# VITA-Group/MLSP

Hardware: AMD Instinct MI355X
Metric: points/sec fwd+bwd, DGCNN+MLSP B=32 N=1024 k=20 (higher is better)
Workload: dtype f32; 1 GPU; DGCNN encoder + 3 MLSP heads + losses, fwd+bwd+Adam, B=32/GPU N=1024 k=20 fp32 (BASELINE.json configs[1]), dropout 0.5, BN train; global_batch=32, points_per_cloud=1024, k=20, parallelism=dp1

## Files before the change

### mlsp_amd/csrc/api.hip

```cpp
#include "common.h"
#include "../../include/mlsp_hip.h"
#include "knn_plan.h"

#define CHECK(x) do { int _r = (x); if (_r != MLSP_OK) return _r; } while (0)
#define SLAB_BOUND_FLOATS ((size_t)16 << 20)

#include <mutex>
#include <unordered_map>
hipError_t mlsp_lds_limit(const void* fn, size_t lds) {
    static std::mutex mu;
    static std::unordered_map<uint64_t, size_t> raised;
    int dev = 0;
    (void)hipGetDevice(&dev);
    const uint64_t key = (uint64_t)(uintptr_t)fn * 64u + (uint64_t)(dev & 63);
    std::lock_guard<std::mutex> lk(mu);
    auto it = raised.find(key);
    if (it != raised.end() && it->second >= lds) return hipSuccess;
    const hipError_t e = hipFuncSetAttribute(fn, hipFuncAttributeMaxDynamicSharedMemorySize, (int)lds);
    if (e == hipSuccess) raised[key] = lds;
    return e;
}

extern "C" {

int mlsp_abi_version(void) { return MLSP_ABI_VERSION; }

const char* mlsp_strerror(int code) {
    switch (code) {
        case MLSP_OK: return "ok";
        case MLSP_ERR_ARG: return "mlsp: bad argument (null pointer, non-positive or unsupported shape)";
        case MLSP_ERR_WORKSPACE: return "mlsp: workspace too small (see mlsp_workspace_bytes)";
        case MLSP_ERR_UNSUPPORTED: return "mlsp: unsupported size for this kernel";
        default: return code > 0 ? hipGetErrorString((hipError_t)code) : "mlsp: unknown error";
    }
}

size_t mlsp_workspace_bytes(int rows, int cin, int cout) {
    size_t r = rows > 0 ? rows : 1, ci = cin > 0 ? cin : 1, co = cout > 0 ? cout : 1;
    size_t act = 3 * r * co * sizeof(float) + r * sizeof(float)
               + r * ci * sizeof(float);
    size_t parts = (r / 64 + 2) * 2 * co * sizeof(double);
    size_t wts = 4 * co * ci * sizeof(float) * 2 + 8 * co * sizeof(float);
    return act + parts + wts + SLAB_BOUND_FLOATS * sizeof(float) + (32 << 20) + MLSP_AMAX_TAIL_BYTES;
}

int mlsp_gemm_f32(int ta, int tb, int M, int N, int K, const float* A, int lda, const float* B, int ldb, float* C, int ldc,
                  const float* bias, int precision, void* ws, size_t ws_bytes, mlsp_stream_t st) {
    CallCtx cx(precision, ws, ws_bytes);
    if (!cx.ok()) return MLSP_ERR_ARG;
    Workspace w(ws, ws_bytes);
    GemmOpts o; o.bias = bias;
    take_slab(w, o, gemm_slab_floats(M, N, K));
    if (!o.slab) o.slab_floats = 0;
    return launch_gemm(st, cx, ta != 0, tb != 0, M, N, K, A, lda, B, ldb, C, ldc, o);
}

int mlsp_knn_f32(const float* x, int ldx, int B, int N, int C, int k, int32_t* idx, int32_t* rev_off, int32_t* rev_ent,
                 void* ws, size_t ws_bytes, mlsp_stream_t st) {
    if (B <= 0 || N <= 0) return MLSP_ERR_ARG;
    Workspace w(ws, ws_bytes);
    float* xx = w.take<float>((size_t)B * N);
    if (!w.ok()) return MLSP_ERR_WORKSPACE;
    KnnAsk q;
    q.B = B; q.N = N; q.C = C; q.k = k; q.ld = ldx; q.x16 = ((uintptr_t)x & 15) == 0; q.planes_avail = (size_t)-1;
    const size_t pbytes = knn_plan(q).plane_bytes;
    char* planes = pbytes ? w.take<char>(pbytes) : nullptr;
    {
        const int cls = C <= 4 ? MLSP_PROF_KNN_C3 : C == 64 ? MLSP_PROF_KNN_C64 : C == 128 ? MLSP_PROF_KNN_C128 : 0;
        const int tok = prof_cls_begin(st, cls);
        const int rc = launch_knn(st, x, ldx, B, N, C, k, idx, xx, planes, planes ? pbytes : 0);
        prof_cls_end(st, tok, C <= 4 ? (double)B * N * (C + k) * 4.0 : 2.0 * B * N * (double)N * C);
        if (rc != MLSP_OK) return rc;
    }
    if (rev_off) CHECK(launch_knn_reverse(st, idx, B, N, k, rev_off, rev_ent));
    return MLSP_OK;
}

int mlsp_knn_reverse(const int32_t* idx, int B, int N, int k, int32_t* rev_off, int32_t* rev_ent, mlsp_stream_t st) {
    return launch_knn_reverse(st, idx, B, N, k, rev_off, rev_ent);
}

int mlsp_region_assign_f32(const float* X, int B, int C, int N, const float* thr, int n, float clip, int32_t* regions, mlsp_stream_t st) {
    return launch_region_assign(st, X, B, C, N, thr, n, clip, regions);
}
int mlsp_deform_regions_f32(float* X, int B, int C, int N, const int32_t* regions, const int32_t* order, int nreg, const float* lookup,
                            const float* noise, int min_pts, int groups, float* mask, mlsp_stream_t st) {
    return launch_deform_regions(st, X, B, C, N, regions, order, nreg, lookup, noise, min_pts, groups, mask);
}
int mlsp_knn_query_f32(const float* ref, int ldr, int Nr, const float* qry, int ldq, int Nq, int B, int C, int k, int32_t* idx, float* dist,
                       mlsp_stream_t st) {
    return launch_knn_query(st, ref, ldr, Nr, qry, ldq, Nq, B, C, k, idx, dist);
}
int mlsp_interp3_fwd_f32(const float* feat, const int32_t* idx, const float* dist, int B, int N, int S, int D, float* out, mlsp_stream_t st) {
    return launch_interp3_fwd(st, feat, idx, dist, B, N, S, D, out);
}
int mlsp_interp3_bwd_f32(const float* dout, const float* dist, const int32_t* rev_off, const int32_t* rev_ent, int B, int N, int S, int D,
                         float* dfeat, mlsp_stream_t st) {
    return launch_interp3_bwd(st, dout, dist, rev_off, rev_ent, B, N, S, D, dfeat);
}
int mlsp_compose_linear_fwd_f32(const float* Wa, const float* ba, const float* Wb, const float* bb, int Cm, int Ci, int Co, float* W, float* b,
                                mlsp_stream_t st) {
    if (!Wa || !ba || !Wb || !bb || !W || !b || Cm <= 0 || Ci <= 0 || Co <= 0 || Cm > 1024 || Ci > 1024 || Co > 1024) return MLSP_ERR_ARG;
    return launch_compose_fwd((hipStream_t)st, Wa, ba, Wb, bb, Cm, Ci, Co, W, b);
}
int mlsp_compose_linear_bwd_f32(const float* dW, const float* db, const float* Wa, const float* ba, const float* Wb, int Cm, int Ci, int Co,
                                float* dWa, float* dba, float* dWb, mlsp_stream_t st) {
    if (!dW || !db || !Wa || !ba || !Wb || !dWa || !dba || !dWb || Cm <= 0 || Ci <= 0 || Co <= 0 || Cm > 1024 || Ci > 1024 || Co > 1024) return MLSP_ERR_ARG;
    return launch_compose_bwd((hipStream_t)st, dW, db, Wa, ba, Wb, Cm, Ci, Co, dWa, dba, dWb);
}

int mlsp_transform3_fwd_f32(const float* x, const float* T, int B, int N, float* out, mlsp_stream_t st) {
    return launch_transform3_fwd(st, x, T, B, N, out);
}
int mlsp_transform3_bwd_f32(const float* x, const float* T, const float* dout, int B, int N, float* dx, float* dT, mlsp_stream_t st) {
    return launch_transform3_bwd(st, x, T, dout, B, N, dx, dT);
}
int mlsp_collapse_to_point_f32(float* X, int B, int N, const int32_t* choice, const float* u, const float* noise, float radius2,
                               int min_pts, float* mask, int32_t* chosen, mlsp_stream_t st) {
    return launch_collapse_to_point(st, X, B, N, choice, u, noise, radius2, min_pts, mask, chosen);
}
int mlsp_scan_select_f32(const float* X, int B, int N, int C, const double* R, int pixel, float* Xs, float* mask, mlsp_stream_t st) {
    return launch_scan_select(st, X, B, N, C, R, pixel, Xs, mask);
}
int mlsp_fps_f32(const float* xyz, int ldx, int B, int N, int S, const int32_t* start, int32_t* fps_idx, mlsp_stream_t st) {
    return launch_fps(st, xyz, ldx, B, N, S, start, fps_idx);
}
int mlsp_ball_query_f32(const float* xyz, int ldx, const float* new_xyz, int ldq, int B, int N, int S, float radius_sq, int nsample,
                        int32_t* idx, mlsp_stream_t st) {
    return launch_ball_query(st, xyz, ldx, new_xyz, ldq, B, N, S, radius_sq, nsample, idx);
}
int mlsp_group_reverse(const int32_t* idx, int B, int S, int N, int ns, int32_t* rev_off, int32_t* rev_ent, mlsp_stream_t st) {
    return launch_group_reverse(st, idx, B, S, N, ns, rev_off, rev_ent);
}
int mlsp_sa_group_fwd_f32(const float* xyz, int ldx, const float* feat, int D, const float* new_xyz, int ldq, const int32_t* idx, int B,
                          int N, int S, int ns, float* G, mlsp_stream_t st) {
    return launch_sa_group_fwd(st, xyz, ldx, feat, D, new_xyz, ldq, idx, B, N, S, ns, G);
}
int mlsp_sa_group_bwd_f32(const float* dG, int ldg, int col, int D, const int32_t* rev_off, const int32_t* rev_ent, int B, int N, int S, int ns,
                          float* dfeat, mlsp_stream_t st) {
    return launch_sa_group_bwd(st, dG, ldg, col, D, rev_off, rev_ent, B, N, S, ns, dfeat);
}


int mlsp_sa_fold_fwd_f32(const float* u, const float* w, const int32_t* idx, int B, int N, int S, int ns, int C, const float* gamma,
                         const float* beta, float* run_mean, float* run_var, float momentum, float eps, int training, float* Z,
                         float* bn_save, void* ws, size_t ws_bytes, mlsp_stream_t st) {
    if (B <= 0 || S <= 0 || ns <= 0 || C <= 0) return MLSP_ERR_ARG;
    Workspace wk(ws, ws_bytes);
    double* part = training ? wk.take<double>((size_t)sa_fold_parts((long)B * S * ns) * 2 * C) : nullptr;
    if (!wk.ok()) return MLSP_ERR_WORKSPACE;
    return launch_sa_fold_fwd(st, u, w, idx, B, N, S, ns, C, gamma, beta, run_mean, run_var, momentum, eps, training, Z, bn_save, part);
}

int mlsp_sa_fold_bwd_f32(const float* dZ, const float* u, const float* w, const int32_t* idx, const int32_t* rev_off, const int32_t* rev_ent,
                         const int32_t* rev_cnt, const int32_t* pad_cnt, int B, int N, int S, int ns, int C, const float* bn_save, int training,
                         float* du, float* dw, float* dgamma, float* dbeta, void* ws, size_t ws_bytes, mlsp_stream_t st) {
    if (B <= 0 || S <= 0 || ns <= 0 || C <= 0) return MLSP_ERR_ARG;
    Workspace wk(ws, ws_bytes);
    double* part = wk.take<double>((size_t)sa_fold_parts((long)B * S * ns) * 2 * C);
    float* mean_dz = wk.take<float>(C);
    float* mean_dzy = wk.take<float>(C);
    if (!wk.ok()) return MLSP_ERR_WORKSPACE;
    return launch_sa_fold_bwd(st, dZ, u, w, idx, rev_off, rev_ent, B, N, S, ns, C, bn_save, training, du, dw, dgamma, dbeta, part, mean_dz,
                              mean_dzy, rev_cnt, pad_cnt);
}

int mlsp_group_reverse_compact(const int32_t* idx, int B, int S, int N, int ns, int32_t* rev_off, int32_t* rev_cnt, int32_t* rev_ent,
                               int32_t* pad_cnt, mlsp_stream_t st) {
    return launch_group_reverse_compact(st, idx, B, S, N, ns, rev_off, rev_cnt, rev_ent, pad_cnt);
}

int mlsp_graph_feature_fwd_f32(const float* x, const int32_t* idx, int B, int N, int C, int k, float* F, mlsp_stream_t st) {
    if (!x || !idx || !F || B <= 0 || N <= 0 || C <= 0 || k <= 0) return MLSP_ERR_ARG;
    return launch_graph_feature_fwd(st, x, idx, B * N, N, C, k, F);
}
int mlsp_graph_feature_bwd_f32(const float* dF, const int32_t* rev_off, const int32_t* rev_ent, int B, int N, int C, int k,
                               float* dx, mlsp_stream_t st) {
    if (!dF || !rev_off || !rev_ent || !dx || B <= 0 || N <= 0 || C <= 0 || k <= 0) return MLSP_ERR_ARG;
    return launch_graph_feature_bwd(st, dF, rev_off, rev_ent, B * N, N, C, k, dx);
}

int mlsp_edgeconv_fwd_f32(const float* x, int ldx, const int32_t* idx, const float* W, const float* gamma, const float* beta,
                          float* run_mean, float* run_var, float momentum, float eps, int act, float slope, int training,
                          int B, int N, int C, int Cout, int k, float* out, int ldo, float* uv, float* msel, uint8_t* argsel,
                          float* s1, float* bn_save, float* Wd_out, int precision, void* ws, size_t ws_bytes, mlsp_stream_t st) {
    CallCtx cx(precision, ws, ws_bytes);
    if (!cx.ok()) return MLSP_ERR_ARG;
    if (!x || !idx || !W || !gamma || !beta || !out || !uv || !msel || !argsel || !s1 || !bn_save) return MLSP_ERR_ARG;
    if (B <= 0 || N <= 0 || C <= 0 || Cout <= 0 || k <= 0 || k > 255 || ldx < C || ldo < Cout) return MLSP_ERR_ARG;
    const int P = B * N;
    Workspace w(ws, ws_bytes);
    float* Wd = Wd_out ? Wd_out : w.take<float>((size_t)2 * Cout * C);
    int nparts = edge_reduce_parts(P);
    double* part = w.take<double>((size_t)nparts * 2 * Cout);
    GemmOpts so; take_slab(w, so, gemm_slab_floats(P, 2 * Cout, C));
    if (!w.ok()) return MLSP_ERR_WORKSPACE;
    float* scale = bn_save, *shift = bn_save + Cout, *mean = bn_save + 2 * Cout, *invstd = bn_save + 3 * Cout;
    if (!training) {
        if (!run_mean || !run_var) return MLSP_ERR_ARG;
        CHECK(launch_build_wd_eval(st, W, Cout, C, Wd, Cout, gamma, beta, run_mean, run_var, bn_save, 0, nullptr, nullptr, nullptr, nullptr, nullptr, eps));
    } else CHECK(launch_build_wd(st, W, Cout, C, Wd, (C >= 128 && C % 32 == 0 && build_wd_leaves_bound(Cout, C)) ? cx.reserve(Wd, 2 * Cout, C, C) : nullptr));
    CHECK(launch_gemm(st, cx, false, true, P, 2 * Cout, C, x, ldx, Wd, C, uv, 2 * Cout, so));
    {
        const int tok = prof_cls_begin(st, MLSP_PROF_EDGE_REDUCE);
        const int rc = launch_edge_reduce(st, uv, idx, gamma, P, N, Cout, k, msel, argsel, s1, part, &nparts);
        prof_cls_end(st, tok, (double)P * (Cout * 4.0 + k * 4.0 + Cout * 9.0));
        if (rc != MLSP_OK) return rc;
    }
    if (training) {
        CHECK(launch_bn_finalize(st, part, nparts, (double)P * k, Cout, gamma, beta, run_mean, run_var, momentum, eps, scale,
                                 shift, mean, invstd, cx.offered_output(out, P, Cout, ldo, Cout)));
    }
    CHECK(launch_edge_select_act(st, msel, uv, P, Cout, scale, shift, act, slope, out, ldo));
    return MLSP_OK;
}

int mlsp_edgeconv_bwd_f32(const float* dOut, int lddo, const float* x, int ldx, const int32_t* rev_off, const int32_t* rev_ent,
                          const float* W, const float* out, int ldo, const float* uv, const float* msel, const uint8_t* argsel,
                          const float* s1, const float* bn_save, const float* Wd_in, int act, float slope, int training, int B, int N, int C,
                          int Cout, int k, float* dx, int lddx, int dx_accumulate, float* dW, float* dgamma, float* dbeta, int precision, void* ws,
                          size_t ws_bytes, mlsp_stream_t st) {
    CallCtx cx(precision, ws, ws_bytes);
    if (!cx.ok()) return MLSP_ERR_ARG;
    if (!dOut || !x || !rev_off || !rev_ent || !W || !out || !uv || !msel || !argsel || !s1 || !bn_save || !dW || !dgamma ||
        !dbeta)
        return MLSP_ERR_ARG;
    if (B <= 0 || N <= 0 || C <= 0 || Cout <= 0 || k <= 0 || ldx < C || lddo < Cout || ldo < Cout || (dx && lddx < C)) return MLSP_ERR_ARG;
    const int P = B * N;
    Workspace w(ws, ws_bytes);
    float* Wd = Wd_in ? nullptr : w.take<float>((size_t)2 * Cout * C);
    float* dWd = w.take<float>((size_t)2 * Cout * C);
    float* gz = w.take<float>((size_t)P * Cout);
    float* duv = w.take<float>((size_t)P * 2 * Cout);
    int nparts = bn_parts_max(P);
    double* part = w.take<double>((size_t)nparts * 2 * Cout);
    float* mean_dz = w.take<float>(Cout);
    float* mean_dzy = w.take<float>(Cout);
    GemmOpts so; take_slab(w, so, gemm_slab_floats(P, C, 2 * Cout), gemm_slab_floats(2 * Cout, C, P));
    if (!w.ok()) return MLSP_ERR_WORKSPACE;
    const float* scale = bn_save, *mean = bn_save + 2 * Cout, *invstd = bn_save + 3 * Cout;
    float* duv_amax = (C % 128 == 0 && edge_bwd_leaves_duv_bound(dOut, out, msel, uv, s1, argsel, Cout, scale, mean, invstd, gz, duv, lddo, ldo))
                          ? cx.reserve(duv, P, 2 * Cout, 2 * Cout) : nullptr;
    CHECK(launch_edge_bwd_reduce(st, dOut, out, msel, uv, P, Cout, mean, invstd, act, slope, part, lddo, ldo, duv_amax));
    CHECK(launch_bn_bwd_finalize(st, part, edge_bwd_reduce_parts(P, Cout, dOut, out, msel, uv, mean, invstd, lddo, ldo), (double)P * k, Cout,
                                 dgamma, dbeta, mean_dz, mean_dzy));
    const float* mdz = training ? mean_dz : nullptr;
    CHECK(launch_edge_bwd_point(st, dOut, out, uv, s1, P, Cout, k, scale, mean, invstd, mdz, mean_dzy, act, slope, gz, duv, lddo, ldo, duv_amax));
    CHECK(launch_edge_bwd_gather(st, gz, argsel, uv, rev_off, rev_ent, P, N, Cout, scale, mean, invstd, mdz, mean_dzy, duv, duv_amax));
    const float* Wdc = Wd_in;
    if (!Wdc && dx) { CHECK(launch_build_wd(st, W, Cout, C, Wd)); Wdc = Wd; }
    GemmOpts od = so; od.accumulate = dx_accumulate != 0;
    if (dx) CHECK(launch_gemm(st, cx, false, false, P, C, 2 * Cout, duv, 2 * Cout, Wdc, C, dx, lddx, od));
    bool unfolded = false;
    GemmOpts ow = so; ow.unfold_dw = dW; ow.unfolded = &unfolded;
    CHECK(launch_gemm(st, cx, true, false, 2 * Cout, C, P, duv, 2 * Cout, x, ldx, dWd, C, ow));
    if (!unfolded) CHECK(launch_unbuild_wd(st, dWd, Cout, C, dW));
    return MLSP_OK;
}

int mlsp_tnet_edge_fwd_f32(const float* x, int ldx, const int32_t* idx, const float* W1, const float* gamma1, const float* beta1,
                           float* run_mean1, float* run_var1, const float* W2, const float* gamma2, const float* beta2,
                           float* run_mean2, float* run_var2, float momentum, float eps, float slope, int training, int B, int N,
                           int C, int C1, int C2, int k, float* out, float* uv, float* s1, float* bn1_save, float* zsel,
                           uint8_t* argsel, float* bn2_save, int precision, void* ws, size_t ws_bytes, mlsp_stream_t st) {
    CallCtx cx(precision, ws, ws_bytes);
    if (!cx.ok()) return MLSP_ERR_ARG;
    if (!x || !idx || !W1 || !gamma1 || !beta1 || !W2 || !gamma2 || !beta2 || !out || !uv || !s1 || !bn1_save || !zsel || !argsel ||
        !bn2_save)
        return MLSP_ERR_ARG;
    if (B <= 0 || N <= 0 || C <= 0 || k <= 0 || ldx < C) return MLSP_ERR_ARG;
    if (C1 != 64 || C2 != 128 || tnet_points_per_tile(k) <= 0) return MLSP_ERR_UNSUPPORTED;
    const int P = B * N;
    Workspace w(ws, ws_bytes);
    float* Wd = w.take<float>((size_t)2 * C1 * C);
    float* msel = w.take<float>((size_t)P * C1);
    uint8_t* arg1 = w.take<uint8_t>((size_t)P * C1);
    int np1 = edge_reduce_parts(P), np2 = tnet_fwd_parts(B, N, k);
    double* part = w.take<double>((size_t)(np1 > np2 ? np1 : np2) * 2 * C2);
    GemmOpts so; take_slab(w, so, gemm_slab_floats(P, 2 * C1, C));
    if (!w.ok()) return MLSP_ERR_WORKSPACE;
    if (!training) {
        if (!run_mean1 || !run_var1 || !run_mean2 || !run_var2) return MLSP_ERR_ARG;
        CHECK(launch_build_wd_eval(st, W1, C1, C, Wd, C1, gamma1, beta1, run_mean1, run_var1, bn1_save, C2, gamma2, beta2, run_mean2, run_var2, bn2_save, eps));
    } else CHECK(launch_build_wd(st, W1, C1, C, Wd));
    CHECK(launch_gemm(st, cx, false, true, P, 2 * C1, C, x, ldx, Wd, C, uv, 2 * C1, so));
    CHECK(launch_edge_reduce(st, uv, idx, gamma1, P, N, C1, k, msel, arg1, s1, part, &np1));
    if (training) {
        CHECK(launch_bn_finalize(st, part, np1, (double)P * k, C1, gamma1, beta1, run_mean1, run_var1, momentum, eps, bn1_save,
                                 bn1_save + C1, bn1_save + 2 * C1, bn1_save + 3 * C1));
    }
    {
        const int tok = prof_cls_begin(st, MLSP_PROF_TNET_FWD);
        const int rc = launch_tnet_edge_fwd(st, cx.mode(), uv, idx, bn1_save, W2, gamma2, P, N, k, slope, zsel, argsel, part);
        prof_cls_end(st, tok, 2.0 * P * (double)k * C1 * C2);
        if (rc != MLSP_OK) return rc;
    }
    if (training) {
        CHECK(launch_bn_finalize(st, part, np2, (double)P * k, C2, gamma2, beta2, run_mean2, run_var2, momentum, eps, bn2_save,
                                 bn2_save + C2, bn2_save + 2 * C2, bn2_save + 3 * C2, cx.offered_output(out, P, C2, C2, C2)));
    }
    CHECK(launch_tnet_out(st, zsel, bn2_save, P, slope, out));
    return MLSP_OK;
}

int mlsp_tnet_edge_bwd_f32(const float* dOut, const float* x, int ldx, const int32_t* idx, const int32_t* rev_off,
                           const int32_t* rev_ent, const float* W1, const float* W2, const float* out, const float* uv,
                           const float* s1, const float* bn1_save, const float* zsel, const uint8_t* argsel, const float* bn2_save,
                           float slope, int training, int B, int N, int C, int C1, int C2, int k, float* dx, float* dW1,
                           float* dgamma1, float* dbeta1, float* dW2, float* dgamma2, float* dbeta2, int precision, void* ws, size_t ws_bytes,
                           mlsp_stream_t st) {
    CallCtx cx(precision, ws, ws_bytes);
    if (!cx.ok()) return MLSP_ERR_ARG;
    if (!dOut || !x || !idx || !W1 || !W2 || !out || !uv || !s1 || !bn1_save || !zsel || !argsel || !bn2_save ||
        !dW1 || !dgamma1 || !dbeta1 || !dW2 || !dgamma2 || !dbeta2)
        return MLSP_ERR_ARG;
    if ((!rev_off || !rev_ent) && (dx || C > 4)) return MLSP_ERR_ARG;
    if (B <= 0 || N <= 0 || C <= 0 || k <= 0 || ldx < C) return MLSP_ERR_ARG;
    if (C1 != 64 || C2 != 128 || tnet_points_per_tile(k) <= 0) return MLSP_ERR_UNSUPPORTED;
    const int P = B * N;
    const size_t E = (size_t)P * k;
    const int ntiles = B * ((N + tnet_points_per_tile(k) - 1) / tnet_points_per_tile(k));
    const int nb = tnet_grid(ntiles);
    Workspace w(ws, ws_bytes);
    float* Wd = w.take<float>((size_t)2 * C1 * C);
    float* dWd = w.take<float>((size_t)2 * C1 * C);
    float* g = w.take<float>((size_t)P * C2);
    float* coef = w.take<float>(2 * C2);
    float* dhp = w.take<float>(E * C1);
    float* dW2part = w.take<float>(tnet_bwd_scratch_floats(ntiles));
    int npr = (P + 511) / 512;
    const int nprv = bn_vec_parts(P);
    const int nrows_part = (npr > nb ? npr : nb) > nprv ? (npr > nb ? npr : nb) : nprv;
    double* part = w.take<double>((size_t)nrows_part * 2 * C2);
    float* mean_dz = w.take<float>(C2);
    float* mean_dzy = w.take<float>(C2);
    float* m1 = w.take<float>(C1);
    float* m2 = w.take<float>(C1);
    float* duv = w.take<float>((size_t)P * 2 * C1);
    GemmOpts so; take_slab(w, so, gemm_slab_floats(P, C, 2 * C1), gemm_slab_floats(2 * C1, C, P));
    if (!w.ok()) return MLSP_ERR_WORKSPACE;
    {
        const int rc = launch_bn_act_bwd_partials_vec(st, dOut, zsel, P, C2, bn2_save, bn2_save + C2, bn2_save + 2 * C2, bn2_save + 3 * C2,
                                                      2, slope, part);
        if (rc == MLSP_OK) npr = nprv;
        else if (rc != MLSP_ERR_UNSUPPORTED) return rc;
        else CHECK(launch_tnet_bwd_reduce(st, dOut, out, zsel, bn2_save, P, slope, part));
    }
    CHECK(launch_bn_bwd_finalize(st, part, npr, (double)E, C2, dgamma2, dbeta2, mean_dz, mean_dzy));
    CHECK(launch_tnet_bwd_g(st, dOut, out, bn2_save, training ? mean_dz : nullptr, mean_dzy, P, slope, g, coef));
    int nparts = 0;
    {
        const int tok = prof_cls_begin(st, MLSP_PROF_TNET_BWD);
        const int rc = launch_tnet_edge_bwd(st, cx.mode(), uv, idx, bn1_save, W2, bn2_save, g, argsel, coef, P, N, k, slope, dhp, dW2part, part, dW2, &nparts);
        prof_cls_end(st, tok, 4.0 * P * (double)k * C1 * C2);
        if (rc != MLSP_OK) return rc;
    }
    CHECK(launch_bn_bwd_finalize(st, part, nparts, (double)E, C1, dgamma1, dbeta1, m1, m2));
    if (!dx && C <= 4) {
        double* mom = w.take<double>(tnet_w1_moment_doubles(P, k));
        if (!w.ok()) return MLSP_ERR_WORKSPACE;
        return launch_tnet_bwd_w1_moments(st, dhp, idx, rev_off, x, ldx, W1, bn1_save, training ? m1 : nullptr, m2, P, N, k, C, mom, dW1);
    }
    CHECK(launch_tnet_edge_bwd2(st, dhp, uv, s1, bn1_save, training ? m1 : nullptr, m2, rev_off, rev_ent, P, N, k, duv));
    CHECK(launch_build_wd(st, W1, C1, C, Wd));
    if (dx) CHECK(launch_gemm(st, cx, false, false, P, C, 2 * C1, duv, 2 * C1, Wd, C, dx, C, so));
    CHECK(launch_gemm(st, cx, true, false, 2 * C1, C, P, duv, 2 * C1, x, ldx, dWd, C, so));
    CHECK(launch_unbuild_wd(st, dWd, C1, C, dW1));
    return MLSP_OK;
}

static bool defer_ok(const mlsp_defer_t* in) {
    return in->bn_save && in->ld > 0 && in->col >= 0 && in->p_drop >= 0.f && in->p_drop < 1.f && in->act >= 0 && in->act <= 2;
}
static GemmXf chain_xf(const mlsp_defer_t& in, int which, int batch_stats) {
    GemmXf x;
    x.scale = in.bn_save + in.col; x.shift = in.bn_save + in.ld + in.col; x.act = in.act; x.slope = in.slope; x.thresh = dropout_thresh8(in.p_drop);
    x.inv_keep = dropout_inv_keep8(in.p_drop); x.seed = in.seed; x.ld = in.ld; x.col = in.col; x.which = which;
    if (batch_stats) { x.mean = in.bn_save + 2 * in.ld + in.col; x.invstd = in.bn_save + 3 * in.ld + in.col; }
    return x;
}
static bool defer_fusable(const mlsp_defer_t& in) { return !(in.act == 2 && !(in.slope >= 0.f && in.slope <= 1.f)); }

static int pointmlp_fwd_impl(CallCtx& cx, const float* X, int ldx, int M, int Cin, const float* W, int ldw, int Cout, const float* bias,
                             const float* gbias, int rows_per_group, const float* gamma, const float* beta, float* run_mean,
                             float* run_var, float momentum, float eps, int training, int act, float slope, float p_drop,
                             uint64_t seed, float* Y, float* Z, float* bn_save, void* ws, size_t ws_bytes, mlsp_stream_t st,
                             const mlsp_defer_t* in, float* group_ysum) {
    if (!X || !W || (!Z && !gamma) || M <= 0 || Cin <= 0 || Cout <= 0 || ldx < Cin || ldw < Cin) return MLSP_ERR_ARG;
    if (group_ysum && (!gamma || !gbias || rows_per_group <= 0 || M % rows_per_group || M <= 32)) return MLSP_ERR_ARG;
    if (gamma && (!beta || !Y || !bn_save)) return MLSP_ERR_ARG;
    if (p_drop < 0.f || p_drop >= 1.f) return MLSP_ERR_ARG;
    if (in && (!defer_ok(in) || in->col + Cin > in->ld)) return MLSP_ERR_ARG;
    if (gamma && !gbias && M <= 32 && !in && Z)
        return launch_skinny_linear_bn_act(st, X, ldx, M, Cin, W, ldw, Cout, bias, gamma, beta, run_mean, run_var, momentum, eps,
                                           training, act, slope, p_drop, seed, Y, Z, bn_save);
    Workspace w(ws, ws_bytes);
    const int fused_parts = (gamma && training) ? gemm_stat_parts(cx, M, Cout, Cin) : 0;
    int nparts = fused_parts ? fused_parts : bn_stat_parts(M);
    double* part = gamma ? w.take<double>((size_t)nparts * 2 * Cout) : nullptr;
    GemmOpts o; o.bias = bias; o.gbias = gbias; o.rows_per_group = rows_per_group;
    take_slab(w, o, gemm_slab_floats(M, Cout, Cin));
    GemmXf xf_s;
    if (in) {
        xf_s = chain_xf(*in, 1, training);
        if (defer_fusable(*in) && gemm_xf_supported(cx, false, true, M, Cout, Cin, X, ldx, W, ldw, 1)) o.xf = &xf_s;
        else {
            float* Xa = w.take<float>((size_t)M * Cin);
            if (!w.ok()) return MLSP_ERR_WORKSPACE;
            CHECK(launch_xf_materialize(st, X, ldx, M, Cin, xf_s, Xa));
            X = Xa; ldx = Cin;
        }
    }
    if (!w.ok()) return MLSP_ERR_WORKSPACE;
    if (!gamma) {
        if (act || p_drop > 0.f) return MLSP_ERR_UNSUPPORTED;
        return launch_gemm(st, cx, false, true, M, Cout, Cin, X, ldx, W, ldw, Z, Cout, o);
    }
    float* scale = bn_save, *shift = bn_save + Cout, *mean = bn_save + 2 * Cout, *invstd = bn_save + 3 * Cout;
    o.stat_part = fused_parts ? part : nullptr;
    CHECK(launch_gemm(st, cx, false, true, M, Cout, Cin, X, ldx, W, ldw, Y, Cout, o));
    const int prow = fused_parts ? M / fused_parts : 0;
    const bool gsum_fin = group_ysum && training && fused_parts && M % fused_parts == 0 && rows_per_group % prow == 0;
    if (training) {
        if (!fused_parts) CHECK(launch_colstats(st, Y, M, Cout, Cout, part));
        if (gsum_fin) CHECK(launch_bn_finalize_groups(st, part, nparts, (double)M, Cout, gamma, beta, run_mean, run_var, momentum, eps, scale, shift,
                                                      mean, invstd, group_ysum, rows_per_group / prow));
        else CHECK(launch_bn_finalize(st, part, nparts, (double)M, Cout, gamma, beta, run_mean, run_var, momentum, eps, scale, shift,
                                      mean, invstd));
    } else {
        if (!run_mean || !run_var) return MLSP_ERR_ARG;
        CHECK(launch_bn_eval_prepare(st, Cout, gamma, beta, run_mean, run_var, eps, scale, shift, mean, invstd));
    }
    if (group_ysum && !gsum_fin) {
        float* gscr = w.take<float>((size_t)(M / rows_per_group) * 16 * Cout);
        if (!w.ok()) return MLSP_ERR_WORKSPACE;
        CHECK(launch_colsum_groups(st, Y, M / rows_per_group, rows_per_group, Cout, group_ysum, gscr));
    }
    if (Z) CHECK(launch_bn_act_fwd(st, Y, Z, (size_t)M, Cout, scale, shift, act, slope, training ? p_drop : 0.f, seed));
    return MLSP_OK;
}

int mlsp_pointmlp_fwd_f32(const float* X, int ldx, int M, int Cin, const float* W, int ldw, int Cout, const float* bias,
                          const float* gbias, int rows_per_group, const float* gamma, const float* beta, float* run_mean,
                          float* run_var, float momentum, float eps, int training, int act, float slope, float p_drop,
                          uint64_t seed, float* Y, float* Z, float* bn_save, float* group_ysum, int precision, void* ws, size_t ws_bytes,
                          mlsp_stream_t st) {
    CallCtx cx(precision, ws, ws_bytes);
    if (!cx.ok()) return MLSP_ERR_ARG;
    return pointmlp_fwd_impl(cx, X, ldx, M, Cin, W, ldw, Cout, bias, gbias, rows_per_group, gamma, beta, run_mean, run_var, momentum, eps,
                             training, act, slope, p_drop, seed, Y, Z, bn_save, ws, ws_bytes, st, nullptr, group_ysum);
}

int mlsp_pointmlp_fwd_chain_f32(const float* Xpre, int ldx, const mlsp_defer_t* in, int M, int Cin, const float* W, int ldw, int Cout, const float* bias,
                                const float* gbias, int rows_per_group, const float* gamma, const float* beta, float* run_mean,
                                float* run_var, float momentum, float eps, int training, int act, float slope, float p_drop,
                                uint64_t seed, float* Y, float* Z, float* bn_save, float* group_ysum, int precision, void* ws, size_t ws_bytes,
                                mlsp_stream_t st) {
    CallCtx cx(precision, ws, ws_bytes);
    if (!cx.ok()) return MLSP_ERR_ARG;
    if (!in) return MLSP_ERR_ARG;
    return pointmlp_fwd_impl(cx, Xpre, ldx, M, Cin, W, ldw, Cout, bias, gbias, rows_per_group, gamma, beta, run_mean, run_var, momentum, eps,
                             training, act, slope, p_drop, seed, Y, Z, bn_save, ws, ws_bytes, st, in, group_ysum);
}

static int pointmlp_bwd_impl(CallCtx& cx, const float* dZ, const float* X, int ldx, int M, int Cin, const float* W, int ldw, int Cout, const float* Y,
                             const float* bn_save, int has_bn, int training, int act, float slope, float p_drop, uint64_t seed,
                             int n_groups, int rows_per_group, float* dX, int lddx, int dx_accumulate, float* dW, float* dbias, float* dgbias,
                             float* dgamma, float* dbeta, void* ws, size_t ws_bytes, mlsp_stream_t st, const mlsp_defer_t* in,
                             double* in_stats, const double* pre_stats, int pre_parts, const float* group_ysum) {
    if (!dZ || !X || !W || !dW || M <= 0 || Cin <= 0 || Cout <= 0 || ldx < Cin || ldw < Cin) return MLSP_ERR_ARG;
    if (in_stats && (!in || !dX || dx_accumulate)) return MLSP_ERR_ARG;
    if (pre_stats && (!has_bn || pre_parts <= 0 || M <= 32)) return MLSP_ERR_ARG;
    if (!pre_stats && pre_parts < 0 && (!has_bn || M <= 32)) return MLSP_ERR_ARG;
    if (has_bn && (!Y || !bn_save || !dgamma || !dbeta)) return MLSP_ERR_ARG;
    if (dgbias && (n_groups <= 0 || rows_per_group <= 0 || (long)n_groups * rows_per_group != M)) return MLSP_ERR_ARG;
    Workspace w(ws, ws_bytes);
    float* dY = has_bn ? w.take<float>((size_t)M * Cout) : nullptr;
    int nparts = bn_parts_max(M);
    double* part = (has_bn || dbias) ? w.take<double>((size_t)nparts * 2 * Cout) : nullptr;
    float* mean_dz = has_bn ? w.take<float>(Cout) : nullptr;
    float* mean_dzy = has_bn ? w.take<float>(Cout) : nullptr;
    GemmOpts so; take_slab(w, so, dX ? gemm_slab_floats(M, Cin, Cout) : 0, gemm_slab_floats(Cout, Cin, M));
    float* gscratch = dgbias ? w.take<float>((size_t)n_groups * 16 * Cout) : nullptr;
    float* coef = has_bn ? w.take<float>((size_t)4 * Cout) : nullptr;
    const float* Xorig = X; const int ldx_orig = ldx;
    GemmXf xf_s; const GemmXf* xf = nullptr;
    if (in) {
        if (!defer_ok(in) || in->col + Cin > in->ld || M <= 32) return MLSP_ERR_ARG;
        xf_s = chain_xf(*in, 2, training);
        if (defer_fusable(*in) && gemm_xf_supported(cx, true, false, Cout, Cin, M, dZ, Cout, X, ldx, 2)) xf = &xf_s;
        else {
            float* Xa = w.take<float>((size_t)M * Cin);
            if (!w.ok()) return MLSP_ERR_WORKSPACE;
            CHECK(launch_xf_materialize(st, X, ldx, M, Cin, xf_s, Xa));
            X = Xa; ldx = Cin;
        }
    }
    if (!w.ok()) return MLSP_ERR_WORKSPACE;
    const float* g = dZ;
    int g_slabs = 0;
    GemmDy dy_s = {Y, coef, Cout, 1}; const GemmDy* dy = nullptr;
    if (has_bn && M > 32 && pre_stats && training && (!in || xf) && M % pre_parts == 0 &&
        (!dX || gemm_dy_supported(cx, false, false, M, Cin, Cout, dZ, Cout, W, ldw)) && gemm_dy_supported(cx, true, false, Cout, Cin, M, dZ, Cout, X, ldx) &&
        (!dgbias || (rows_per_group >= 256 && rows_per_group % (M / pre_parts) == 0 && Cout % 4 == 0 && 256 % (Cout / 4) == 0 && Cout <= 1024)))
        dy = &dy_s;
    float* zb = (dbias && has_bn && training) ? dbias : nullptr;
    bool dbias_zeroed = false;
    if (dy && dgbias && group_ysum) {
        CHECK(launch_bn_bwd_finalize_coef_groups(st, pre_stats, pre_parts, (double)M, Cout, bn_save, dgamma, dbeta, coef, group_ysum,
                                                 rows_per_group / (M / pre_parts), rows_per_group, dgbias));
    } else if (dy) {
        CHECK(launch_bn_bwd_finalize_coef_z(st, pre_stats, pre_parts, (double)M, Cout, bn_save, dgamma, dbeta, coef, zb));
        dbias_zeroed = zb != nullptr;
        if (dgbias) CHECK(launch_bn_dy_gbias(st, Y, n_groups, rows_per_group, Cout, pre_stats, M / pre_parts, coef, gscratch, dgbias, group_ysum));
    } else if (has_bn && M <= 32) {
        CHECK(launch_skinny_bn_bwd_z(st, dZ, Y, dY, M, Cout, bn_save, training, act, slope, p_drop, seed, dgamma, dbeta, zb));
        dbias_zeroed = zb != nullptr;
        g = dY;
    } else if (has_bn) {
        const float* scale = bn_save, *shift = bn_save + Cout, *mean = bn_save + 2 * Cout, *invstd = bn_save + 3 * Cout;
        CHECK(launch_bn_act_bwd(st, dZ, Y, dY, M, Cout, scale, shift, mean, invstd, training, act, slope, training ? p_drop : 0.f, seed, part,
                                dgamma, dbeta, mean_dz, mean_dzy, zb, dgbias ? gscratch : nullptr, rows_per_group, &g_slabs, pre_stats, pre_parts));
        dbias_zeroed = zb != nullptr;
        g = dY;
    }
    GemmBs bs_s; const GemmBs* bs = nullptr;
    if (in_stats) {
        bs_s = {Xorig, ldx_orig, in->bn_save + in->col, in->ld, in->act, in->slope, dropout_thresh8(in->p_drop), dropout_inv_keep8(in->p_drop), in->seed,
                in->ld, in->col, in_stats + in->col, in->ld};
        bs_s.amax = (float*)(in_stats + (size_t)(M / 128) * 2 * in->ld) + in->col;
        bs = &bs_s;
    }
    if (M <= 32 && dX && !bs && !dy && !xf) {
        CHECK(launch_skinny_bwd_pair(st, g, Cout, W, ldw, X, ldx, dX, lddx, dW, M, Cin, Cout, dx_accumulate));
    } else {
    GemmOpts od = so; od.accumulate = dx_accumulate != 0; od.bs = bs; od.dy = dy;
    if (dX) CHECK(launch_gemm(st, cx, false, false, M, Cin, Cout, g, Cout, W, ldw, dX, lddx, od));
    GemmOpts ow = so; ow.xf = xf; ow.dy = dy;
    CHECK(launch_gemm(st, cx, true, false, Cout, Cin, M, g, Cout, X, ldx, dW, Cin, ow));
    }
    if (dbias) {
        if (has_bn && training) {
            if (!dbias_zeroed) {
                hipError_t e = hipMemsetAsync(dbias, 0, (size_t)Cout * sizeof(float), st);
                if (e != hipSuccess) return (int)e;
            }
        } else {
            CHECK(launch_colsum(st, g, M, Cout, part, dbias));
        }
    }
    if (dgbias && !dy) {
        if (g_slabs > 0) CHECK(launch_colsum_groups_fin(st, gscratch, n_groups, Cout, g_slabs, dgbias));
        else CHECK(launch_colsum_groups(st, g, n_groups, rows_per_group, Cout, dgbias, gscratch));
    }
    return MLSP_OK;
}

int mlsp_pointmlp_bwd_f32(const float* dZ, const float* X, int ldx, int M, int Cin, const float* W, int ldw, int Cout, const float* Y,
                          const float* bn_save, int has_bn, int training, int act, float slope, float p_drop, uint64_t seed,
                          int n_groups, int rows_per_group, float* dX, int lddx, int dx_accumulate, float* dW, float* dbias, float* dgbias,
                          float* dgamma, float* dbeta, const double* pre_stats, int pre_parts, const float* group_ysum, int precision, void* ws,
                          size_t ws_bytes, mlsp_stream_t st) {
    CallCtx cx(precision, ws, ws_bytes);
    if (!cx.ok()) return MLSP_ERR_ARG;
    return pointmlp_bwd_impl(cx, dZ, X, ldx, M, Cin, W, ldw, Cout, Y, bn_save, has_bn, training, act, slope, p_drop, seed, n_groups,
                             rows_per_group, dX, lddx, dx_accumulate, dW, dbias, dgbias, dgamma, dbeta, ws, ws_bytes, st, nullptr, nullptr,
                             pre_stats, pre_parts, group_ysum);
}

int mlsp_pointmlp_bwd_stats_parts(int M, int Cin, int Cout, int ldw, int lddx, int precision) {
    const CallCtx cx = CallCtx::query(precision);
    if (!cx.ok()) return 0;
    const int t = thin_bs_parts(M, Cin, Cout);
    return t ? t : gemm_bs_parts(cx, M, Cin, Cout, Cout, ldw, lddx);
}

int mlsp_pointmlp_bwd_chain_f32(const float* dZ, const float* Xpre, int ldx, const mlsp_defer_t* in, int M, int Cin, const float* W, int ldw, int Cout, const float* Y,
                                const float* bn_save, int has_bn, int training, int act, float slope, float p_drop, uint64_t seed,
                                int n_groups, int rows_per_group, float* dX, int lddx, int dx_accumulate, float* dW, float* dbias,
                                float* dgbias, float* dgamma, float* dbeta, double* in_stats, const double* pre_stats, int pre_parts,
                                const float* group_ysum, int precision, void* ws, size_t ws_bytes, mlsp_stream_t st) {
    CallCtx cx(precision, ws, ws_bytes);
    if (!cx.ok()) return MLSP_ERR_ARG;
    if (!in) return MLSP_ERR_ARG;
    return pointmlp_bwd_impl(cx, dZ, Xpre, ldx, M, Cin, W, ldw, Cout, Y, bn_save, has_bn, training, act, slope, p_drop, seed, n_groups,
                             rows_per_group, dX, lddx, dx_accumulate, dW, dbias, dgbias, dgamma, dbeta, ws, ws_bytes, st, in, in_stats,
                             pre_stats, pre_parts, group_ysum);
}

int mlsp_pointmlp_segmax_fwd_f32(const float* X, int ldx, int M, int Cin, const float* W, int ldw, int Cout, const float* bias,
                                 const float* gamma, const float* beta, float* run_mean, float* run_var, float momentum, float eps,
                                 int training, int act, float slope, int k, float* Y, float* out, float* ysel, uint8_t* argk, float* bn_save,
                                 int precision, void* ws, size_t ws_bytes, mlsp_stream_t st) {
    CallCtx cx(precision, ws, ws_bytes);
    if (!cx.ok()) return MLSP_ERR_ARG;
    if (!X || !W || !gamma || !beta || !Y || !out || !ysel || !argk || !bn_save || M <= 0 || Cin <= 0 || Cout <= 0 || ldx < Cin || ldw < Cin)
        return MLSP_ERR_ARG;
    if (k < 1 || k > 255 || M % k || Cout % 4) return MLSP_ERR_UNSUPPORTED;
    Workspace w(ws, ws_bytes);
    const int fused_parts = training ? gemm_stat_parts(cx, M, Cout, Cin) : 0;
    int nparts = fused_parts ? fused_parts : bn_stat_parts(M);
    double* part = w.take<double>((size_t)nparts * 2 * Cout);
    GemmOpts o; o.bias = bias; o.stat_part = fused_parts ? part : nullptr;
    take_slab(w, o, gemm_slab_floats(M, Cout, Cin));
    if (!w.ok()) return MLSP_ERR_WORKSPACE;
    float* scale = bn_save, *shift = bn_save + Cout, *mean = bn_save + 2 * Cout, *invstd = bn_save + 3 * Cout;
    CHECK(launch_gemm(st, cx, false, true, M, Cout, Cin, X, ldx, W, ldw, Y, Cout, o));
    if (training) {
        if (!fused_parts) CHECK(launch_colstats(st, Y, M, Cout, Cout, part));
        CHECK(launch_bn_finalize(st, part, nparts, (double)M, Cout, gamma, beta, run_mean, run_var, momentum, eps, scale, shift, mean, invstd));
    } else {
        if (!run_mean || !run_var) return MLSP_ERR_ARG;
        CHECK(launch_bn_eval_prepare(st, Cout, gamma, beta, run_mean, run_var, eps, scale, shift, mean, invstd));
    }
    return launch_segsel_act_fwd(st, Y, M / k, k, Cout, scale, shift, act, slope, out, ysel, argk);
}

int mlsp_pointmlp_segmax_bwd_f32(const float* dOut, const float* X, int ldx, int M, int Cin, const float* W, int ldw, int Cout, const float* Y,
                                 const float* ysel, const uint8_t* argk, const float* bn_save, int training, int act, float slope, int k,
                                 float* dX, int lddx, float* dW, float* dbias, float* dgamma, float* dbeta, int precision, void* ws, size_t ws_bytes,
                                 mlsp_stream_t st) {
    CallCtx cx(precision, ws, ws_bytes);
    if (!cx.ok()) return MLSP_ERR_ARG;
    if (!dOut || !X || !W || !Y || !ysel || !argk || !bn_save || !dW || !dgamma || !dbeta || M <= 0 || Cin <= 0 || Cout <= 0 || ldx < Cin ||
        ldw < Cin) return MLSP_ERR_ARG;
    if (k < 1 || k > 255 || M % k || Cout % 4) return MLSP_ERR_UNSUPPORTED;
    const int G = M / k;
    Workspace w(ws, ws_bytes);
    float* dY = w.take<float>((size_t)M * Cout);
    const int npr = bn_vec_parts(G);
    double* part = w.take<double>((size_t)npr * 2 * Cout);
    float* mean_dz = w.take<float>(Cout);
    float* mean_dzy = w.take<float>(Cout);
    GemmOpts so; take_slab(w, so, dX ? gemm_slab_floats(M, Cin, Cout) : 0, gemm_slab_floats(Cout, Cin, M));
    if (!w.ok()) return MLSP_ERR_WORKSPACE;
    const float* scale = bn_save, *shift = bn_save + Cout, *mean = bn_save + 2 * Cout, *invstd = bn_save + 3 * Cout;
    {
        const int rc = launch_bn_act_bwd_partials_vec(st, dOut, ysel, G, Cout, scale, shift, mean, invstd, act, slope, part);
        if (rc != MLSP_OK) return rc;
    }
    CHECK(launch_bn_bwd_finalize(st, part, npr, (double)M, Cout, dgamma, dbeta, mean_dz, mean_dzy));
    CHECK(launch_segsel_bwd_apply(st, dOut, Y, ysel, argk, (size_t)M, k, Cout, bn_save, training ? mean_dz : nullptr, mean_dzy, act, slope, dY));
    if (dX) CHECK(launch_gemm(st, cx, false, false, M, Cin, Cout, dY, Cout, W, ldw, dX, lddx, so));
    CHECK(launch_gemm(st, cx, true, false, Cout, Cin, M, dY, Cout, X, ldx, dW, Cin, so));
    if (dbias) {
        if (training) {
            hipError_t e = hipMemsetAsync(dbias, 0, (size_t)Cout * sizeof(float), st);
            if (e != hipSuccess) return (int)e;
        } else {
            CHECK(launch_colsum(st, dY, M, Cout, part, dbias));
        }
    }
    return MLSP_OK;
}

static int pointmlp_mx_supported(const CallCtx& cx, int M, int Cin, int Cout, int ldx, int x_bf16, int training) {
    if (M <= 32 || Cin % 32 || Cout % 128 || M % 128) return 0;
    if (x_bf16 ? (ldx % 8) : (ldx % 4)) return 0;
    if (Cout > 1024 || 256 % (Cout / 4)) return 0;
    if (training && gemm_stat_parts(cx, M, Cout, Cin) <= 0) return 0;
    if (gemm_slab_floats(M, Cout, Cin) != 0 || gemm_slab_floats(M, Cin, Cout) != 0) return 0;
    return 1;
}

int mlsp_pointmlp_mx_supported(int M, int Cin, int Cout, int ldx, int x_bf16, int training, int precision) {
    const CallCtx cx = CallCtx::query(precision);
    return cx.ok() ? pointmlp_mx_supported(cx, M, Cin, Cout, ldx, x_bf16, training) : 0;
}

int mlsp_pointmlp_fwd_mx(const void* X, int x_bf16, int ldx, int M, int Cin, const float* W, int ldw, int Cout, const float* bias,
                         const float* gbias, int rows_per_group, const float* gamma, const float* beta, float* run_mean,
                         float* run_var, float momentum, float eps, int training, int act, float slope, float p_drop, uint64_t seed,
                         void* Y, void* Z, int out_bf16, float* bn_save, int precision, void* ws, size_t ws_bytes, mlsp_stream_t st) {
    CallCtx cx(precision, ws, ws_bytes);
    if (!cx.ok()) return MLSP_ERR_ARG;
    if (!X || !W || !Y || !Z || !gamma || !beta || !bn_save || ldw < Cin || ldx < Cin) return MLSP_ERR_ARG;
    if (p_drop < 0.f || p_drop >= 1.f) return MLSP_ERR_ARG;
    if (!pointmlp_mx_supported(cx, M, Cin, Cout, ldx, x_bf16, training)) return MLSP_ERR_UNSUPPORTED;
    Workspace w(ws, ws_bytes);
    const int fused_parts = training ? gemm_stat_parts(cx, M, Cout, Cin) : 0;
    double* part = w.take<double>((size_t)(fused_parts ? fused_parts : 1) * 2 * Cout);
    if (!w.ok()) return MLSP_ERR_WORKSPACE;
    float* scale = bn_save, *shift = bn_save + Cout, *mean = bn_save + 2 * Cout, *invstd = bn_save + 3 * Cout;
    GemmOpts o; o.bias = bias; o.gbias = gbias; o.rows_per_group = rows_per_group; o.stat_part = fused_parts ? part : nullptr;
    CHECK(launch_gemm_mx(st, cx, false, true, M, Cout, Cin, X, x_bf16, ldx, W, 0, ldw, Y, out_bf16, Cout, o));
    if (training) {
        CHECK(launch_bn_finalize(st, part, fused_parts, (double)M, Cout, gamma, beta, run_mean, run_var, momentum, eps, scale, shift,
                                 mean, invstd));
    } else {
        if (!run_mean || !run_var) return MLSP_ERR_ARG;
        CHECK(launch_bn_eval_prepare(st, Cout, gamma, beta, run_mean, run_var, eps, scale, shift, mean, invstd));
    }
    if (out_bf16) return launch_bn_act_fwd_b16(st, Y, Z, M, Cout, scale, shift, act, slope, training ? p_drop : 0.f, seed);
    return launch_bn_act_fwd(st, (const float*)Y, (float*)Z, (size_t)M, Cout, scale, shift, act, slope, training ? p_drop : 0.f, seed);
}

int mlsp_pointmlp_bwd_mx(const void* dZ, const void* X, int x_bf16, int ldx, int M, int Cin, const float* W, int ldw, int Cout,
                         const void* Y, int out_bf16, const float* bn_save, int training, int act, float slope, float p_drop,
                         uint64_t seed, int n_groups, int rows_per_group, void* dX, int lddx, int dx_accumulate, float* dW, float* dbias,
                         float* dgbias, float* dgamma, float* dbeta, int precision, void* ws, size_t ws_bytes, mlsp_stream_t st) {
    CallCtx cx(precision, ws, ws_bytes);
    if (!cx.ok()) return MLSP_ERR_ARG;
    if (!dZ || !X || !W || !Y || !bn_save || !dW || !dgamma || !dbeta || ldw < Cin || ldx < Cin) return MLSP_ERR_ARG;
    if (dgbias && (n_groups <= 0 || rows_per_group <= 0 || (long)n_groups * rows_per_group != M)) return MLSP_ERR_ARG;
    if (!pointmlp_mx_supported(cx, M, Cin, Cout, ldx, x_bf16, training)) return MLSP_ERR_UNSUPPORTED;
    if (dbias && !training) return MLSP_ERR_UNSUPPORTED;
    Workspace w(ws, ws_bytes);
    void* dY = w.take<char>((size_t)M * Cout * (out_bf16 ? 2 : 4));
    const int nparts = bn_parts_max(M);
    double* part = w.take<double>((size_t)nparts * 2 * Cout);
    float* mean_dz = w.take<float>(Cout);
    float* mean_dzy = w.take<float>(Cout);
    GemmOpts ow; take_slab(w, ow, gemm_slab_floats(Cout, Cin, M));
    float* gscratch = dgbias ? w.take<float>((size_t)n_groups * 16 * Cout) : nullptr;
    if (!w.ok()) return MLSP_ERR_WORKSPACE;
    const float* scale = bn_save, *shift = bn_save + Cout, *mean = bn_save + 2 * Cout, *invstd = bn_save + 3 * Cout;
    if (out_bf16) CHECK(launch_bn_act_bwd_b16(st, dZ, Y, dY, M, Cout, scale, shift, mean, invstd, training, act, slope, training ? p_drop : 0.f, seed,
                                              part, dgamma, dbeta, mean_dz, mean_dzy, dbias));
    else CHECK(launch_bn_act_bwd(st, (const float*)dZ, (const float*)Y, (float*)dY, M, Cout, scale, shift, mean, invstd, training, act, slope,
                                 training ? p_drop : 0.f, seed, part, dgamma, dbeta, mean_dz, mean_dzy, dbias));
    GemmOpts od; od.accumulate = dx_accumulate != 0;
    if (dX) CHECK(launch_gemm_mx(st, cx, false, false, M, Cin, Cout, dY, out_bf16, Cout, W, 0, ldw, dX, x_bf16, lddx, od));
    CHECK(launch_gemm_mx(st, cx, true, false, Cout, Cin, M, dY, out_bf16, Cout, X, x_bf16, ldx, dW, 0, Cin, ow));
    if (dgbias) {
        if (out_bf16) CHECK(launch_colsum_groups_b16(st, dY, n_groups, rows_per_group, Cout, dgbias, gscratch));
        else CHECK(launch_colsum_groups(st, (const float*)dY, n_groups, rows_per_group, Cout, dgbias, gscratch));
    }
    return MLSP_OK;
}

static int colmax_fused_panel_rows(const CallCtx& cx, int N, int P, int Cin, int Cout) {
    const int prow = gemm_panel_rows(cx, P, Cout, Cin);
    return ((N % prow == 0) && gemm_stat_parts(cx, P, Cout, Cin) > 0) ? prow : 0;
}

int mlsp_pointmlp_colmax_panel_rows(int B, int N, int Cin, int Cout, int precision) {
    const CallCtx cx = CallCtx::query(precision);
    if (!cx.ok() || B <= 0 || N <= 0 || Cin <= 0 || Cout <= 0) return 0;
    return colmax_fused_panel_rows(cx, N, B * N, Cin, Cout);
}

int mlsp_pointmlp_colmax_fwd_f32(const float* X, int ldx, int B, int N, int Cin, const float* W, int ldw, int Cout,
                                 const float* gamma, const float* beta, float* run_mean, float* run_var, float momentum, float eps,
                                 int training, int act, float slope, float* out, float* ysel, int32_t* arg, float* bn_save, int precision, void* ws,
                                 size_t ws_bytes, mlsp_stream_t st) {
    CallCtx cx(precision, ws, ws_bytes);
    if (!cx.ok()) return MLSP_ERR_ARG;
    if (!X || !W || !gamma || !beta || !out || !ysel || !arg || !bn_save) return MLSP_ERR_ARG;
    if (B <= 0 || N <= 0 || Cin <= 0 || Cout <= 0 || ldx < Cin || ldw < Cin) return MLSP_ERR_ARG;
    const int P = B * N;
    Workspace w(ws, ws_bytes);
    const int fused_parts = training ? gemm_stat_parts(cx, P, Cout, Cin) : 0;
    const int prow = colmax_fused_panel_rows(cx, N, P, Cin, Cout);
    const bool fuse_sel = prow > 0;
    float* Y = fuse_sel ? nullptr : w.take<float>((size_t)P * Cout);
    float* pv = fuse_sel ? w.take<float>((size_t)(P / prow) * Cout) : nullptr;
    int* pr = fuse_sel ? w.take<int>((size_t)(P / prow) * Cout) : nullptr;
    int nparts = fused_parts ? fused_parts : bn_stat_parts(P);
    double* part = w.take<double>((size_t)nparts * 2 * Cout);
    GemmOpts o; o.stat_part = fused_parts ? part : nullptr; o.sel_gamma = fuse_sel ? gamma : nullptr; o.sel_val = pv; o.sel_row = pr;
    take_slab(w, o, gemm_slab_floats(P, Cout, Cin));
    if (!w.ok()) return MLSP_ERR_WORKSPACE;
    CHECK(launch_gemm(st, cx, false, true, P, Cout, Cin, X, ldx, W, ldw, Y, Cout, o));
    if (training) {
        if (!fused_parts) CHECK(launch_colstats(st, Y, P, Cout, Cout, part));
        CHECK(launch_bn_finalize(st, part, nparts, (double)P, Cout, gamma, beta, run_mean, run_var, momentum, eps, bn_save,
                                 bn_save + Cout, bn_save + 2 * Cout, bn_save + 3 * Cout));
    } else {
        if (!run_mean || !run_var) return MLSP_ERR_ARG;
        CHECK(launch_bn_eval_prepare(st, Cout, gamma, beta, run_mean, run_var, eps, bn_save, bn_save + Cout, bn_save + 2 * Cout,
                                     bn_save + 3 * Cout));
    }
    if (fuse_sel) CHECK(launch_colsel_panels(st, pv, pr, gamma, B, N, Cout, prow, ysel, arg, bn_save, act, slope, out));
    else {
        CHECK(launch_colsel(st, Y, gamma, B, N, Cout, ysel, arg));
        CHECK(launch_colsel_out(st, ysel, bn_save, B, Cout, act, slope, out));
    }
    return MLSP_OK;
}

int mlsp_pointmlp_colmax_bwd_f32(const float* dOut, const float* X, int ldx, int B, int N, int Cin, const float* W, int ldw,
                                 int Cout, const float* out, const float* ysel, const int32_t* arg, const float* bn_save,
                                 int training, int act, float slope, float* dX, int dx_accumulate, float* dW, float* dgamma, float* dbeta,
                                 int precision, void* ws, size_t ws_bytes, mlsp_stream_t st) {
    CallCtx cx(precision, ws, ws_bytes);
    if (!cx.ok()) return MLSP_ERR_ARG;
    if (!dOut || !X || !W || !out || !ysel || !arg || !bn_save || !dW || !dgamma || !dbeta) return MLSP_ERR_ARG;
    if (B <= 0 || N <= 0 || Cin <= 0 || Cout <= 0 || ldx != Cin || ldw < Cin) return MLSP_ERR_ARG;
    const int P = B * N;
    Workspace w(ws, ws_bytes);
    float* g = w.take<float>((size_t)B * Cout);
    float* coef = w.take<float>((size_t)4 * Cout);
    float* S = w.take<float>((size_t)Cout * Cin);
    float* sx = w.take<float>(Cin);
    double* part = w.take<double>((size_t)bn_parts_max(P) * 2 * Cin);
    float* G = w.take<float>((size_t)Cin * Cin);
    float* WG = w.take<float>((size_t)Cout * Cin);
    float* Wb = w.take<float>((size_t)Cout * Cin);
    float* Mneg = w.take<float>((size_t)Cin * Cin);
    float* negr = w.take<float>(Cin);
    const size_t s1 = gemm_slab_floats(Cin, Cin, P), s2 = gemm_slab_floats(Cout, Cin, Cin), s3 = gemm_slab_floats(Cin, Cin, Cout),
                 s4 = gemm_slab_floats(P, Cin, Cin);
    GemmOpts so; take_slab(w, so, s1 > s2 ? s1 : s2, s3 > s4 ? s3 : s4);
    if (!w.ok()) return MLSP_ERR_WORKSPACE;
    CHECK(launch_colmax_bwd_coef(st, dOut, out, ysel, bn_save, B, Cout, (double)P, act, slope, training, g, coef, dgamma, dbeta));
    CHECK(launch_colmax_gather_rows(st, g, arg, X, ldx, B, N, Cout, Cin, S));
    if (training) {
        CHECK(launch_colsum(st, X, P, Cin, part, sx));
        CHECK(launch_gemm(st, cx, true, false, Cin, Cin, P, X, ldx, X, ldx, G, Cin, so));
        CHECK(launch_gemm(st, cx, false, false, Cout, Cin, Cin, W, ldw, G, Cin, WG, Cin, so));
        CHECK(launch_colmax_dw(st, S, WG, sx, coef, bn_save, Cout, Cin, dW));
    } else {
        hipError_t e = hipMemcpyAsync(dW, S, (size_t)Cout * Cin * sizeof(float), hipMemcpyDeviceToDevice, st);
        if (e != hipSuccess) return (int)e;
    }
    if (dX) {
        if (training) {
            CHECK(launch_wt_vec_neg_scale_rows(st, W, ldw, coef + 2 * Cout, coef + 3 * Cout, Cout, Cin, negr, Wb));
            CHECK(launch_gemm(st, cx, true, false, Cin, Cin, Cout, Wb, Cin, W, ldw, Mneg, Cin, so));
            GemmOpts od = so; od.bias = negr; od.accumulate = dx_accumulate != 0;
            CHECK(launch_gemm(st, cx, false, false, P, Cin, Cin, X, ldx, Mneg, Cin, dX, Cin, od));
        } else if (!dx_accumulate) {
            hipError_t e = hipMemsetAsync(dX, 0, (size_t)P * Cin * sizeof(float), st);
            if (e != hipSuccess) return (int)e;
        }
        CHECK(launch_colmax_scatter_rows(st, g, arg, W, ldw, B, N, Cout, Cin, dX, Cin));
    }
    return MLSP_OK;
}

int mlsp_radius_count_f32(const float* x, int ldx, int B, int N, float radius, int max_nn, int32_t* count, mlsp_stream_t st) {
    if (!x || !count || B <= 0 || N <= 0 || ldx < 3 || !(radius > 0.f) || max_nn <= 0) return MLSP_ERR_ARG;
    return launch_radius_count(st, x, ldx, B, N, radius, max_nn, count);
}
int mlsp_knn_normals_f32(const float* x, int ldx, const int32_t* idx, int B, int N, int k, float* normals, mlsp_stream_t st) {
    if (!x || !idx || !normals || B <= 0 || N <= 0 || k < 3 || ldx < 3) return MLSP_ERR_ARG;
    return launch_knn_normals(st, x, ldx, idx, B, N, k, normals);
}

int mlsp_segmax_fwd_f32(const float* Z, int P, int k, int C, float* out, uint8_t* argk, mlsp_stream_t st) {
    if (!Z || !out || !argk || P <= 0 || k <= 0 || k > 255 || C <= 0) return MLSP_ERR_ARG;
    return launch_segmax_fwd(st, Z, P, k, C, out, argk);
}
int mlsp_segmax_bwd_f32(const float* dOut, const uint8_t* argk, int P, int k, int C, float* dZ, mlsp_stream_t st) {
    if (!dOut || !argk || !dZ || P <= 0 || k <= 0 || C <= 0) return MLSP_ERR_ARG;
    return launch_segmax_bwd(st, dOut, argk, P, k, C, dZ);
}
int mlsp_colmax_fwd_f32(const float* Z, int B, int N, int C, float* out, int32_t* arg, mlsp_stream_t st) {
    if (!Z || !out || !arg || B <= 0 || N <= 0 || C <= 0) return MLSP_ERR_ARG;
    return launch_colmax_fwd(st, Z, B, N, C, out, arg);
}
int mlsp_colmax_bwd_f32(const float* dOut, const int32_t* arg, int B, int N, int C, float* dZ, mlsp_stream_t st) {
    if (!dOut || !arg || !dZ || B <= 0 || N <= 0 || C <= 0) return MLSP_ERR_ARG;
    return launch_colmax_bwd(st, dOut, arg, B, N, C, dZ);
}

int mlsp_chamfer_masked_fwd_f32(const float* pred, const float* gold, const float* mask, int B, int N, float scale,
                                float* per_cloud, int32_t* argA, int32_t* argB, float* loss, mlsp_stream_t st) {
    if (!pred || !gold || !mask || !per_cloud || !argA || !argB || !loss || B <= 0 || N <= 0) return MLSP_ERR_ARG;
    return launch_chamfer_fwd(st, pred, gold, mask, B, N, scale, per_cloud, argA, argB, loss);
}
int mlsp_chamfer_masked_bwd_f32(const float* pred, const float* gold, const float* mask, int B, int N, float scale,
                                const float* per_cloud, const int32_t* argA, const int32_t* argB, const float* grad_loss,
                                float* dpred, mlsp_stream_t st) {
    if (!pred || !gold || !mask || !per_cloud || !argA || !argB || !grad_loss || !dpred || B <= 0 || N <= 0) return MLSP_ERR_ARG;
    return launch_chamfer_bwd(st, pred, gold, mask, B, N, scale, per_cloud, argA, argB, grad_loss, dpred);
}

int mlsp_chamfer_dir_fwd_f32(const float* p1, const float* p2, const float* mask_cord, int B, int N, float* per_cloud, int32_t* arg,
                             float* loss, mlsp_stream_t st) {
    if (!p1 || !p2 || !mask_cord || !per_cloud || !arg || !loss || B <= 0 || N <= 0) return MLSP_ERR_ARG;
    return launch_chamfer_dir_fwd(st, p1, p2, mask_cord, B, N, per_cloud, arg, loss);
}
int mlsp_chamfer_dir_bwd_f32(const float* p1, const float* p2, const float* mask_cord, int B, int N, const float* per_cloud,
                             const int32_t* arg, const float* grad_loss, float* dp1, float* dp2, mlsp_stream_t st) {
    if (!p1 || !p2 || !mask_cord || !per_cloud || !arg || !grad_loss || (!dp1 && !dp2) || B <= 0 || N <= 0) return MLSP_ERR_ARG;
    return launch_chamfer_dir_bwd(st, p1, p2, mask_cord, B, N, per_cloud, arg, grad_loss, dp1, dp2);
}

int mlsp_normal_loss_fwd_f32(const float* pred, const float* gt, const float* wgt, int P, float weight, float* out, void* ws,
                             size_t ws_bytes, mlsp_stream_t st) {
    if (!pred || !gt || !out || P <= 0) return MLSP_ERR_ARG;
    Workspace w(ws, ws_bytes);
    double* part = w.take<double>(256 * 2);
    if (!w.ok()) return MLSP_ERR_WORKSPACE;
    return launch_normal_loss_fwd(st, pred, gt, wgt, P, weight, part, out);
}
int mlsp_normal_loss_bwd_f32(const float* pred, const float* gt, const float* wgt, int P, float weight, const float* fwd_out,
                             const float* grad_loss, float* dpred, mlsp_stream_t st) {
    if (!pred || !gt || !fwd_out || !grad_loss || !dpred || P <= 0) return MLSP_ERR_ARG;
    return launch_normal_loss_bwd(st, pred, gt, wgt, P, weight, fwd_out, grad_loss, dpred);
}

int mlsp_density_tail_fwd_f32(const float* logits, const float* fc2w, int P, int nc, float* pvec, float* dens, mlsp_stream_t st) {
    if (!logits || !fc2w || !pvec || !dens || P <= 0 || nc <= 0) return MLSP_ERR_ARG;
    return launch_density_tail_fwd(st, logits, fc2w, P, nc, pvec, dens);
}
int mlsp_density_tail_bwd_f32(const float* pvec, const float* fc2w, const float* dpvec, const float* ddens, int P, int nc,
                              float* dlogits, mlsp_stream_t st) {
    if (!pvec || !fc2w || !dlogits || P <= 0 || nc <= 0) return MLSP_ERR_ARG;
    return launch_density_tail_bwd(st, pvec, fc2w, dpvec, ddens, P, nc, dlogits);
}

int mlsp_density_loss_fwd_f32(const float* pvec, const float* dens, const float* target_vec, const float* target,
                              const float* mask, int P, int nc, float density_weight, float* out, void* ws, size_t ws_bytes,
                              mlsp_stream_t st) {
    if (!pvec || !dens || !target_vec || !target || !out || P <= 0 || nc <= 0) return MLSP_ERR_ARG;
    Workspace w(ws, ws_bytes);
    double* part = w.take<double>(256 * 3);
    if (!w.ok()) return MLSP_ERR_WORKSPACE;
    return launch_density_loss_fwd(st, pvec, dens, target_vec, target, mask, P, nc, density_weight, part, out);
}
int mlsp_density_loss_bwd_f32(const float* pvec, const float* dens, const float* target_vec, const float* target,
                              const float* mask, int P, int nc, float density_weight, const float* fwd_out,
                              const float* grad_kl, const float* grad_mae, float* dpvec, float* ddens, mlsp_stream_t st) {
    if (!pvec || !dens || !target_vec || !target || !fwd_out || !dpvec || !ddens || P <= 0 || nc <= 0) return MLSP_ERR_ARG;
    return launch_density_loss_bwd(st, pvec, dens, target_vec, target, mask, P, nc, density_weight, fwd_out, grad_kl, grad_mae,
                                   dpvec, ddens);
}

int mlsp_def_nearest_index_f32(const float* pred, const float* gold, const float* mask, int B, int N, int64_t* index1, int64_t* index2,
                               mlsp_stream_t st) {
    if (!pred || !gold || !mask || !index1 || !index2 || B <= 0 || N <= 0) return MLSP_ERR_ARG;
    return launch_def_nearest(st, pred, gold, mask, B, N, index1, index2);
}
int mlsp_def_normal_loss_fwd_f32(const float* pred, const float* labels, const float* mask, const int64_t* index1, const int64_t* index2,
                                 int B, int N, int defpart, float weight, float* out, void* ws, size_t ws_bytes, mlsp_stream_t st) {
    if (!pred || !labels || !mask || !index1 || !index2 || !out || B <= 0 || N <= 0) return MLSP_ERR_ARG;
    Workspace w(ws, ws_bytes);
    double* part = w.take<double>((size_t)B * 2);
    if (!w.ok()) return MLSP_ERR_WORKSPACE;
    return launch_def_normal_fwd(st, pred, labels, mask, index1, index2, B, N, defpart, weight, part, out);
}
int mlsp_def_normal_loss_bwd_f32(const float* pred, const float* labels, const float* mask, const int64_t* index1, const int64_t* index2,
                                 int B, int N, int defpart, float weight, const float* fwd_out, const float* grad_loss, float* dpred,
                                 mlsp_stream_t st) {
    if (!pred || !labels || !mask || !index1 || !index2 || !fwd_out || !grad_loss || !dpred || B <= 0 || N <= 0) return MLSP_ERR_ARG;
    return launch_def_normal_bwd(st, pred, labels, mask, index1, index2, B, N, defpart, weight, fwd_out, grad_loss, dpred);
}
int mlsp_def_density_loss_fwd_f32(const float* pvec, const float* dens, const float* label_vec, const float* label_val, const float* mask,
                                  const int64_t* index1, const int64_t* index2, int B, int N, int nc, int defpart, float density_weight,
                                  float* out, void* ws, size_t ws_bytes, mlsp_stream_t st) {
    if (!pvec || !dens || !label_vec || !label_val || !mask || !index1 || !index2 || !out || B <= 0 || N <= 0 || nc <= 0 ||
        (long long)B * N > INT32_MAX)
        return MLSP_ERR_ARG;
    Workspace w(ws, ws_bytes);
    double* part = w.take<double>(256 * 3);
    if (!w.ok()) return MLSP_ERR_WORKSPACE;
    return launch_def_density_fwd(st, pvec, dens, label_vec, label_val, mask, index1, index2, B, N, nc, defpart, density_weight, part,
                                  out);
}
int mlsp_def_density_loss_bwd_f32(const float* pvec, const float* dens, const float* label_vec, const float* label_val, const float* mask,
                                  const int64_t* index1, const int64_t* index2, int B, int N, int nc, int defpart, float density_weight,
                                  const float* fwd_out, const float* grad_kl, const float* grad_mae, float* dpvec, float* ddens,
                                  mlsp_stream_t st) {
    if (!pvec || !dens || !label_vec || !label_val || !mask || !index1 || !index2 || !fwd_out || !dpvec || !ddens || B <= 0 || N <= 0 ||
        nc <= 0)
        return MLSP_ERR_ARG;
    return launch_def_density_bwd(st, pvec, dens, label_vec, label_val, mask, index1, index2, B, N, nc, defpart, density_weight, fwd_out,
                                  grad_kl, grad_mae, dpvec, ddens);
}
int mlsp_gather_rows_u32(const void* x, const int64_t* index, int B, int N, int W, void* out, mlsp_stream_t st) {
    if (!x || !index || !out || B <= 0 || N <= 0 || W <= 0) return MLSP_ERR_ARG;
    return launch_def_gather(st, (const uint32_t*)x, index, B, N, W, (uint32_t*)out);
}
int mlsp_gather_rows_bwd_f32(const float* dout, const int64_t* index, int B, int N, int C, float* dx, mlsp_stream_t st) {
    if (!dout || !index || !dx || B <= 0 || N <= 0 || C <= 0 || (long long)N * C > INT32_MAX) return MLSP_ERR_ARG;
    return launch_def_gather_bwd(st, dout, index, B, N, C, dx);
}

int mlsp_vecattn_delta_fwd_f32(const float* xyz, int ldx, const int32_t* idx, const float* Wd1, const float* bd1, int B, int N, int k, int d,
                               float* H1, mlsp_stream_t st) {
    if (!xyz || !idx || !Wd1 || !bd1 || !H1 || B <= 0 || N <= 0 || k <= 0 || d <= 0) return MLSP_ERR_ARG;
    return launch_vecattn_delta_fwd(st, xyz, ldx, idx, Wd1, bd1, B, N, k, d, H1);
}
int mlsp_vecattn_delta_bwd_f32(const float* dH1, const float* H1, const float* xyz, int ldx, const int32_t* idx, int B, int N, int k, int d,
                               float* dWd1, float* dbd1, void* ws, size_t ws_bytes, mlsp_stream_t st) {
    if (!dH1 || !H1 || !xyz || !idx || !dWd1 || !dbd1 || B <= 0 || N <= 0 || k <= 0 || d <= 0) return MLSP_ERR_ARG;
    if (d % 4 || k > 64) return MLSP_ERR_UNSUPPORTED;
    Workspace w(ws, ws_bytes);
    float* part = w.take<float>(vecattn_delta_bwd_ws_floats(B, N, k, d));
    if (!w.ok()) return MLSP_ERR_WORKSPACE;
    return launch_vecattn_delta_bwd(st, dH1, H1, xyz, ldx, idx, B, N, k, d, part, dWd1, dbd1);
}
int mlsp_vecattn_mix_fwd_f32(const float* q, int ldq, const float* kk, int ldk, const float* pos, const int32_t* idx, int B, int N, int k, int d,
                             float* T, mlsp_stream_t st) {
    if (!q || !kk || !pos || !idx || !T || B <= 0 || N <= 0 || k <= 0 || d <= 0) return MLSP_ERR_ARG;
    return launch_vecattn_mix_fwd(st, q, ldq, kk, ldk, pos, idx, B, N, k, d, T);
}
int mlsp_vecattn_mix_bwd_f32(const float* dT, int B, int N, int k, int d, float* dq, mlsp_stream_t st) {
    if (!dT || !dq || B <= 0 || N <= 0 || k <= 0 || d <= 0) return MLSP_ERR_ARG;
    return launch_vecattn_mix_bwd(st, dT, B, N, k, d, dq);
}
int mlsp_vecattn_aggregate_fwd_f32(const float* A, const float* v, int ldv, const float* pos, const int32_t* idx, int B, int N, int k, int d,
                                   float* attn, float* res, mlsp_stream_t st) {
    if (!A || !v || !pos || !idx || !attn || !res || B <= 0 || N <= 0 || k <= 0 || d <= 0) return MLSP_ERR_ARG;
    return launch_vecattn_aggregate_fwd(st, A, v, ldv, pos, idx, B, N, k, d, attn, res);
}
int mlsp_vecattn_aggregate_bwd_f32(const float* dres, const float* attn, const float* v, int ldv, const float* pos, const int32_t* idx, int B,
                                   int N, int k, int d, float* dVP, float* dA, mlsp_stream_t st) {
    if (!dres || !attn || !v || !pos || !idx || !dVP || !dA || B <= 0 || N <= 0 || k <= 0 || d <= 0) return MLSP_ERR_ARG;
    return launch_vecattn_aggregate_bwd(st, dres, attn, v, ldv, pos, idx, B, N, k, d, dVP, dA);
}
int mlsp_vecattn_relu_fwd_f32(const float* x, int64_t rows, int d, float* y, mlsp_stream_t st) {
    if (!x || !y) return MLSP_ERR_ARG;
    return launch_vecattn_relu_fwd(st, x, rows, d, y);
}
int mlsp_vecattn_relu_bwd_f32(const float* dy, const float* y, int64_t rows, int d, float* dx, mlsp_stream_t st) {
    if (!dy || !y || !dx) return MLSP_ERR_ARG;
    return launch_vecattn_relu_bwd(st, dy, y, rows, d, dx);
}

int mlsp_mhsa_fwd_f32(const float* qkv, int ld, int B, int L, int H, int dh, float scale, float* out, float* lse, mlsp_stream_t st) {
    if (!qkv || !out || !lse || B <= 0 || L <= 0 || H <= 0 || dh <= 0) return MLSP_ERR_ARG;
    return launch_mhsa_fwd(st, qkv, ld, B, L, H, dh, scale, out, lse);
}
int mlsp_mhsa_bwd_f32(const float* qkv, int ld, const float* lse, const float* dout, int B, int L, int H, int dh, float scale, float* dqkv, int ldd,
                      mlsp_stream_t st) {
    if (!qkv || !lse || !dout || !dqkv || B <= 0 || L <= 0 || H <= 0 || dh <= 0) return MLSP_ERR_ARG;
    return launch_mhsa_bwd(st, qkv, ld, lse, dout, B, L, H, dh, scale, dqkv, ldd);
}
int mlsp_layernorm_fwd_f32(const float* x, const float* add, const float* sample_scale, int rows_per_sample, const float* gamma, const float* beta,
                           int64_t rows, int d, float eps, float* u, float* y, float* mean, float* rstd, mlsp_stream_t st) {
    if (!x || (sample_scale && !add) || (!gamma && !(add && u)) || (gamma && (!beta || !y || !mean || !rstd)) || (add && !u)) return MLSP_ERR_ARG;
    return launch_layernorm_fwd(st, x, add, sample_scale, rows_per_sample, gamma, beta, rows, d, eps, u, y, mean, rstd);
}
int mlsp_layernorm_bwd_f32(const float* dy, const float* du, const float* u, const float* sample_scale, int rows_per_sample, const float* gamma,
                           const float* mean, const float* rstd, int64_t rows, int d, float* dx, float* dadd, float* dgamma, float* dbeta,
                           void* ws, size_t ws_bytes, mlsp_stream_t st) {
    if (dy ? (!u || !gamma || !mean || !rstd || !dx || !dgamma || !dbeta) : (!du || !dadd)) return MLSP_ERR_ARG;
    if (rows <= 0 || d <= 0 || d % 4) return MLSP_ERR_UNSUPPORTED;
    Workspace w(ws, ws_bytes);
    float* part = dy ? w.take<float>(layernorm_bwd_ws_floats(rows, d)) : nullptr;
    if (!w.ok()) return MLSP_ERR_WORKSPACE;
    return launch_layernorm_bwd(st, dy, du, u, sample_scale, rows_per_sample, gamma, mean, rstd, rows, d, dx, dadd, part, dgamma, dbeta);
}
int mlsp_gelu_fwd_f32(const float* x, int64_t rows, int d, float* y, mlsp_stream_t st) {
    if (!x || !y) return MLSP_ERR_ARG;
    return launch_gelu_fwd(st, x, rows, d, y);
}
int mlsp_gelu_bwd_f32(const float* dy, const float* x, int64_t rows, int d, float* dx, mlsp_stream_t st) {
    if (!dy || !x || !dx) return MLSP_ERR_ARG;
    return launch_gelu_bwd(st, dy, x, rows, d, dx);
}

size_t mlsp_gn_edge_workspace_bytes(int B, int Nk, int Nq, int k, int C, int groups) { return gn_edge_ws_bytes(B, Nk, Nq, k, C, groups); }
int mlsp_gn_edge_fwd_f32(const float* u, int ldu, const float* w, int ldw, const int32_t* idx, const float* gamma, const float* beta, int B, int Nk,
                         int Nq, int k, int C, int groups, float eps, float slope, float* out, uint8_t* argk, float* stats, void* ws,
                         size_t ws_bytes, mlsp_stream_t st) {
    if (!u || !w || !idx || !gamma || !beta || !out || !argk || !stats || B <= 0 || Nk <= 0 || Nq <= 0 || k <= 0 || C <= 0 || groups <= 0)
        return MLSP_ERR_ARG;
    Workspace wsp(ws, ws_bytes);
    return launch_gn_edge_fwd(st, u, ldu, w, ldw, idx, gamma, beta, B, Nk, Nq, k, C, groups, eps, slope, out, argk, stats, wsp);
}
int mlsp_gn_edge_bwd_f32(const float* dOut, const float* u, int ldu, const float* w, int ldw, const int32_t* idx, const uint8_t* argk,
                         const float* stats, const int32_t* rev_off, const int32_t* rev_ent, const float* gamma, const float* beta, int B, int Nk,
                         int Nq, int k, int C, int groups, float slope, float* du, float* dw, float* dgamma, float* dbeta, void* ws,
                         size_t ws_bytes, mlsp_stream_t st) {
    if (!dOut || !u || !w || !idx || !argk || !stats || !rev_off || !rev_ent || !gamma || !beta || !du || !dw || !dgamma || !dbeta || B <= 0 ||
        Nk <= 0 || Nq <= 0 || k <= 0 || C <= 0 || groups <= 0)
        return MLSP_ERR_ARG;
    Workspace wsp(ws, ws_bytes);
    return launch_gn_edge_bwd(st, dOut, u, ldu, w, ldw, idx, argk, stats, rev_off, rev_ent, gamma, beta, B, Nk, Nq, k, C, groups, slope, du, dw,
                              dgamma, dbeta, wsp);
}

size_t mlsp_thin_in_workspace_bytes(int M, int Cin, int C) { return thin_in_ws_bytes(M, Cin, C); }
int mlsp_thin_in_fwd_f32(const float* X, int ldx, int M, int Cin, const float* W, const float* bias, int C, const float* gamma, const float* beta,
                         float* run_mean, float* run_var, float momentum, float eps, int training, int act, float* H, float* bn_save, double* xmom,
                         void* ws, size_t ws_bytes, mlsp_stream_t st) {
    const bool bn = gamma != nullptr;
    if (!X || !W || !H || (bn && (!beta || !bn_save)) || (!bn && beta) || M <= 0 || Cin <= 0 || C <= 0) return MLSP_ERR_ARG;
    if (bn && training && (M < 2 || !xmom)) return MLSP_ERR_ARG;
    if (bn && !training && (!run_mean || !run_var)) return MLSP_ERR_ARG;
    Workspace wsp(ws, ws_bytes);
    return launch_thin_in_fwd(st, X, ldx, M, Cin, W, bias, C, gamma, beta, run_mean, run_var, momentum, eps, training, act, H, bn_save, xmom, wsp);
}
int mlsp_thin_in_bwd_f32(const float* dH, const float* X, int ldx, int M, int Cin, const float* W, const float* bias, int C, const float* gamma,
                         const float* beta, const float* bn_save, const double* xmom, int training, int act, float* dW, float* db, float* dgamma,
                         float* dbeta, void* ws, size_t ws_bytes, mlsp_stream_t st) {
    const bool bn = gamma != nullptr;
    if (!dH || !X || !W || !dW || (bn && (!beta || !bn_save || !dgamma || !dbeta)) || (!bn && beta) || M <= 0 || Cin <= 0 || C <= 0)
        return MLSP_ERR_ARG;
    if (bn && training && (M < 2 || !xmom)) return MLSP_ERR_ARG;
    Workspace wsp(ws, ws_bytes);
    return launch_thin_in_bwd(st, dH, X, ldx, M, Cin, W, bias, C, gamma, beta, bn_save, xmom, training, act, dW, db, dgamma, dbeta, wsp);
}
int mlsp_token_pool_fwd_f32(const float* y, int B, int L, int d, float* out, int32_t* arg, mlsp_stream_t st) {
    if (!y || !out || !arg || B <= 0 || L <= 0 || d <= 0) return MLSP_ERR_ARG;
    return launch_token_pool_fwd(st, y, B, L, d, out, arg);
}
int mlsp_token_pool_bwd_f32(const float* dOut, const int32_t* arg, int B, int L, int d, float* dy, mlsp_stream_t st) {
    if (!dOut || !arg || !dy || B <= 0 || L <= 0 || d <= 0) return MLSP_ERR_ARG;
    return launch_token_pool_bwd(st, dOut, arg, B, L, d, dy);
}

int mlsp_interp3_add_fwd_f32(const float* feat, const int32_t* idx, const float* dist, const float* add, int B, int N, int S, int C, float* out,
                             mlsp_stream_t st) {
    if (!feat || !add || !out || (S != 1 && (!idx || !dist)) || B <= 0 || N <= 0 || S <= 0 || C <= 0) return MLSP_ERR_ARG;
    return launch_interp3_add_fwd(st, feat, idx, dist, add, B, N, S, C, out);
}
int mlsp_interp3_add_bwd_f32(const float* dout, const float* dist, const int32_t* rev_off, const int32_t* rev_ent, int B, int N, int S, int C,
                             float* dfeat, mlsp_stream_t st) {
    if (!dout || !dfeat || (S != 1 && (!dist || !rev_off || !rev_ent)) || B <= 0 || N <= 0 || S <= 0 || C <= 0) return MLSP_ERR_ARG;
    return launch_interp3_add_bwd(st, dout, dist, rev_off, rev_ent, B, N, S, C, dfeat);
}
int mlsp_cloud_mean_fwd_f32(const float* X, int B, int N, int C, float* out, mlsp_stream_t st) {
    if (!X || !out || B <= 0 || N <= 0 || C <= 0) return MLSP_ERR_ARG;
    return launch_cloud_mean_fwd(st, X, B, N, C, out);
}
int mlsp_cloud_mean_bwd_f32(const float* dOut, int B, int N, int C, float* dX, mlsp_stream_t st) {
    if (!dOut || !dX || B <= 0 || N <= 0 || C <= 0) return MLSP_ERR_ARG;
    return launch_cloud_mean_bwd(st, dOut, B, N, C, dX);
}

int mlsp_batch_prepare_f32(const float* raw, int ld, int B, int Nmax, const int* counts, int S, const int* flags, const int* start,
                           const double* Rpre, const double* Rpost, const double* noise, double sigma, double clip, float* out, int* idx,
                           mlsp_stream_t st) {
    return launch_batch_prepare(st, raw, ld, B, Nmax, counts, S, flags, start, Rpre, Rpost, noise, sigma, clip, out, idx);
}

}
```

### mlsp_amd/csrc/edge.hip

```cpp
#include "common.h"
#include <math.h>
#include <cstdlib>

#define EDGE_PTS_PER_WAVE 16

__global__ __launch_bounds__(256) void build_wd_kernel(const float* __restrict__ W, int Cout, int C, float* __restrict__ Wd, float* __restrict__ amax) {
    __shared__ float sm[4];
    int t = blockIdx.x * blockDim.x + threadIdx.x;
    float m = 0.f;
    if (t < Cout * C) {
        int o = t / C, c = t % C;
        float wa = W[(size_t)o * 2 * C + c], wb = W[(size_t)o * 2 * C + C + c];
        Wd[(size_t)o * C + c] = wa;
        Wd[(size_t)(Cout + o) * C + c] = wb - wa;
        m = fmaxf(fabsf(wa), fabsf(wb - wa));
    }
    if (!amax) return;
#pragma unroll
    for (int o = 1; o < 64; o <<= 1) m = fmaxf(m, __shfl_xor(m, o, 64));
    if ((threadIdx.x & 63) == 0) sm[threadIdx.x >> 6] = m;
    __syncthreads();
    if (threadIdx.x == 0) amax[blockIdx.x] = fmaxf(fmaxf(sm[0], sm[1]), fmaxf(sm[2], sm[3]));
    if (blockIdx.x == 0 && threadIdx.x >= gridDim.x) amax[threadIdx.x] = 0.f;
}
struct EvalPrep { int C; const float* gamma; const float* beta; const float* rm; const float* rv; float eps; float* save; };
__device__ __forceinline__ void eval_prep_one(const EvalPrep& e, int c) {
    const float invstd = 1.0f / sqrtf(e.rv[c] + e.eps);
    const float sc = e.gamma[c] * invstd;
    e.save[c] = sc; e.save[e.C + c] = e.beta[c] - e.rm[c] * sc; e.save[2 * e.C + c] = e.rm[c]; e.save[3 * e.C + c] = invstd;
}
__global__ void build_wd_eval_kernel(const float* __restrict__ W, int Cout, int C, float* __restrict__ Wd, EvalPrep a, EvalPrep b) {
    int t = blockIdx.x * blockDim.x + threadIdx.x;
    if (t < a.C) eval_prep_one(a, t);
    if (t < b.C) eval_prep_one(b, t);
    if (t >= Cout * C) return;
    int o = t / C, c = t % C;
    float wa = W[(size_t)o * 2 * C + c], wb = W[(size_t)o * 2 * C + C + c];
    Wd[(size_t)o * C + c] = wa;
    Wd[(size_t)(Cout + o) * C + c] = wb - wa;
}
__global__ void unbuild_wd_kernel(const float* __restrict__ dWd, int Cout, int C, float* __restrict__ dW) {
    int t = blockIdx.x * blockDim.x + threadIdx.x;
    if (t >= Cout * C) return;
    int o = t / C, c = t % C;
    float du = dWd[(size_t)o * C + c], dv = dWd[(size_t)(Cout + o) * C + c];
    dW[(size_t)o * 2 * C + c] = du - dv;
    dW[(size_t)o * 2 * C + C + c] = dv;
}

__global__ __launch_bounds__(256) void edge_reduce_kernel(const float* __restrict__ uv, const int* __restrict__ idx,
                                                          const float* __restrict__ gamma, int P, int N, int Cout, int k,
                                                          float* __restrict__ msel, uint8_t* __restrict__ argsel,
                                                          float* __restrict__ s1out, double* __restrict__ part) {
    extern __shared__ double shd[];
    const int lane = threadIdx.x & 63;
    const int w = __builtin_amdgcn_readfirstlane(threadIdx.x >> 6);
    const int ld = 2 * Cout;
    const int p0 = (blockIdx.x * 4 + w) * EDGE_PTS_PER_WAVE;
    for (int c = lane; c < Cout; c += 64) {
        const bool use_max = gamma[c] >= 0.f;
        double ps = 0.0, pq = 0.0;
        for (int pi = 0; pi < EDGE_PTS_PER_WAVE; ++pi) {
            const int i = p0 + pi;
            if (i >= P) break;
            const int base = (i / N) * N;
            const int* irow = idx + (size_t)i * k;
            float best = 0.f, s1 = 0.f, s2 = 0.f;
            int bs = 0;
            for (int s = 0; s < k; ++s) {
                const int j = base + irow[s];
                float u = uv[(size_t)j * ld + c];
                s1 += u; s2 = fmaf(u, u, s2);
                bool take = (s == 0) || (use_max ? (u > best) : (u < best));
                best = take ? u : best; bs = take ? s : bs;
            }
            float v = uv[(size_t)i * ld + Cout + c];
            msel[(size_t)i * Cout + c] = best;
            argsel[(size_t)i * Cout + c] = (uint8_t)bs;
            s1out[(size_t)i * Cout + c] = s1;
            ps += (double)s1 + (double)k * v;
            pq += (double)s2 + 2.0 * (double)v * s1 + (double)k * v * v;
        }
        shd[(0 * 4 + w) * Cout + c] = ps;
        shd[(1 * 4 + w) * Cout + c] = pq;
    }
    __syncthreads();
    for (int c = threadIdx.x; c < Cout; c += 256) {
        double a = 0.0, b = 0.0;
        for (int u = 0; u < 4; ++u) { a += shd[(0 * 4 + u) * Cout + c]; b += shd[(1 * 4 + u) * Cout + c]; }
        part[((size_t)blockIdx.x * 2 + 0) * Cout + c] = a;
        part[((size_t)blockIdx.x * 2 + 1) * Cout + c] = b;
    }
}


template <int LR>
__global__ __launch_bounds__(256) void edge_reduce_vec_kernel(const float* __restrict__ uv, const int* __restrict__ idx,
                                                              const float* __restrict__ gamma, int P, int N, int k,
                                                              float* __restrict__ msel, uint8_t* __restrict__ argsel,
                                                              float* __restrict__ s1out, double* __restrict__ part) {
    constexpr int Cout = LR * 4, NP = 64 / LR;
    __shared__ double shd[2][4][Cout];
    const int lane = threadIdx.x & 63;
    const int w = __builtin_amdgcn_readfirstlane(threadIdx.x >> 6);
    const int sub = lane / LR, c = (lane % LR) * 4;
    const int ld = 2 * Cout;
    int p0 = (blockIdx.x * 4 + w) * EDGE_PTS_PER_WAVE;
    if (N % (4 * EDGE_PTS_PER_WAVE) == 0) {
        int cloud, chunk;
        xcd_cloud_map(blockIdx.x, N / (4 * EDGE_PTS_PER_WAVE), P / N, cloud, chunk);
        p0 = cloud * N + (chunk * 4 + w) * EDGE_PTS_PER_WAVE;
    }
    const f32x4 g4 = *(const f32x4*)(gamma + c);
    bool use_max[4];
#pragma unroll
    for (int e = 0; e < 4; ++e) use_max[e] = g4[e] >= 0.f;
    double ps[4] = {0, 0, 0, 0}, pq[4] = {0, 0, 0, 0};
    for (int pi = 0; pi < EDGE_PTS_PER_WAVE; ++pi) {
        const int i = p0 + pi;
        if (i >= P) break;
        const int base = (i / N) * N;
        const int* irow = idx + (size_t)i * k;
        float best[4], s1[4] = {0, 0, 0, 0}, s2[4] = {0, 0, 0, 0};
        int bs[4];
#pragma unroll
        for (int e = 0; e < 4; ++e) { best[e] = use_max[e] ? -INFINITY : INFINITY; bs[e] = 255; }
        int jv = base;
        for (int s0 = 0; s0 < k; s0 += NP) {
            if ((s0 & 63) == 0) jv = s0 + lane < k ? base + irow[s0 + lane] : base;
            const int s = s0 + sub;
            const bool ok = s < k;
            const int j = __shfl(jv, ok ? (s & 63) : 0, 64);
            const f32x4 u = *(const f32x4*)(uv + (size_t)j * ld + c);
#pragma unroll
            for (int e = 0; e < 4; ++e) {
                const float ue = ok ? u[e] : 0.f;
                s1[e] += ue; s2[e] = fmaf(ue, ue, s2[e]);
                bool take = ok && (use_max[e] ? (u[e] > best[e]) : (u[e] < best[e]));
                best[e] = take ? u[e] : best[e]; bs[e] = take ? s : bs[e];
            }
        }
#pragma unroll
        for (int o = LR; o < 64; o <<= 1) {
#pragma unroll
            for (int e = 0; e < 4; ++e) {
                float ob = __shfl_xor(best[e], o, 64);
                int os = __shfl_xor(bs[e], o, 64);
                s1[e] += __shfl_xor(s1[e], o, 64);
                s2[e] += __shfl_xor(s2[e], o, 64);
                bool better = use_max[e] ? (ob > best[e]) : (ob < best[e]);
                bool take = better || (ob == best[e] && os < bs[e]);
                best[e] = take ? ob : best[e]; bs[e] = take ? os : bs[e];
            }
        }
        if (sub == 0) {
            const f32x4 v = *(const f32x4*)(uv + (size_t)i * ld + Cout + c);
            f32x4 b4, s4;
            uint32_t a4 = 0;
#pragma unroll
            for (int e = 0; e < 4; ++e) {
                b4[e] = best[e]; s4[e] = s1[e]; a4 |= (uint32_t)(bs[e] & 255) << (8 * e);
                ps[e] += (double)s1[e] + (double)k * v[e];
                pq[e] += (double)s2[e] + 2.0 * (double)v[e] * s1[e] + (double)k * v[e] * v[e];
            }
            *(f32x4*)(msel + (size_t)i * Cout + c) = b4;
            *(f32x4*)(s1out + (size_t)i * Cout + c) = s4;
            *(uint32_t*)(argsel + (size_t)i * Cout + c) = a4;
        }
    }
    if (sub == 0) {
#pragma unroll
        for (int e = 0; e < 4; ++e) { shd[0][w][c + e] = ps[e]; shd[1][w][c + e] = pq[e]; }
    }
    __syncthreads();
    for (int cc = threadIdx.x; cc < Cout; cc += 256) {
        part[((size_t)blockIdx.x * 2 + 0) * Cout + cc] = shd[0][0][cc] + shd[0][1][cc] + shd[0][2][cc] + shd[0][3][cc];
        part[((size_t)blockIdx.x * 2 + 1) * Cout + cc] = shd[1][0][cc] + shd[1][1][cc] + shd[1][2][cc] + shd[1][3][cc];
    }
}

#define ELDS_CS 8
template <int KMAX, bool EXACT>
__global__ __launch_bounds__(256) void edge_reduce_lds_kernel(const float* __restrict__ uv, const int* __restrict__ idx,
                                                              const float* __restrict__ gamma, int B, int N, int k, int Cout, int psplit,
                                                              float* __restrict__ msel, uint8_t* __restrict__ argsel,
                                                              float* __restrict__ s1out, double* __restrict__ part) {
    extern __shared__ __attribute__((aligned(16))) float esm[];
    constexpr int CS = ELDS_CS, QPP = CS / 4, PL = 256 / QPP;
    float* Us = esm;
    unsigned short* Is = (unsigned short*)(esm + (size_t)N * CS);
    const int tid = threadIdx.x;
    const int nsl = Cout / CS, bpc = nsl * psplit;
    int b, r;
    xcd_cloud_map(blockIdx.x, bpc, B, b, r);
    const int sl = r % nsl, ch = r / nsl;
    const int c0 = sl * CS, ld = 2 * Cout;
    const int pper = (N + psplit - 1) / psplit, pbeg = ch * pper, pend = min(N, pbeg + pper);
    const int q = tid % QPP, pl = tid / QPP;
    const float* ub = uv + (size_t)b * N * ld;
    for (int row = pl; row < N; row += PL)
        *(f32x4*)(Us + row * CS + 4 * q) = *(const f32x4*)(ub + (size_t)row * ld + c0 + 4 * q);
    const int* ib = idx + ((size_t)b * N + pbeg) * k;
    for (int t = tid; t < (pend - pbeg) * k; t += 256) Is[t] = (unsigned short)ib[t];
    __syncthreads();
    const f32x4 g4 = *(const f32x4*)(gamma + c0 + 4 * q);
    bool use_max[4];
#pragma unroll
    for (int e = 0; e < 4; ++e) use_max[e] = g4[e] >= 0.f;
    double ps[4] = {0, 0, 0, 0}, pq[4] = {0, 0, 0, 0};
    for (int il = pl; il < pend - pbeg; il += PL) {
        const unsigned short* irow = Is + il * k;
        float best[4];
        f32x2 s1a = {0.f, 0.f}, s1b = {0.f, 0.f}, s2a = {0.f, 0.f}, s2b = {0.f, 0.f};
        const f32x2 sga = {use_max[0] ? 1.f : -1.f, use_max[1] ? 1.f : -1.f}, sgb = {use_max[2] ? 1.f : -1.f, use_max[3] ? 1.f : -1.f};
        int bs[4] = {0, 0, 0, 0};
        int jr[KMAX];
#pragma unroll
        for (int s = 0; s < KMAX; ++s) jr[s] = (EXACT || s < k) ? (int)irow[s] : 0;
#pragma unroll
        for (int s = 0; s < KMAX; ++s) {
            if (EXACT || s < k) {
                const f32x4 u = *(const f32x4*)(Us + jr[s] * CS + 4 * q);
                const f32x2 ua = {u[0], u[1]}, ub = {u[2], u[3]};
                s1a += ua; s1b += ub;
                s2a = __builtin_elementwise_fma(ua, ua, s2a); s2b = __builtin_elementwise_fma(ub, ub, s2b);
                const f32x2 ta = ua * sga, tb = ub * sgb;
                const float t[4] = {ta[0], ta[1], tb[0], tb[1]};
#pragma unroll
                for (int e = 0; e < 4; ++e) {
                    const bool take = (s == 0) || (t[e] > best[e]);
                    best[e] = take ? t[e] : best[e]; bs[e] = take ? s : bs[e];
                }
            }
        }
        const float s1[4] = {s1a[0], s1a[1], s1b[0], s1b[1]}, s2[4] = {s2a[0], s2a[1], s2b[0], s2b[1]};
#pragma unroll
        for (int e = 0; e < 4; ++e) best[e] = use_max[e] ? best[e] : -best[e];
        const size_t i = (size_t)b * N + pbeg + il;
        const f32x4 v = *(const f32x4*)(uv + i * ld + Cout + c0 + 4 * q);
        f32x4 b4, s4;
        uint32_t a4 = 0;
#pragma unroll
        for (int e = 0; e < 4; ++e) {
            b4[e] = best[e]; s4[e] = s1[e]; a4 |= (uint32_t)(bs[e] & 255) << (8 * e);
            ps[e] += (double)s1[e] + (double)k * v[e];
            pq[e] += (double)s2[e] + 2.0 * (double)v[e] * s1[e] + (double)k * v[e] * v[e];
        }
        *(f32x4*)(msel + i * Cout + c0 + 4 * q) = b4;
        *(f32x4*)(s1out + i * Cout + c0 + 4 * q) = s4;
        *(uint32_t*)(argsel + i * Cout + c0 + 4 * q) = a4;
    }
    __syncthreads();
    double* red = (double*)esm;
#pragma unroll
    for (int e = 0; e < 4; ++e) { red[(0 * PL + pl) * CS + 4 * q + e] = ps[e]; red[(1 * PL + pl) * CS + 4 * q + e] = pq[e]; }
    __syncthreads();
    if (tid < 2 * CS) {
        const int which = tid / CS, c = tid % CS;
        double a = 0.0;
        for (int u = 0; u < PL; ++u) a += red[(which * PL + u) * CS + c];
        part[((size_t)(b * psplit + ch) * 2 + which) * Cout + c0 + c] = a;
    }
}

template <int KMAX, bool EXACT, int CS, int NT>
__global__ __launch_bounds__(NT, 4) void edge_reduce_wide_kernel(const float* __restrict__ uv, const int* __restrict__ idx,
                                                                const float* __restrict__ gamma, int B, int N, int k, int Cout, int psplit,
                                                                float* __restrict__ msel, uint8_t* __restrict__ argsel,
                                                                float* __restrict__ s1out, double* __restrict__ part) {
    extern __shared__ __attribute__((aligned(16))) float esm[];
    constexpr int QPP = CS / 4, PL = NT / QPP;
    float* Us = esm;
    const int tid = threadIdx.x;
    const int nsl = Cout / CS, bpc = nsl * psplit;
    int b, r;
    xcd_cloud_map(blockIdx.x, bpc, B, b, r);
    const int sl = r % nsl, ch = r / nsl;
    const int c0 = sl * CS, ld = 2 * Cout;
    const int pper = (N + psplit - 1) / psplit, pbeg = ch * pper, pend = min(N, pbeg + pper);
    const int q = tid % QPP, pl = tid / QPP;
    const float* ub = uv + (size_t)b * N * ld;
    const f32x4 g4 = *(const f32x4*)(gamma + c0 + 4 * q);
    f32x4 sg;
#pragma unroll
    for (int e = 0; e < 4; ++e) sg[e] = g4[e] >= 0.f ? 1.f : -1.f;
    for (int row = pl; row < N; row += 4 * PL) {
        f32x4 v[4];
#pragma unroll
        for (int u = 0; u < 4; ++u)
            if (row + u * PL < N) v[u] = *(const f32x4*)(ub + (size_t)(row + u * PL) * ld + c0 + 4 * q);
#pragma unroll
        for (int u = 0; u < 4; ++u)
            if (row + u * PL < N) *(f32x4*)(Us + (row + u * PL) * CS + 4 * q) = v[u] * sg;
    }
    __syncthreads();
    double ps[4] = {0, 0, 0, 0}, pq[4] = {0, 0, 0, 0};
    constexpr int KC = (KMAX % 20 == 0) ? 20 : KMAX;
    for (int il = pbeg + pl; il < pend; il += PL) {
        const size_t i = (size_t)b * N + il;
        const int* irow = idx + i * k;
        const f32x4 v = *(const f32x4*)(uv + i * ld + Cout + c0 + 4 * q);
        float best[4];
        f32x2 s1a = {0.f, 0.f}, s1b = {0.f, 0.f}, s2a = {0.f, 0.f}, s2b = {0.f, 0.f};
        int bs[4] = {0, 0, 0, 0};
#pragma unroll 1
        for (int s0 = 0; s0 < KMAX; s0 += KC) {
            int jr[KC];
            if (EXACT && (KC % 4) == 0) {
#pragma unroll
                for (int s4 = 0; s4 < KC / 4; ++s4) {
                    const int4 t = *(const int4*)(irow + s0 + 4 * s4);
                    jr[4 * s4] = t.x; jr[4 * s4 + 1] = t.y; jr[4 * s4 + 2] = t.z; jr[4 * s4 + 3] = t.w;
                }
            } else {
#pragma unroll
                for (int s = 0; s < KC; ++s) jr[s] = (EXACT || s0 + s < k) ? irow[s0 + s] : 0;
            }
#pragma unroll
            for (int s = 0; s < KC; ++s) {
                if (EXACT || s0 + s < k) {
                    const f32x4 t = *(const f32x4*)(Us + jr[s] * CS + 4 * q);
                    const f32x2 ta = {t[0], t[1]}, tb = {t[2], t[3]};
                    s1a += ta; s1b += tb;
                    s2a = __builtin_elementwise_fma(ta, ta, s2a); s2b = __builtin_elementwise_fma(tb, tb, s2b);
#pragma unroll
                    for (int e = 0; e < 4; ++e) {
                        const bool take = (s0 + s == 0) || (t[e] > best[e]);
                        best[e] = take ? t[e] : best[e]; bs[e] = take ? s0 + s : bs[e];
                    }
                }
            }
        }
        const float s1[4] = {s1a[0] * sg[0], s1a[1] * sg[1], s1b[0] * sg[2], s1b[1] * sg[3]}, s2[4] = {s2a[0], s2a[1], s2b[0], s2b[1]};
        f32x4 b4, s4;
        uint32_t a4 = 0;
#pragma unroll
        for (int e = 0; e < 4; ++e) {
            b4[e] = best[e] * sg[e]; s4[e] = s1[e]; a4 |= (uint32_t)(bs[e] & 255) << (8 * e);
            ps[e] += (double)s1[e] + (double)k * v[e];
            pq[e] += (double)s2[e] + 2.0 * (double)v[e] * s1[e] + (double)k * v[e] * v[e];
        }
        *(f32x4*)(msel + i * Cout + c0 + 4 * q) = b4;
        *(f32x4*)(s1out + i * Cout + c0 + 4 * q) = s4;
        *(uint32_t*)(argsel + i * Cout + c0 + 4 * q) = a4;
    }
    __syncthreads();
    double* red = (double*)esm;
#pragma unroll
    for (int e = 0; e < 4; ++e) { red[(0 * PL + pl) * CS + 4 * q + e] = ps[e]; red[(1 * PL + pl) * CS + 4 * q + e] = pq[e]; }
    __syncthreads();
    if (tid < 2 * CS) {
        const int which = tid / CS, c = tid % CS;
        double a = 0.0;
        for (int u = 0; u < PL; ++u) a += red[(which * PL + u) * CS + c];
        part[((size_t)(b * psplit + ch) * 2 + which) * Cout + c0 + c] = a;
    }
}

__device__ __forceinline__ void edge_amax_raise(float* __restrict__ amax, float m) {
    __shared__ float wm[4];
#pragma unroll
    for (int o = 1; o < 64; o <<= 1) m = fmaxf(m, __shfl_xor(m, o, 64));
    if ((threadIdx.x & 63) == 0) wm[threadIdx.x >> 6] = m;
    __syncthreads();
    if (threadIdx.x == 0) atomicMax((unsigned int*)amax + (blockIdx.x & 255), __float_as_uint(fmaxf(fmaxf(wm[0], wm[1]), fmaxf(wm[2], wm[3]))));
}

template <int LR>
__global__ __launch_bounds__(256) void edge_bwd_gather_vec_kernel(const float* __restrict__ gz, const uint8_t* __restrict__ argsel,
                                                                  const float* __restrict__ uv, const int* __restrict__ rev_off,
                                                                  const int* __restrict__ rev_ent, int P, int N,
                                                                  const float* __restrict__ scale, const float* __restrict__ mean,
                                                                  const float* __restrict__ invstd,
                                                                  const float* __restrict__ mean_dz,
                                                                  const float* __restrict__ mean_dzy, float* __restrict__ duv,
                                                                  float* __restrict__ duv_amax) {
    constexpr int Cout = LR * 4, NP = 64 / LR;
    const int lane = threadIdx.x & 63;
    const int w = __builtin_amdgcn_readfirstlane(threadIdx.x >> 6);
    int j = blockIdx.x * 4 + w;
    if (N % 4 == 0) {
        int cloud, chunk;
        xcd_cloud_map(blockIdx.x, N / 4, P / N, cloud, chunk);
        j = cloud * N + chunk * 4 + w;
    }
    float pm = 0.f;
    if (j < P) {
        const int sub = lane / LR, c = (lane % LR) * 4;
        const int base = (j / N) * N;
        const int e0 = rev_off[j], e1 = rev_off[j + 1];
        const int ld = 2 * Cout;
        float A[4] = {0, 0, 0, 0}, Bc[4] = {0, 0, 0, 0};
        if (mean_dz) {
#pragma unroll
            for (int e = 0; e < 4; ++e) { float sc = scale[c + e]; A[e] = sc * mean_dz[c + e]; Bc[e] = sc * invstd[c + e] * mean_dzy[c + e]; }
        }
        float acc[4] = {0, 0, 0, 0};
        for (int ec = e0; ec < e1; ec += 64) {
            const int nent = min(64, e1 - ec);
            const int entv = lane < nent ? rev_ent[ec + lane] : 0;
            for (int t0 = 0; t0 < nent; t0 += NP) {
                const int t = t0 + sub;
                const bool ok = t < nent;
                const int ent = __shfl(entv, ok ? t : 0, 64);
                const int i = base + (ent >> 8), slot = ent & 255;
                const f32x4 g = *(const f32x4*)(gz + (size_t)i * Cout + c);
                const uint32_t a4 = *(const uint32_t*)(argsel + (size_t)i * Cout + c);
                const f32x4 v = *(const f32x4*)(uv + (size_t)i * ld + Cout + c);
#pragma unroll
                for (int e = 0; e < 4; ++e) {
                    float ge = (((a4 >> (8 * e)) & 255) == (uint32_t)slot) ? g[e] : 0.f;
                    acc[e] += ok ? (ge - Bc[e] * v[e]) : 0.f;
                }
            }
        }
#pragma unroll
        for (int o = LR; o < 64; o <<= 1)
#pragma unroll
            for (int e = 0; e < 4; ++e) acc[e] += __shfl_xor(acc[e], o, 64);
        if (sub == 0) {
            const f32x4 u = *(const f32x4*)(uv + (size_t)j * ld + c);
            f32x4 o4;
#pragma unroll
            for (int e = 0; e < 4; ++e) { o4[e] = acc[e] - (float)(e1 - e0) * (A[e] + Bc[e] * (u[e] - mean[c + e])); pm = fmaxf(pm, fabsf(o4[e])); }
            *(f32x4*)(duv + (size_t)j * ld + c) = o4;
        }
    }
    if (duv_amax) edge_amax_raise(duv_amax, pm);
}

__global__ __launch_bounds__(256) void edge_select_act_kernel(const float* __restrict__ msel, const float* __restrict__ uv,
                                                              int P, int Cout, const float* __restrict__ scale,
                                                              const float* __restrict__ shift, int act, float slope,
                                                              float* __restrict__ out, int ldo) {
    size_t total = (size_t)P * Cout;
    for (size_t t = blockIdx.x * (size_t)blockDim.x + threadIdx.x; t < total; t += (size_t)gridDim.x * blockDim.x) {
        size_t i = t / Cout; int c = (int)(t % Cout);
        float y = msel[t] + uv[i * 2 * Cout + Cout + c];
        out[i * ldo + c] = lrelu_or_relu(fmaf(y, scale[c], shift[c]), act, slope);
    }
}

__global__ __launch_bounds__(256) void edge_bwd_reduce_kernel(const float* __restrict__ dOut, const float* __restrict__ out,
                                                              const float* __restrict__ msel, const float* __restrict__ uv,
                                                              int P, int Cout, const float* __restrict__ mean,
                                                              const float* __restrict__ invstd, int act, float slope,
                                                              double* __restrict__ part, int lddo, int ldo) {
    __shared__ double sh[2][4][64];
    const int lane = threadIdx.x & 63, w = threadIdx.x >> 6;
    const int c = blockIdx.x * 64 + lane;
    const int r0 = blockIdx.y * 512, r1 = min(P, r0 + 512);
    double s = 0.0, q = 0.0;
    if (c < Cout) {
        float mu = mean[c], is = invstd[c];
        for (int r = r0 + w; r < r1; r += 4) {
            size_t t = (size_t)r * Cout + c;
            float d = dOut[(size_t)r * lddo + c];
            if (act && !(out[(size_t)r * ldo + c] > 0.f)) d *= (act == 1 ? 0.f : slope);
            float yh = (msel[t] + uv[(size_t)r * 2 * Cout + Cout + c] - mu) * is;
            s += d; q += (double)d * yh;
        }
    }
    sh[0][w][lane] = s; sh[1][w][lane] = q;
    __syncthreads();
    if (w == 0 && c < Cout) {
        part[((size_t)blockIdx.y * 2 + 0) * Cout + c] = sh[0][0][lane] + sh[0][1][lane] + sh[0][2][lane] + sh[0][3][lane];
        part[((size_t)blockIdx.y * 2 + 1) * Cout + c] = sh[1][0][lane] + sh[1][1][lane] + sh[1][2][lane] + sh[1][3][lane];
    }
}

__global__ __launch_bounds__(256) void edge_bwd_point_kernel(const float* __restrict__ dOut, const float* __restrict__ out,
                                                             const float* __restrict__ uv, const float* __restrict__ s1,
                                                             int P, int Cout, int k, const float* __restrict__ scale,
                                                             const float* __restrict__ mean, const float* __restrict__ invstd,
                                                             const float* __restrict__ mean_dz,
                                                             const float* __restrict__ mean_dzy, int act, float slope,
                                                             float* __restrict__ gz, float* __restrict__ duv, int lddo, int ldo) {
    size_t total = (size_t)P * Cout;
    for (size_t t = blockIdx.x * (size_t)blockDim.x + threadIdx.x; t < total; t += (size_t)gridDim.x * blockDim.x) {
        size_t i = t / Cout; int c = (int)(t % Cout);
        float d = dOut[i * lddo + c];
        if (act && !(out[i * ldo + c] > 0.f)) d *= (act == 1 ? 0.f : slope);
        float sc = scale[c];
        float g = sc * d;
        gz[t] = g;
        float dv = g;
        if (mean_dz) {
            float A = sc * mean_dz[c], Bc = sc * invstd[c] * mean_dzy[c];
            float v = uv[i * 2 * Cout + Cout + c];
            dv = g - (float)k * A - Bc * (s1[t] + (float)k * (v - mean[c]));
        }
        duv[i * 2 * Cout + Cout + c] = dv;
    }
}


#define EVROWS 64
__global__ __launch_bounds__(256) void edge_bwd_reduce_vec_kernel(const float* __restrict__ dOut, const float* __restrict__ out,
                                                                  const float* __restrict__ msel, const float* __restrict__ uv,
                                                                  int P, int Cout, const float* __restrict__ mean,
                                                                  const float* __restrict__ invstd, int act, float slope,
                                                                  double* __restrict__ part, int lddo, int ldo,
                                                                  float* __restrict__ duv_amax) {
    __shared__ double shd[256 * 8];
    const int tid = threadIdx.x, tpr = Cout >> 2, nrg = 256 / tpr;
    if (duv_amax && blockIdx.x == 0) duv_amax[tid] = 0.f;
    const int cg = tid % tpr, rg = tid / tpr, c = cg * 4;
    double s[4] = {0, 0, 0, 0}, q[4] = {0, 0, 0, 0};
    const f32x4 mu = *(const f32x4*)(mean + c), is = *(const f32x4*)(invstd + c);
    const int r0 = blockIdx.x * EVROWS, r1 = min(P, r0 + EVROWS);
    for (int r = r0 + rg; r < r1; r += nrg) {
        const size_t t = (size_t)r * Cout + c;
        const f32x4 d4 = *(const f32x4*)(dOut + (size_t)r * lddo + c), o4 = *(const f32x4*)(out + (size_t)r * ldo + c);
        const f32x4 m4 = *(const f32x4*)(msel + t);
        const f32x4 v4 = *(const f32x4*)(uv + (size_t)r * 2 * Cout + Cout + c);
#pragma unroll
        for (int e = 0; e < 4; ++e) {
            float d = d4[e];
            if (act && !(o4[e] > 0.f)) d *= (act == 1 ? 0.f : slope);
            s[e] += d; q[e] += (double)d * ((m4[e] + v4[e] - mu[e]) * is[e]);
        }
    }
#pragma unroll
    for (int e = 0; e < 4; ++e) { shd[tid * 8 + e] = s[e]; shd[tid * 8 + 4 + e] = q[e]; }
    __syncthreads();
    if (tid < tpr) {
        double a[8] = {0, 0, 0, 0, 0, 0, 0, 0};
        for (int g = 0; g < nrg; ++g)
#pragma unroll
            for (int e = 0; e < 8; ++e) a[e] += shd[(g * tpr + tid) * 8 + e];
#pragma unroll
        for (int e = 0; e < 4; ++e) {
            part[((size_t)blockIdx.x * 2 + 0) * Cout + tid * 4 + e] = a[e];
            part[((size_t)blockIdx.x * 2 + 1) * Cout + tid * 4 + e] = a[4 + e];
        }
    }
}

__global__ __launch_bounds__(256) void edge_select_act_vec_kernel(const float* __restrict__ msel, const float* __restrict__ uv,
                                                                  size_t total4, int C4, const float* __restrict__ scale,
                                                                  const float* __restrict__ shift, int act, float slope,
                                                                  float* __restrict__ out, int ldo) {
    for (size_t v = blockIdx.x * (size_t)blockDim.x + threadIdx.x; v < total4; v += (size_t)gridDim.x * blockDim.x) {
        const size_t i = v / C4; const int c = (int)(v % C4) * 4;
        const f32x4 m = *(const f32x4*)(msel + v * 4), vv = *(const f32x4*)(uv + i * 8 * C4 + 4 * C4 + c);
        const f32x4 sc = *(const f32x4*)(scale + c), sh = *(const f32x4*)(shift + c);
        f32x4 o;
#pragma unroll
        for (int e = 0; e < 4; ++e) o[e] = lrelu_or_relu(fmaf(m[e] + vv[e], sc[e], sh[e]), act, slope);
        *(f32x4*)(out + i * ldo + c) = o;
    }
}

__global__ __launch_bounds__(256) void edge_bwd_point_vec_kernel(const float* __restrict__ dOut, const float* __restrict__ out,
                                                                 const float* __restrict__ uv, const float* __restrict__ s1,
                                                                 size_t total4, int C4, int k, const float* __restrict__ scale,
                                                                 const float* __restrict__ mean, const float* __restrict__ invstd,
                                                                 const float* __restrict__ mean_dz, const float* __restrict__ mean_dzy,
                                                                 int act, float slope, float* __restrict__ gz,
                                                                 float* __restrict__ duv, int lddo, int ldo,
                                                                 float* __restrict__ duv_amax) {
    const float fk = (float)k;
    float pm = 0.f;
    for (size_t v = blockIdx.x * (size_t)blockDim.x + threadIdx.x; v < total4; v += (size_t)gridDim.x * blockDim.x) {
        const size_t i = v / C4; const int c = (int)(v % C4) * 4;
        const f32x4 d4 = *(const f32x4*)(dOut + i * lddo + c), o4 = *(const f32x4*)(out + i * ldo + c);
        const f32x4 sc = *(const f32x4*)(scale + c);
        f32x4 g, dv;
#pragma unroll
        for (int e = 0; e < 4; ++e) {
            float d = d4[e];
            if (act && !(o4[e] > 0.f)) d *= (act == 1 ? 0.f : slope);
            g[e] = sc[e] * d; dv[e] = g[e];
        }
        if (mean_dz) {
            const f32x4 vv = *(const f32x4*)(uv + i * 8 * C4 + 4 * C4 + c), s4 = *(const f32x4*)(s1 + v * 4);
#pragma unroll
            for (int e = 0; e < 4; ++e) {
                float A = sc[e] * mean_dz[c + e], Bc = sc[e] * invstd[c + e] * mean_dzy[c + e];
                dv[e] = g[e] - fk * A - Bc * (s4[e] + fk * (vv[e] - mean[c + e]));
            }
        }
        *(f32x4*)(gz + v * 4) = g;
        *(f32x4*)(duv + i * 8 * C4 + 4 * C4 + c) = dv;
#pragma unroll
        for (int e = 0; e < 4; ++e) pm = fmaxf(pm, fabsf(dv[e]));
    }
    if (duv_amax) edge_amax_raise(duv_amax, pm);
}

__global__ __launch_bounds__(256) void edge_bwd_gather_kernel(const float* __restrict__ gz, const uint8_t* __restrict__ argsel,
                                                              const float* __restrict__ uv, const int* __restrict__ rev_off,
                                                              const int* __restrict__ rev_ent, int P, int N, int Cout,
                                                              const float* __restrict__ scale, const float* __restrict__ mean,
                                                              const float* __restrict__ invstd,
                                                              const float* __restrict__ mean_dz,
                                                              const float* __restrict__ mean_dzy, float* __restrict__ duv) {
    const int lane = threadIdx.x & 63;
    const int w = __builtin_amdgcn_readfirstlane(threadIdx.x >> 6);
    const int j = blockIdx.x * 4 + w;
    if (j >= P) return;
    const int base = (j / N) * N;
    const int e0 = rev_off[j], e1 = rev_off[j + 1];
    const int ld = 2 * Cout;
    for (int c = lane; c < Cout; c += 64) {
        float A = 0.f, Bc = 0.f;
        if (mean_dz) { float sc = scale[c]; A = sc * mean_dz[c]; Bc = sc * invstd[c] * mean_dzy[c]; }
        float acc = 0.f;
        for (int e = e0; e < e1; ++e) {
            int ent = rev_ent[e];
            int i = base + (ent >> 8), slot = ent & 255;
            size_t t = (size_t)i * Cout + c;
            float g = (argsel[t] == slot) ? gz[t] : 0.f;
            acc += g - Bc * uv[(size_t)i * ld + Cout + c];
        }
        float u = uv[(size_t)j * ld + c];
        duv[(size_t)j * ld + c] = acc - (float)(e1 - e0) * (A + Bc * (u - mean[c]));
    }
}

__global__ __launch_bounds__(256) void graph_feature_fwd_kernel(const float* __restrict__ x, const int* __restrict__ idx,
                                                                int P, int N, int C, int k, float* __restrict__ F) {
    size_t total = (size_t)P * k * C;
    for (size_t t = blockIdx.x * (size_t)blockDim.x + threadIdx.x; t < total; t += (size_t)gridDim.x * blockDim.x) {
        int c = (int)(t % C);
        size_t e = t / C;
        size_t i = e / k;
        int j = (int)(i / N) * N + idx[e];
        float xi = x[i * C + c];
        F[e * 2 * C + c] = x[(size_t)j * C + c] - xi;
        F[e * 2 * C + C + c] = xi;
    }
}

__global__ __launch_bounds__(256) void graph_feature_bwd_kernel(const float* __restrict__ dF, const int* __restrict__ rev_off,
                                                                const int* __restrict__ rev_ent, int P, int N, int C, int k,
                                                                float* __restrict__ dx) {
    size_t total = (size_t)P * C;
    for (size_t t = blockIdx.x * (size_t)blockDim.x + threadIdx.x; t < total; t += (size_t)gridDim.x * blockDim.x) {
        int c = (int)(t % C);
        size_t i = t / C;
        int base = (int)(i / N) * N;
        float acc = 0.f;
        for (int s = 0; s < k; ++s) {
            const float* r = dF + (i * k + s) * 2 * C;
            acc += r[C + c] - r[c];
        }
        for (int e = rev_off[i]; e < rev_off[i + 1]; ++e) {
            int ent = rev_ent[e];
            size_t src = (size_t)(base + (ent >> 8)) * k + (ent & 255);
            acc += dF[src * 2 * C + c];
        }
        dx[t] = acc;
    }
}

static inline int ew_blocks2(size_t total) {
    size_t b = (total + 255) / 256;
    return (int)(b < 4096 ? (b ? b : 1) : 4096);
}

int edge_bwd_reduce_parts(int P, int Cout, const void* a, const void* b, const void* c, const void* d, const void* e, const void* f,
                          int lddo, int ldo) {
    bool vec = Cout % 4 == 0 && Cout <= 1024 && 256 % (Cout / 4) == 0 && lddo % 4 == 0 && ldo % 4 == 0 &&
               ((((uintptr_t)a | (uintptr_t)b | (uintptr_t)c | (uintptr_t)d | (uintptr_t)e | (uintptr_t)f) & 15) == 0);
    return vec ? (P + EVROWS - 1) / EVROWS : (P + 511) / 512;
}
int edge_reduce_parts(int P) { return (P + 4 * EDGE_PTS_PER_WAVE - 1) / (4 * EDGE_PTS_PER_WAVE); }

bool build_wd_leaves_bound(int Cout, int C) { return (Cout * C + 255) / 256 <= 256; }
int launch_build_wd(hipStream_t st, const float* W, int Cout, int C, float* Wd, float* amax) {
    if (amax && (Cout * C + 255) / 256 > 256) return MLSP_ERR_ARG;
    hipLaunchKernelGGL(build_wd_kernel, dim3((Cout * C + 255) / 256), dim3(256), 0, st, W, Cout, C, Wd, amax);
    return mlsp_launch_status();
}
int launch_build_wd_eval(hipStream_t st, const float* W, int Cout, int C, float* Wd, int Ca, const float* ga, const float* ba, const float* rma,
                         const float* rva, float* sva, int Cb, const float* gb, const float* bb, const float* rmb, const float* rvb, float* svb,
                         float eps) {
    const EvalPrep a = {Ca, ga, ba, rma, rva, eps, sva}, b = {Cb, gb, bb, rmb, rvb, eps, svb};
    int n = Cout * C; if (Ca > n) n = Ca; if (Cb > n) n = Cb;
    hipLaunchKernelGGL(build_wd_eval_kernel, dim3((n + 255) / 256), dim3(256), 0, st, W, Cout, C, Wd, a, b);
    return mlsp_launch_status();
}
int launch_unbuild_wd(hipStream_t st, const float* dWd, int Cout, int C, float* dW) {
    hipLaunchKernelGGL(unbuild_wd_kernel, dim3((Cout * C + 255) / 256), dim3(256), 0, st, dWd, Cout, C, dW);
    return mlsp_launch_status();
}
int launch_edge_reduce(hipStream_t st, const float* uv, const int* idx, const float* gamma, int P, int N, int Cout, int k,
                       float* msel, uint8_t* argsel, float* s1, double* part, int* nparts_used) {
    const bool al = (((uintptr_t)uv | (uintptr_t)msel | (uintptr_t)s1 | (uintptr_t)gamma) & 15) == 0 && (((uintptr_t)argsel) & 3) == 0;
    if (nparts_used) *nparts_used = edge_reduce_parts(P);
    if (al && P % N == 0 && N % 4 == 0 && (k == 20 || k == 40 || k <= 32) && Cout % 32 == 0 && N <= 2048) {
        constexpr int CS = 16;
        const int B = P / N, nsl = Cout / CS;
        const int NT = N <= 1024 ? 512 : 1024;
        const int want = NT == 512 ? 512 : 256;
        int psplit = 1;
        while (psplit < 8 && B * nsl * psplit < want && N % (psplit * 2) == 0) psplit *= 2;
        const size_t lds = (size_t)N * CS * sizeof(float);
        const size_t red = (size_t)2 * (NT / (CS / 4)) * CS * sizeof(double);
        if ((lds > red ? lds : red) <= 150 * 1024 && B * psplit <= edge_reduce_parts(P)) {
            const size_t ldsz = lds > red ? lds : red;
#define EW_GO(KM, EX) do { auto kern = NT == 512 ? edge_reduce_wide_kernel<KM, EX, CS, 512> : edge_reduce_wide_kernel<KM, EX, CS, 1024>; \
                if (ldsz > 64 * 1024) { hipError_t e_ = mlsp_lds_limit((const void*)kern, ldsz); if (e_ != hipSuccess) return (int)e_; } \
                hipLaunchKernelGGL(kern, dim3(B * nsl * psplit), dim3(NT), ldsz, st, uv, idx, gamma, B, N, k, Cout, psplit, msel, argsel, s1, part); } while (0)
            if (k == 20) EW_GO(20, true); else if (k <= 20) EW_GO(20, false); else if (k <= 32) EW_GO(32, false); else EW_GO(40, true);
#undef EW_GO
            if (nparts_used) *nparts_used = B * psplit;
            return mlsp_launch_status();
        }
    }
    if (al && Cout % ELDS_CS == 0 && P % N == 0 && N <= 4096 && k <= 40 && N % 4 == 0) {
        const int B = P / N, nsl = Cout / ELDS_CS;
        int psplit = 1;
        while (psplit < 8 && (B * nsl * psplit < 512 || (N / psplit) * k * 2 > 16 * 1024) && N % (psplit * 2) == 0) psplit *= 2;
        const size_t lds = (size_t)N * ELDS_CS * sizeof(float) + align_up((size_t)((N + psplit - 1) / psplit) * k * 2, 16);
        if (lds <= 150 * 1024 && B * psplit <= edge_reduce_parts(P) && lds >= (size_t)2 * (256 / (ELDS_CS / 4)) * ELDS_CS * sizeof(double)) {
            auto kern = k == 20 ? edge_reduce_lds_kernel<20, true> : k <= 20 ? edge_reduce_lds_kernel<20, false> : k <= 32 ? edge_reduce_lds_kernel<32, false>
                      : k == 40 ? edge_reduce_lds_kernel<40, true> : edge_reduce_lds_kernel<40, false>;
            if (lds > 64 * 1024) {
                hipError_t e = mlsp_lds_limit((const void*)kern, lds);
                if (e != hipSuccess) return (int)e;
            }
            hipLaunchKernelGGL(kern, dim3(B * nsl * psplit), dim3(256), lds, st, uv, idx, gamma, B, N, k, Cout, psplit, msel, argsel, s1, part);
            if (nparts_used) *nparts_used = B * psplit;
            return mlsp_launch_status();
        }
    }
    if (al && (Cout == 64 || Cout == 128 || Cout == 256)) {
        dim3 g(edge_reduce_parts(P)), b(256);
        if (Cout == 64) hipLaunchKernelGGL((edge_reduce_vec_kernel<16>), g, b, 0, st, uv, idx, gamma, P, N, k, msel, argsel, s1, part);
        else if (Cout == 128) hipLaunchKernelGGL((edge_reduce_vec_kernel<32>), g, b, 0, st, uv, idx, gamma, P, N, k, msel, argsel, s1, part);
        else hipLaunchKernelGGL((edge_reduce_vec_kernel<64>), g, b, 0, st, uv, idx, gamma, P, N, k, msel, argsel, s1, part);
        return mlsp_launch_status();
    }
    size_t lds = (size_t)8 * Cout * sizeof(double);
    if (lds > 64 * 1024) return MLSP_ERR_UNSUPPORTED;
    hipLaunchKernelGGL(edge_reduce_kernel, dim3(edge_reduce_parts(P)), dim3(256), lds, st, uv, idx, gamma, P, N, Cout, k,
                       msel, argsel, s1, part);
    return mlsp_launch_status();
}
int launch_edge_select_act(hipStream_t st, const float* msel, const float* uv, int P, int Cout, const float* scale,
                           const float* shift, int act, float slope, float* out, int ldo) {
    if (Cout % 4 == 0 && ldo % 4 == 0 && ((((uintptr_t)msel | (uintptr_t)uv | (uintptr_t)out | (uintptr_t)scale | (uintptr_t)shift) & 15) == 0)) {
        size_t t4 = (size_t)P * Cout / 4;
        hipLaunchKernelGGL(edge_select_act_vec_kernel, dim3(ew_blocks2(t4)), dim3(256), 0, st, msel, uv, t4, Cout / 4, scale, shift,
                           act, slope, out, ldo);
        return mlsp_launch_status();
    }
    hipLaunchKernelGGL(edge_select_act_kernel, dim3(ew_blocks2((size_t)P * Cout)), dim3(256), 0, st, msel, uv, P, Cout, scale,
                       shift, act, slope, out, ldo);
    return mlsp_launch_status();
}
static bool edge_bwd_reduce_vec_ok(const float* dOut, const float* out, const float* msel, const float* uv, int Cout, const float* mean,
                                   const float* invstd, int lddo, int ldo) {
    return Cout % 4 == 0 && Cout <= 1024 && 256 % (Cout / 4) == 0 && lddo % 4 == 0 && ldo % 4 == 0 &&
           ((((uintptr_t)dOut | (uintptr_t)out | (uintptr_t)msel | (uintptr_t)uv | (uintptr_t)mean | (uintptr_t)invstd) & 15) == 0);
}
static bool edge_bwd_point_vec_ok(const float* dOut, const float* out, const float* uv, const float* s1, int Cout, const float* scale,
                                  const float* gz, const float* duv, int lddo, int ldo) {
    return Cout % 4 == 0 && lddo % 4 == 0 && ldo % 4 == 0 &&
           ((((uintptr_t)dOut | (uintptr_t)out | (uintptr_t)uv | (uintptr_t)s1 | (uintptr_t)gz | (uintptr_t)duv | (uintptr_t)scale) & 15) == 0);
}
static bool edge_bwd_gather_vec_ok(const float* gz, const uint8_t* argsel, const float* uv, int Cout, const float* duv) {
    return (((uintptr_t)uv | (uintptr_t)gz | (uintptr_t)duv) & 15) == 0 && (((uintptr_t)argsel) & 3) == 0 && (Cout == 64 || Cout == 128 || Cout == 256);
}
bool edge_bwd_leaves_duv_bound(const float* dOut, const float* out, const float* msel, const float* uv, const float* s1, const uint8_t* argsel,
                               int Cout, const float* scale, const float* mean, const float* invstd, const float* gz, const float* duv,
                               int lddo, int ldo) {
    return edge_bwd_reduce_vec_ok(dOut, out, msel, uv, Cout, mean, invstd, lddo, ldo) &&
           edge_bwd_point_vec_ok(dOut, out, uv, s1, Cout, scale, gz, duv, lddo, ldo) && edge_bwd_gather_vec_ok(gz, argsel, uv, Cout, duv);
}
int launch_edge_bwd_reduce(hipStream_t st, const float* dOut, const float* out, const float* msel, const float* uv, int P,
                           int Cout, const float* mean, const float* invstd, int act, float slope, double* part, int lddo, int ldo,
                           float* duv_amax) {
    if (edge_bwd_reduce_vec_ok(dOut, out, msel, uv, Cout, mean, invstd, lddo, ldo)) {
        hipLaunchKernelGGL(edge_bwd_reduce_vec_kernel, dim3((P + EVROWS - 1) / EVROWS), dim3(256), 0, st, dOut, out, msel, uv, P, Cout,
                           mean, invstd, act, slope, part, lddo, ldo, duv_amax);
        return mlsp_launch_status();
    }
    hipLaunchKernelGGL(edge_bwd_reduce_kernel, dim3((Cout + 63) / 64, (P + 511) / 512), dim3(256), 0, st, dOut, out, msel, uv,
                       P, Cout, mean, invstd, act, slope, part, lddo, ldo);
    return mlsp_launch_status();
}
int launch_edge_bwd_point(hipStream_t st, const float* dOut, const float* out, const float* uv, const float* s1, int P,
                          int Cout, int k, const float* scale, const float* mean, const float* invstd, const float* mean_dz,
                          const float* mean_dzy, int act, float slope, float* gz, float* duv, int lddo, int ldo, float* duv_amax) {
    if (edge_bwd_point_vec_ok(dOut, out, uv, s1, Cout, scale, gz, duv, lddo, ldo)) {
        size_t t4 = (size_t)P * Cout / 4;
        hipLaunchKernelGGL(edge_bwd_point_vec_kernel, dim3(ew_blocks2(t4)), dim3(256), 0, st, dOut, out, uv, s1, t4, Cout / 4, k, scale,
                           mean, invstd, mean_dz, mean_dzy, act, slope, gz, duv, lddo, ldo, duv_amax);
        return mlsp_launch_status();
    }
    hipLaunchKernelGGL(edge_bwd_point_kernel, dim3(ew_blocks2((size_t)P * Cout)), dim3(256), 0, st, dOut, out, uv, s1, P, Cout,
                       k, scale, mean, invstd, mean_dz, mean_dzy, act, slope, gz, duv, lddo, ldo);
    return mlsp_launch_status();
}
int launch_edge_bwd_gather(hipStream_t st, const float* gz, const uint8_t* argsel, const float* uv, const int* rev_off,
                           const int* rev_ent, int P, int N, int Cout, const float* scale, const float* mean,
                           const float* invstd, const float* mean_dz, const float* mean_dzy, float* duv, float* duv_amax) {
    if (edge_bwd_gather_vec_ok(gz, argsel, uv, Cout, duv)) {
        dim3 g((P + 3) / 4), b(256);
        if (Cout == 64) hipLaunchKernelGGL((edge_bwd_gather_vec_kernel<16>), g, b, 0, st, gz, argsel, uv, rev_off, rev_ent, P, N, scale, mean, invstd, mean_dz, mean_dzy, duv, duv_amax);
        else if (Cout == 128) hipLaunchKernelGGL((edge_bwd_gather_vec_kernel<32>), g, b, 0, st, gz, argsel, uv, rev_off, rev_ent, P, N, scale, mean, invstd, mean_dz, mean_dzy, duv, duv_amax);
        else hipLaunchKernelGGL((edge_bwd_gather_vec_kernel<64>), g, b, 0, st, gz, argsel, uv, rev_off, rev_ent, P, N, scale, mean, invstd, mean_dz, mean_dzy, duv, duv_amax);
        return mlsp_launch_status();
    }
    hipLaunchKernelGGL(edge_bwd_gather_kernel, dim3((P + 3) / 4), dim3(256), 0, st, gz, argsel, uv, rev_off, rev_ent, P, N,
                       Cout, scale, mean, invstd, mean_dz, mean_dzy, duv);
    return mlsp_launch_status();
}
int launch_graph_feature_fwd(hipStream_t st, const float* x, const int* idx, int P, int N, int C, int k, float* F) {
    hipLaunchKernelGGL(graph_feature_fwd_kernel, dim3(ew_blocks2((size_t)P * k * C)), dim3(256), 0, st, x, idx, P, N, C, k, F);
    return mlsp_launch_status();
}
int launch_graph_feature_bwd(hipStream_t st, const float* dF, const int* rev_off, const int* rev_ent, int P, int N, int C,
                             int k, float* dx) {
    hipLaunchKernelGGL(graph_feature_bwd_kernel, dim3(ew_blocks2((size_t)P * C)), dim3(256), 0, st, dF, rev_off, rev_ent, P, N,
                       C, k, dx);
    return mlsp_launch_status();
}
```

### mlsp_amd/csrc/launchers.h

```cpp
#pragma once

hipError_t mlsp_lds_limit(const void* fn, size_t lds);

int launch_slab_reduce(hipStream_t st, const float* slab, float* C, int M, int N, int ldc, int nsplit, float* unfold_dw = nullptr,
                       bool* unfolded = nullptr);
int gemm_stat_parts(const CallCtx& cx, int M, int N, int K);
int gemm_panel_rows(const CallCtx& cx, int M, int N, int K);
size_t gemm_slab_floats(int M, int N, int K);
int prof_cls_begin(hipStream_t st, int cls);
void prof_cls_end(hipStream_t st, int token, double work);
bool gemm_xf_supported(const CallCtx& cx, bool ta, bool tb, int M, int N, int K, const float* A, int lda, const float* B, int ldb, int which);
int gemm_bs_parts(const CallCtx& cx, int M, int N, int K, int lda, int ldb, int ldc);
bool gemm_dy_supported(const CallCtx& cx, bool ta, bool tb, int M, int N, int K, const float* A, int lda, const float* B, int ldb);
bool gemm_xf_on_split(const CallCtx& cx, bool ta, bool tb, int M, int N, int K, int which);
int launch_gemm(hipStream_t st, CallCtx& cx, bool ta, bool tb, int M, int N, int K, const float* A, int lda, const float* B, int ldb, float* C,
                int ldc, const GemmOpts& o = GemmOpts());
int launch_gemm_mx(hipStream_t st, CallCtx& cx, bool ta, bool tb, int M, int N, int K, const void* A, int a_bf16, int lda, const void* B, int b_bf16,
                   int ldb, void* C, int c_bf16, int ldc, const GemmOpts& o = GemmOpts());

int launch_knn(hipStream_t st, const float* x, int ld, int B, int N, int C, int k, int* idx, float* xx_ws, void* planes, size_t plane_bytes);
bool knn6_vex_supported(int B, int N, int C, int k);
bool knn6_supported(int B, int N, int C, int k);
bool knn6w_supported(int B, int N, int C, int k);

struct KnnPlan;
int launch_knn6(hipStream_t st, const KnnPlan& p, const float* x, int ld, int B, int N, int C, int k, int* idx, float* xx, void* planes,
                int** flags_out);

int launch_group_reverse(hipStream_t st, const int* idx, int B, int S, int N, int k, int* rev_off, int* rev_ent);
int launch_group_reverse_compact(hipStream_t st, const int* idx, int B, int S, int N, int k, int* rev_off, int* rev_cnt, int* rev_ent, int* pad_cnt);
int launch_knn_reverse(hipStream_t st, const int* idx, int B, int N, int k, int* rev_off, int* rev_ent);

int bn_vec_parts(int M);
int bn_stat_parts(int M);
int bn_parts_max(int M);
int launch_colstats_n(hipStream_t st, const float* Y, int M, int C, int ld, double* part, int* nparts_out);
int launch_colstats(hipStream_t st, const float* Y, int M, int C, int ld, double* part);
int launch_bn_finalize(hipStream_t st, const double* part, int nparts, double count, int C, const float* gamma, const float* beta, float* run_mean,
                       float* run_var, float momentum, float eps, float* scale, float* shift, float* save_mean, float* save_invstd,
                       float* bound_out = nullptr);
int launch_bn_finalize_groups(hipStream_t st, const double* part, int nparts, double count, int C, const float* gamma, const float* beta,
                              float* run_mean, float* run_var, float momentum, float eps, float* scale, float* shift, float* save_mean,
                              float* save_invstd, float* gsum, int ppg);
int launch_bn_eval_prepare(hipStream_t st, int C, const float* gamma, const float* beta, const float* run_mean, const float* run_var, float eps,
                           float* scale, float* shift, float* save_mean, float* save_invstd);
int launch_bn_act_fwd(hipStream_t st, const float* Y, float* Z, size_t rows, int C, const float* scale, const float* shift, int act, float slope,
                      float p_drop, uint64_t seed);
int launch_bn_act_bwd(hipStream_t st, const float* dZ, const float* Y, float* dY, int M, int C, const float* scale, const float* shift,
                      const float* mean, const float* invstd, int training, int act, float slope, float p_drop, uint64_t seed, double* part,
                      float* dgamma, float* dbeta, float* mean_dz, float* mean_dzy, float* zero_vec, float* gpart = nullptr,
                      int rows_per_group = 0, int* gpart_slabs = nullptr, const double* pre_stats = nullptr, int pre_parts = 0);
int launch_bn_bwd_finalize_coef_z(hipStream_t st, const double* part, int nparts, double count, int C, const float* bn_save, float* dgamma,
                                  float* dbeta, float* coef, float* zero_vec);
int launch_bn_bwd_finalize_coef_groups(hipStream_t st, const double* part, int nparts, double count, int C, const float* bn_save, float* dgamma,
                                       float* dbeta, float* coef, const float* gys, int ppg, int rows, float* gout);
int launch_bn_bwd_finalize_z(hipStream_t st, const double* part, int nparts, double count, int C, float* dgamma, float* dbeta, float* mean_dz,
                             float* mean_dzy, float* zero_vec);
int launch_bn_bwd_finalize(hipStream_t st, const double* part, int nparts, double count, int C, float* dgamma, float* dbeta, float* mean_dz,
                           float* mean_dzy);
int launch_colsum_groups(hipStream_t st, const float* X, int G, int rows_per_group, int C, float* out, float* scratch = nullptr);
int launch_bn_dy_gbias(hipStream_t st, const float* Y, int G, int rows_per_group, int C, const double* stats, int panel_rows, const float* coef,
                       float* scratch, float* out, const float* ysum);
int launch_colsum_groups_fin(hipStream_t st, const float* scratch, int G, int C, int slabs, float* out);
int launch_colsum(hipStream_t st, const float* X, int M, int C, double* part, float* out);
int launch_bn_act_bwd_partials_vec(hipStream_t st, const float* dZ, const float* Y, int M, int C, const float* scale, const float* shift,
                                   const float* mean, const float* invstd, int act, float slope, double* part);
int launch_colmax_fwd(hipStream_t st, const float* Z, int B, int N, int C, float* out, int* arg);
int launch_colmax_bwd(hipStream_t st, const float* dOut, const int* arg, int B, int N, int C, float* dZ);
int launch_segmax_fwd(hipStream_t st, const float* Z, int P, int k, int C, float* out, uint8_t* argk);
int launch_segsel_act_fwd(hipStream_t st, const float* Y, int G, int k, int C, const float* scale, const float* shift, int act, float slope,
                          float* out, float* ysel, uint8_t* argk);
int launch_segsel_bwd_apply(hipStream_t st, const float* dOut, const float* Y, const float* ysel, const uint8_t* argk, size_t M, int k, int C,
                            const float* bn, const float* m1, const float* m2, int act, float slope, float* dY);
int launch_segmax_bwd(hipStream_t st, const float* dOut, const uint8_t* argk, int P, int k, int C, float* dZ);
int launch_bn_act_fwd_b16(hipStream_t st, const void* Y, void* Z, int rows, int C, const float* scale, const float* shift, int act, float slope,
                          float p_drop, uint64_t seed);
int launch_bn_act_bwd_b16(hipStream_t st, const void* dZ, const void* Y, void* dY, int M, int C, const float* scale, const float* shift,
                          const float* mean, const float* invstd, int training, int act, float slope, float p_drop, uint64_t seed, double* part,
                          float* dgamma, float* dbeta, float* mean_dz, float* mean_dzy, float* zero_vec);
int launch_colsum_groups_b16(hipStream_t st, const void* X, int G, int rows_per_group, int C, float* out, float* scratch);

int edge_bwd_reduce_parts(int P, int Cout, const void* a, const void* b, const void* c, const void* d, const void* e, const void* f, int lddo,
                          int ldo);
int edge_reduce_parts(int P);
bool build_wd_leaves_bound(int Cout, int C);
int launch_build_wd(hipStream_t st, const float* W, int Cout, int C, float* Wd, float* amax = nullptr);
int launch_build_wd_eval(hipStream_t st, const float* W, int Cout, int C, float* Wd, int Ca, const float* ga, const float* ba, const float* rma,
                         const float* rva, float* sva, int Cb, const float* gb, const float* bb, const float* rmb, const float* rvb, float* svb,
                         float eps);
int launch_unbuild_wd(hipStream_t st, const float* dWd, int Cout, int C, float* dW);
int launch_edge_reduce(hipStream_t st, const float* uv, const int* idx, const float* gamma, int P, int N, int Cout, int k, float* msel,
                       uint8_t* argsel, float* s1, double* part, int* nparts_used);
int launch_edge_select_act(hipStream_t st, const float* msel, const float* uv, int P, int Cout, const float* scale, const float* shift, int act,
                           float slope, float* out, int ldo);
bool edge_bwd_leaves_duv_bound(const float* dOut, const float* out, const float* msel, const float* uv, const float* s1, const uint8_t* argsel,
                               int Cout, const float* scale, const float* mean, const float* invstd, const float* gz, const float* duv, int lddo,
                               int ldo);
int launch_edge_bwd_reduce(hipStream_t st, const float* dOut, const float* out, const float* msel, const float* uv, int P, int Cout,
                           const float* mean, const float* invstd, int act, float slope, double* part, int lddo, int ldo, float* duv_amax);
int launch_edge_bwd_point(hipStream_t st, const float* dOut, const float* out, const float* uv, const float* s1, int P, int Cout, int k,
                          const float* scale, const float* mean, const float* invstd, const float* mean_dz, const float* mean_dzy, int act,
                          float slope, float* gz, float* duv, int lddo, int ldo, float* duv_amax);
int launch_edge_bwd_gather(hipStream_t st, const float* gz, const uint8_t* argsel, const float* uv, const int* rev_off, const int* rev_ent, int P,
                           int N, int Cout, const float* scale, const float* mean, const float* invstd, const float* mean_dz, const float* mean_dzy,
                           float* duv, float* duv_amax);
int launch_graph_feature_fwd(hipStream_t st, const float* x, const int* idx, int P, int N, int C, int k, float* F);
int launch_graph_feature_bwd(hipStream_t st, const float* dF, const int* rev_off, const int* rev_ent, int P, int N, int C, int k, float* dx);

int launch_chamfer_fwd(hipStream_t st, const float* pred, const float* gold, const float* mask, int B, int N, float scale, float* per_cloud,
                       int* argA, int* argB, float* loss);
int launch_chamfer_bwd(hipStream_t st, const float* pred, const float* gold, const float* mask, int B, int N, float scale, const float* per_cloud,
                       const int* argA, const int* argB, const float* gout, float* dpred);
int launch_chamfer_dir_fwd(hipStream_t st, const float* p1, const float* p2, const float* mc, int B, int N, float* per_cloud, int* arg, float* loss);
int launch_chamfer_dir_bwd(hipStream_t st, const float* p1, const float* p2, const float* mc, int B, int N, const float* per_cloud, const int* arg,
                           const float* gout, float* dp1, float* dp2);
int launch_normal_loss_fwd(hipStream_t st, const float* pred, const float* gt, const float* w, int P, float weight, double* part, float* out);
int launch_normal_loss_bwd(hipStream_t st, const float* pred, const float* gt, const float* w, int P, float weight, const float* fwd_out,
                           const float* gout, float* dpred);
int launch_density_tail_fwd(hipStream_t st, const float* logits, const float* w, int P, int nc, float* pvec, float* dens);
int launch_density_tail_bwd(hipStream_t st, const float* pvec, const float* w, const float* dp, const float* dd, int P, int nc, float* dlogits);
int launch_density_loss_fwd(hipStream_t st, const float* pvec, const float* dens, const float* tvec, const float* target, const float* m, int P,
                            int nc, float dweight, double* part, float* out);
int launch_density_loss_bwd(hipStream_t st, const float* pvec, const float* dens, const float* tvec, const float* target, const float* m, int P,
                            int nc, float dweight, const float* fwd_out, const float* gkl, const float* gmae, float* dp, float* dd);

int tnet_grid(int ntiles);
int tnet_points_per_tile(int k);
int tnet_fwd_parts(int B, int N, int k);
int launch_tnet_edge_fwd(hipStream_t st, int mode, const float* uv, const int* idx, const float* bn1, const float* W2, const float* gamma2, int P, int N, int k,
                         float slope, float* zsel, uint8_t* argsel, double* part);
int launch_tnet_out(hipStream_t st, const float* zsel, const float* bn2, int P, float slope, float* out);
int launch_tnet_bwd_reduce(hipStream_t st, const float* dT, const float* T, const float* zsel, const float* bn2, int P, float slope, double* part);
int launch_tnet_bwd_g(hipStream_t st, const float* dT, const float* T, const float* bn2, const float* mean_dz, const float* mean_dzy, int P,
                      float slope, float* g, float* coef);
size_t tnet_bwd_scratch_floats(int ntiles);
int launch_tnet_edge_bwd(hipStream_t st, int mode, const float* uv, const int* idx, const float* bn1, const float* W2, const float* bn2, const float* g,
                         const uint8_t* argsel, const float* coef, int P, int N, int k, float slope, float* dhp, float* scratch, double* part1,
                         float* dW2, int* nparts);
int launch_tnet_edge_bwd2(hipStream_t st, const float* dhp, const float* uv, const float* s1, const float* bn1, const float* m1, const float* m2,
                          const int* rev_off, const int* rev_ent, int P, int N, int k, float* duv);
size_t tnet_w1_moment_doubles(int P, int k);
int launch_tnet_bwd_w1_moments(hipStream_t st, const float* dhp, const int* idx, const int* rev_off, const float* x, int ldx, const float* W1,
                               const float* bn1, const float* m1, const float* m2, int P, int N, int k, int C, double* scratch, float* dW1);

int launch_colsel(hipStream_t st, const float* Y, const float* gamma, int B, int N, int C, float* ysel, int* arg);
int launch_colsel_panels(hipStream_t st, const float* pv, const int* pr, const float* gamma, int B, int N, int C, int panel_rows, float* ysel,
                         int* arg, const float* bn, int act, float slope, float* out);
int launch_colsel_out(hipStream_t st, const float* ysel, const float* bn, int B, int C, int act, float slope, float* out);
int launch_colmax_bwd_coef(hipStream_t st, const float* dOut, const float* out, const float* ysel, const float* bn, int B, int C, double count,
                           int act, float slope, int training, float* g, float* coef, float* dgamma, float* dbeta);
int launch_wt_vec_neg_scale_rows(hipStream_t st, const float* W, int ldw, const float* v, const float* rowscale, int Cout, int Cin, float* negr,
                                 float* Wb);
int launch_colmax_gather_rows(hipStream_t st, const float* g, const int* arg, const float* X, int ldx, int B, int N, int Cout, int Cin, float* S);
int launch_colmax_dw(hipStream_t st, const float* S, const float* WG, const float* sx, const float* coef, const float* bn, int Cout, int Cin,
                     float* dW);
int launch_colmax_scatter_rows(hipStream_t st, const float* g, const int* arg, const float* W, int ldw, int B, int N, int Cout, int Cin, float* dX,
                               int lddx);

int launch_radius_count(hipStream_t st, const float* x, int ld, int B, int N, float radius, int max_nn, int* count);
int launch_knn_normals(hipStream_t st, const float* x, int ld, const int* idx, int B, int N, int k, float* normals);

int launch_skinny_bwd_pair(hipStream_t st, const float* G, int ldg, const float* W, int ldw, const float* X, int ldx, float* dX, int lddx, float* dW,
                           int M, int Cin, int Cout, int dx_accumulate = 0);
int launch_skinny_gemm(hipStream_t st, bool ta, bool tb, int M, int N, int K, const float* A, int lda, const float* B, int ldb, float* C, int ldc,
                       const float* bias);
int launch_skinny_linear_bn_act(hipStream_t st, const float* X, int ldx, int M, int Cin, const float* W, int ldw, int Cout, const float* bias,
                                const float* gamma, const float* beta, float* run_mean, float* run_var, float momentum, float eps, int training,
                                int act, float slope, float p_drop, uint64_t seed, float* Y, float* Z, float* bn_save);
int launch_skinny_bn_bwd_z(hipStream_t st, const float* dZ, const float* Y, float* dY, int M, int C, const float* bn_save, int training, int act,
                           float slope, float p_drop, uint64_t seed, float* dgamma, float* dbeta, float* zero_vec);
int launch_compose_fwd(hipStream_t st, const float* Wa, const float* ba, const float* Wb, const float* bb, int Cm, int Ci, int Co, float* W,
                       float* b);
int launch_compose_bwd(hipStream_t st, const float* dW, const float* db, const float* Wa, const float* ba, const float* Wb, int Cm, int Ci, int Co,
                       float* dWa, float* dba, float* dWb);

int launch_fps(hipStream_t st, const float* xyz, int ldx, int B, int N, int S, const int* start, int* out);
int launch_ball_query(hipStream_t st, const float* xyz, int ldx, const float* q, int ldq, int B, int N, int S, float r2, int nsample, int* idx);
int launch_sa_group_fwd(hipStream_t st, const float* xyz, int ldx, const float* feat, int D, const float* q, int ldq, const int* idx, int B, int N,
                        int S, int ns, float* G);
int launch_sa_group_bwd(hipStream_t st, const float* dG, int ldg, int col, int D, const int* rev_off, const int* rev_ent, int B, int N, int S, int ns,
                        float* dfeat);
int launch_knn_query(hipStream_t st, const float* ref, int ldr, int Nr, const float* qry, int ldq, int Nq, int B, int C, int k, int* idx,
                     float* dist);
int launch_interp3_fwd(hipStream_t st, const float* feat, const int* idx, const float* dist, int B, int N, int S, int D, float* out);
int launch_interp3_bwd(hipStream_t st, const float* dout, const float* dist, const int* rev_off, const int* rev_ent, int B, int N, int S, int D,
                       float* dfeat);
int sa_fold_parts(long E);
int launch_sa_fold_fwd(hipStream_t st, const float* u, const float* w, const int* idx, int B, int N, int S, int ns, int C, const float* gamma,
                       const float* beta, float* run_mean, float* run_var, float momentum, float eps, int training, float* Z, float* bn_save,
                       double* part);
int launch_sa_fold_bwd(hipStream_t st, const float* dZ, const float* u, const float* w, const int* idx, const int* rev_off, const int* rev_ent, int B,
                       int N, int S, int ns, int C, const float* bn_save, int training, float* du, float* dw, float* dgamma, float* dbeta,
                       double* part, float* mean_dz, float* mean_dzy, const int* rev_cnt, const int* pad_cnt);

int launch_collapse_to_point(hipStream_t st, float* X, int B, int N, const int* choice, const float* u, const float* noise, float r2, int min_pts,
                             float* mask, int* chosen);
int launch_scan_select(hipStream_t st, const float* X, int B, int N, int C, const double* R, int pixel, float* Xs, float* mask);
int launch_region_assign(hipStream_t st, const float* X, int B, int C, int N, const float* thr, int n, float clip, int* Y);
int launch_deform_regions(hipStream_t st, float* X, int B, int C, int N, const int* regions, const int* order, int nreg, const float* lookup,
                          const float* noise, int min_pts, int groups, float* mask);
int launch_transform3_fwd(hipStream_t st, const float* x, const float* T, int B, int N, float* out);
int launch_transform3_bwd(hipStream_t st, const float* x, const float* T, const float* dout, int B, int N, float* dx, float* dT);

size_t thin_tn_slab_floats(int M, int N, int K);
int thin_bs_parts(int M, int N, int K);
int launch_thin_gemm(hipStream_t st, bool ta, bool tb, int M, int N, int K, const float* A, int lda, const float* B, int ldb, float* C, int ldc,
                     const GemmOpts& o);
bool thin_xf_supported(bool ta, bool tb, int M, int N, int K, const float* A, int lda, const float* B, int ldb, int which);

int launch_xf_materialize(hipStream_t st, const float* X, int ldx, int M, int C, const GemmXf& xf, float* out);

int launch_def_nearest(hipStream_t st, const float* pred, const float* gold, const float* mask, int B, int N, int64_t* index1, int64_t* index2);
int launch_def_normal_fwd(hipStream_t st, const float* pred, const float* lab, const float* mask, const int64_t* index1, const int64_t* index2, int B,
                          int N, int defpart, float weight, double* part, float* out);
int launch_def_normal_bwd(hipStream_t st, const float* pred, const float* lab, const float* mask, const int64_t* index1, const int64_t* index2, int B,
                          int N, int defpart, float weight, const float* fwd_out, const float* gout, float* dpred);
int launch_def_density_fwd(hipStream_t st, const float* pvec, const float* dens, const float* lvec, const float* lval, const float* mask,
                           const int64_t* index1, const int64_t* index2, int B, int N, int nc, int defpart, float dweight, double* part, float* out);
int launch_def_density_bwd(hipStream_t st, const float* pvec, const float* dens, const float* lvec, const float* lval, const float* mask,
                           const int64_t* index1, const int64_t* index2, int B, int N, int nc, int defpart, float dweight, const float* fwd_out,
                           const float* gkl, const float* gmae, float* dp, float* dd);
int launch_def_gather(hipStream_t st, const uint32_t* x, const int64_t* index, int B, int N, int W, uint32_t* out);
int launch_def_gather_bwd(hipStream_t st, const float* dout, const int64_t* index, int B, int N, int C, float* dx);

size_t vecattn_delta_bwd_ws_floats(int B, int N, int k, int d);
int launch_vecattn_delta_fwd(hipStream_t st, const float* xyz, int ldx, const int* idx, const float* Wd1, const float* bd1, int B, int N, int k,
                             int d, float* H1);
int launch_vecattn_delta_bwd(hipStream_t st, const float* dH1, const float* H1, const float* xyz, int ldx, const int* idx, int B, int N, int k,
                             int d, float* part, float* dWd1, float* dbd1);
int launch_vecattn_mix_fwd(hipStream_t st, const float* q, int ldq, const float* kk, int ldk, const float* pos, const int* idx, int B, int N, int k,
                           int d, float* T);
int launch_vecattn_mix_bwd(hipStream_t st, const float* dT, int B, int N, int k, int d, float* dq);
int launch_vecattn_aggregate_fwd(hipStream_t st, const float* A, const float* v, int ldv, const float* pos, const int* idx, int B, int N, int k,
                                 int d, float* attn, float* res);
int launch_vecattn_aggregate_bwd(hipStream_t st, const float* dres, const float* attn, const float* v, int ldv, const float* pos, const int* idx,
                                 int B, int N, int k, int d, float* dVP, float* dA);
int launch_vecattn_relu_fwd(hipStream_t st, const float* x, long long rows, int d, float* y);
int launch_vecattn_relu_bwd(hipStream_t st, const float* dy, const float* y, long long rows, int d, float* dx);


int launch_mhsa_fwd(hipStream_t st, const float* qkv, int ld, int B, int L, int H, int dh, float scale, float* out, float* lse);
int launch_mhsa_bwd(hipStream_t st, const float* qkv, int ld, const float* lse, const float* dout, int B, int L, int H, int dh, float scale,
                    float* dqkv, int ldd);
int launch_layernorm_fwd(hipStream_t st, const float* x, const float* a, const float* s, int rows_per_sample, const float* gamma, const float* beta,
                         long long rows, int d, float eps, float* u, float* y, float* mean, float* rstd);
size_t layernorm_bwd_ws_floats(long long rows, int d);
int launch_layernorm_bwd(hipStream_t st, const float* dy, const float* du, const float* u, const float* s, int rows_per_sample, const float* gamma,
                         const float* mean, const float* rstd, long long rows, int d, float* dx, float* da, float* part, float* dgamma,
                         float* dbeta);
int launch_gelu_fwd(hipStream_t st, const float* x, long long rows, int d, float* y);
int launch_gelu_bwd(hipStream_t st, const float* dy, const float* x, long long rows, int d, float* dx);

size_t gn_edge_ws_bytes(int B, int Nk, int Nq, int k, int C, int groups);
int launch_gn_edge_fwd(hipStream_t st, const float* u, int ldu, const float* w, int ldw, const int* idx, const float* gamma, const float* beta,
                       int B, int Nk, int Nq, int k, int C, int groups, float eps, float slope, float* out, uint8_t* argk, float* stats,
                       Workspace& ws);
int launch_gn_edge_bwd(hipStream_t st, const float* dOut, const float* u, int ldu, const float* w, int ldw, const int* idx, const uint8_t* argk,
                       const float* stats, const int* rev_off, const int* rev_ent, const float* gamma, const float* beta, int B, int Nk, int Nq,
                       int k, int C, int groups, float slope, float* du, float* dw, float* dgamma, float* dbeta, Workspace& ws);

size_t thin_in_ws_bytes(int M, int Cin, int C);
int launch_thin_in_fwd(hipStream_t st, const float* X, int ldx, int M, int Cin, const float* W, const float* bias, int C, const float* gamma,
                       const float* beta, float* run_mean, float* run_var, float momentum, float eps, int training, int act, float* H,
                       float* bn_save, double* xmom, Workspace& ws);
int launch_thin_in_bwd(hipStream_t st, const float* dH, const float* X, int ldx, int M, int Cin, const float* W, const float* bias, int C,
                       const float* gamma, const float* beta, const float* bn_save, const double* xmom, int training, int act, float* dW,
                       float* db, float* dgamma, float* dbeta, Workspace& ws);
int launch_token_pool_fwd(hipStream_t st, const float* y, int B, int L, int d, float* out, int* arg);
int launch_token_pool_bwd(hipStream_t st, const float* dOut, const int* arg, int B, int L, int d, float* dy);

int launch_interp3_add_fwd(hipStream_t st, const float* feat, const int* idx, const float* dist, const float* add, int B, int N, int S, int C,
                           float* out);
int launch_interp3_add_bwd(hipStream_t st, const float* dout, const float* dist, const int* rev_off, const int* rev_ent, int B, int N, int S,
                           int C, float* dfeat);
int launch_cloud_mean_fwd(hipStream_t st, const float* X, int B, int N, int C, float* out);
int launch_cloud_mean_bwd(hipStream_t st, const float* dOut, int B, int N, int C, float* dX);

int launch_batch_prepare(hipStream_t st, const float* raw, int ld, int B, int Nmax, const int* counts, int S, const int* flags, const int* start,
                         const double* Rpre, const double* Rpost, const double* noise, double sigma, double clip, float* out, int* idx);
```

Measured before the change: 8.521 million points/s.

## Store pre-activation y in edge reduce and fuse edge backward point pass into reduce/gather

The edge-reduce kernels now write the selected max plus the centre term (y = best + v) directly, so select-act and the backward reduce no longer re-read the v half of uv. In backward, the edge_bwd_reduce kernel also writes gz, and the gather kernel computes the dv half of duv from s1 and uv. Together these replace the separate edge_bwd_point launch. The T-net forward skips writing msel/argsel entirely. The aim is fewer kernel launches and less global memory traffic in the EdgeConv layers, at the cost of heavier gather and reduce kernels and an extra template variant.

```diff
diff --git a/mlsp_amd/csrc/api.hip b/mlsp_amd/csrc/api.hip
--- a/mlsp_amd/csrc/api.hip
+++ b/mlsp_amd/csrc/api.hip
@@ -211,7 +211,7 @@
         CHECK(launch_bn_finalize(st, part, nparts, (double)P * k, Cout, gamma, beta, run_mean, run_var, momentum, eps, scale,
                                  shift, mean, invstd, cx.offered_output(out, P, Cout, ldo, Cout)));
     }
-    CHECK(launch_edge_select_act(st, msel, uv, P, Cout, scale, shift, act, slope, out, ldo));
+    CHECK(launch_edge_select_act(st, msel, P, Cout, scale, shift, act, slope, out, ldo));
     return MLSP_OK;
 }
 
@@ -239,14 +239,16 @@
     GemmOpts so; take_slab(w, so, gemm_slab_floats(P, C, 2 * Cout), gemm_slab_floats(2 * Cout, C, P));
     if (!w.ok()) return MLSP_ERR_WORKSPACE;
     const float* scale = bn_save, *mean = bn_save + 2 * Cout, *invstd = bn_save + 3 * Cout;
-    float* duv_amax = (C % 128 == 0 && edge_bwd_leaves_duv_bound(dOut, out, msel, uv, s1, argsel, Cout, scale, mean, invstd, gz, duv, lddo, ldo))
-                          ? cx.reserve(duv, P, 2 * Cout, 2 * Cout) : nullptr;
-    CHECK(launch_edge_bwd_reduce(st, dOut, out, msel, uv, P, Cout, mean, invstd, act, slope, part, lddo, ldo, duv_amax));
-    CHECK(launch_bn_bwd_finalize(st, part, edge_bwd_reduce_parts(P, Cout, dOut, out, msel, uv, mean, invstd, lddo, ldo), (double)P * k, Cout,
+    const bool fused = edge_bwd_leaves_duv_bound(dOut, out, msel, uv, s1, argsel, Cout, scale, mean, invstd, gz, duv, lddo, ldo);
+    float* duv_amax = (C % 128 == 0 && fused) ? cx.reserve(duv, P, 2 * Cout, 2 * Cout) : nullptr;
+    CHECK(launch_edge_bwd_reduce(st, dOut, out, msel, P, Cout, scale, mean, invstd, act, slope, part, lddo, ldo, fused ? gz : nullptr, duv_amax));
+    CHECK(launch_bn_bwd_finalize(st, part, edge_bwd_reduce_parts(P, Cout, dOut, out, msel, mean, invstd, lddo, ldo), (double)P * k, Cout,
                                  dgamma, dbeta, mean_dz, mean_dzy));
     const float* mdz = training ? mean_dz : nullptr;
-    CHECK(launch_edge_bwd_point(st, dOut, out, uv, s1, P, Cout, k, scale, mean, invstd, mdz, mean_dzy, act, slope, gz, duv, lddo, ldo, duv_amax));
-    CHECK(launch_edge_bwd_gather(st, gz, argsel, uv, rev_off, rev_ent, P, N, Cout, scale, mean, invstd, mdz, mean_dzy, duv, duv_amax));
+    if (!fused)
+        CHECK(launch_edge_bwd_point(st, dOut, out, uv, s1, P, Cout, k, scale, mean, invstd, mdz, mean_dzy, act, slope, gz, duv, lddo, ldo, duv_amax));
+    CHECK(launch_edge_bwd_gather(st, gz, argsel, uv, fused ? s1 : nullptr, k, rev_off, rev_ent, P, N, Cout, scale, mean, invstd, mdz, mean_dzy,
+                                 duv, duv_amax));
     const float* Wdc = Wd_in;
     if (!Wdc && dx) { CHECK(launch_build_wd(st, W, Cout, C, Wd)); Wdc = Wd; }
     GemmOpts od = so; od.accumulate = dx_accumulate != 0;
@@ -273,8 +275,6 @@
     const int P = B * N;
     Workspace w(ws, ws_bytes);
     float* Wd = w.take<float>((size_t)2 * C1 * C);
-    float* msel = w.take<float>((size_t)P * C1);
-    uint8_t* arg1 = w.take<uint8_t>((size_t)P * C1);
     int np1 = edge_reduce_parts(P), np2 = tnet_fwd_parts(B, N, k);
     double* part = w.take<double>((size_t)(np1 > np2 ? np1 : np2) * 2 * C2);
     GemmOpts so; take_slab(w, so, gemm_slab_floats(P, 2 * C1, C));
@@ -284,7 +284,7 @@
         CHECK(launch_build_wd_eval(st, W1, C1, C, Wd, C1, gamma1, beta1, run_mean1, run_var1, bn1_save, C2, gamma2, beta2, run_mean2, run_var2, bn2_save, eps));
     } else CHECK(launch_build_wd(st, W1, C1, C, Wd));
     CHECK(launch_gemm(st, cx, false, true, P, 2 * C1, C, x, ldx, Wd, C, uv, 2 * C1, so));
-    CHECK(launch_edge_reduce(st, uv, idx, gamma1, P, N, C1, k, msel, arg1, s1, part, &np1));
+    CHECK(launch_edge_reduce(st, uv, idx, gamma1, P, N, C1, k, nullptr, nullptr, s1, part, &np1));
     if (training) {
         CHECK(launch_bn_finalize(st, part, np1, (double)P * k, C1, gamma1, beta1, run_mean1, run_var1, momentum, eps, bn1_save,
                                  bn1_save + C1, bn1_save + 2 * C1, bn1_save + 3 * C1));
diff --git a/mlsp_amd/csrc/edge.hip b/mlsp_amd/csrc/edge.hip
--- a/mlsp_amd/csrc/edge.hip
+++ b/mlsp_amd/csrc/edge.hip
@@ -50,7 +50,7 @@
 
 __global__ __launch_bounds__(256) void edge_reduce_kernel(const float* __restrict__ uv, const int* __restrict__ idx,
                                                           const float* __restrict__ gamma, int P, int N, int Cout, int k,
-                                                          float* __restrict__ msel, uint8_t* __restrict__ argsel,
+                                                          float* __restrict__ ysel, uint8_t* __restrict__ argsel,
                                                           float* __restrict__ s1out, double* __restrict__ part) {
     extern __shared__ double shd[];
     const int lane = threadIdx.x & 63;
@@ -75,8 +75,10 @@
                 best = take ? u : best; bs = take ? s : bs;
             }
             float v = uv[(size_t)i * ld + Cout + c];
-            msel[(size_t)i * Cout + c] = best;
-            argsel[(size_t)i * Cout + c] = (uint8_t)bs;
+            if (ysel) {
+                ysel[(size_t)i * Cout + c] = best + v;
+                argsel[(size_t)i * Cout + c] = (uint8_t)bs;
+            }
             s1out[(size_t)i * Cout + c] = s1;
             ps += (double)s1 + (double)k * v;
             pq += (double)s2 + 2.0 * (double)v * s1 + (double)k * v * v;
@@ -97,7 +99,7 @@
 template <int LR>
 __global__ __launch_bounds__(256) void edge_reduce_vec_kernel(const float* __restrict__ uv, const int* __restrict__ idx,
                                                               const float* __restrict__ gamma, int P, int N, int k,
-                                                              float* __restrict__ msel, uint8_t* __restrict__ argsel,
+                                                              float* __restrict__ ysel, uint8_t* __restrict__ argsel,
                                                               float* __restrict__ s1out, double* __restrict__ part) {
     constexpr int Cout = LR * 4, NP = 64 / LR;
     __shared__ double shd[2][4][Cout];
@@ -159,13 +161,15 @@
             uint32_t a4 = 0;
 #pragma unroll
             for (int e = 0; e < 4; ++e) {
-                b4[e] = best[e]; s4[e] = s1[e]; a4 |= (uint32_t)(bs[e] & 255) << (8 * e);
+                b4[e] = best[e] + v[e]; s4[e] = s1[e]; a4 |= (uint32_t)(bs[e] & 255) << (8 * e);
                 ps[e] += (double)s1[e] + (double)k * v[e];
                 pq[e] += (double)s2[e] + 2.0 * (double)v[e] * s1[e] + (double)k * v[e] * v[e];
             }
-            *(f32x4*)(msel + (size_t)i * Cout + c) = b4;
             *(f32x4*)(s1out + (size_t)i * Cout + c) = s4;
-            *(uint32_t*)(argsel + (size_t)i * Cout + c) = a4;
+            if (ysel) {
+                *(f32x4*)(ysel + (size_t)i * Cout + c) = b4;
+                *(uint32_t*)(argsel + (size_t)i * Cout + c) = a4;
+            }
         }
     }
     if (sub == 0) {
@@ -180,10 +184,10 @@
 }
 
 #define ELDS_CS 8
-template <int KMAX, bool EXACT>
+template <int KMAX, bool EXACT, bool SEL>
 __global__ __launch_bounds__(256) void edge_reduce_lds_kernel(const float* __restrict__ uv, const int* __restrict__ idx,
                                                               const float* __restrict__ gamma, int B, int N, int k, int Cout, int psplit,
-                                                              float* __restrict__ msel, uint8_t* __restrict__ argsel,
+                                                              float* __restrict__ ysel, uint8_t* __restrict__ argsel,
                                                               float* __restrict__ s1out, double* __restrict__ part) {
     extern __shared__ __attribute__((aligned(16))) float esm[];
     constexpr int CS = ELDS_CS, QPP = CS / 4, PL = 256 / QPP;
@@ -242,13 +246,15 @@
         uint32_t a4 = 0;
 #pragma unroll
         for (int e = 0; e < 4; ++e) {
-            b4[e] = best[e]; s4[e] = s1[e]; a4 |= (uint32_t)(bs[e] & 255) << (8 * e);
+            b4[e] = best[e] + v[e]; s4[e] = s1[e]; a4 |= (uint32_t)(bs[e] & 255) << (8 * e);
             ps[e] += (double)s1[e] + (double)k * v[e];
             pq[e] += (double)s2[e] + 2.0 * (double)v[e] * s1[e] + (double)k * v[e] * v[e];
         }
-        *(f32x4*)(msel + i * Cout + c0 + 4 * q) = b4;
         *(f32x4*)(s1out + i * Cout + c0 + 4 * q) = s4;
-        *(uint32_t*)(argsel + i * Cout + c0 + 4 * q) = a4;
+        if (SEL) {
+            *(f32x4*)(ysel + i * Cout + c0 + 4 * q) = b4;
+            *(uint32_t*)(argsel + i * Cout + c0 + 4 * q) = a4;
+        }
     }
     __syncthreads();
     double* red = (double*)esm;
@@ -263,15 +269,16 @@
     }
 }
 
-template <int KMAX, bool EXACT, int CS, int NT>
+template <int KMAX, bool EXACT, int CS, int NT, bool SEL>
 __global__ __launch_bounds__(NT, 4) void edge_reduce_wide_kernel(const float* __restrict__ uv, const int* __restrict__ idx,
                                                                 const float* __restrict__ gamma, int B, int N, int k, int Cout, int psplit,
-                                                                float* __restrict__ msel, uint8_t* __restrict__ argsel,
+                                                                float* __restrict__ ysel, uint8_t* __restrict__ argsel,
                                                                 float* __restrict__ s1out, double* __restrict__ part) {
     extern __shared__ __attribute__((aligned(16))) float esm[];
     constexpr int QPP = CS / 4, PL = NT / QPP;
     float* Us = esm;
     const int tid = threadIdx.x;
+    const int wv = __builtin_amdgcn_readfirstlane(tid >> 6);
     const int nsl = Cout / CS, bpc = nsl * psplit;
     int b, r;
     xcd_cloud_map(blockIdx.x, bpc, B, b, r);
@@ -336,21 +343,24 @@
         uint32_t a4 = 0;
 #pragma unroll
         for (int e = 0; e < 4; ++e) {
-            b4[e] = best[e] * sg[e]; s4[e] = s1[e]; a4 |= (uint32_t)(bs[e] & 255) << (8 * e);
+            b4[e] = best[e] * sg[e] + v[e]; s4[e] = s1[e]; a4 |= (uint32_t)(bs[e] & 255) << (8 * e);
             ps[e] += (double)s1[e] + (double)k * v[e];
             pq[e] += (double)s2[e] + 2.0 * (double)v[e] * s1[e] + (double)k * v[e] * v[e];
         }
-        *(f32x4*)(msel + i * Cout + c0 + 4 * q) = b4;
         *(f32x4*)(s1out + i * Cout + c0 + 4 * q) = s4;
-        *(uint32_t*)(argsel + i * Cout + c0 + 4 * q) = a4;
+        if (SEL) {
+            *(f32x4*)(ysel + i * Cout + c0 + 4 * q) = b4;
+            *(uint32_t*)(argsel + i * Cout + c0 + 4 * q) = a4;
+        }
     }
     __syncthreads();
     double* red = (double*)esm;
-#pragma unroll
-    for (int e = 0; e < 4; ++e) { red[(0 * PL + pl) * CS + 4 * q + e] = ps[e]; red[(1 * PL + pl) * CS + 4 * q + e] = pq[e]; }
-    __syncthreads();
-    if (tid < 2 * CS) {
-        const int which = tid / CS, c = tid % CS;
+    const int t2 = wv * 64 + (int)__builtin_amdgcn_mbcnt_hi(~0u, __builtin_amdgcn_mbcnt_lo(~0u, 0u));
+#pragma unroll
+    for (int e = 0; e < 4; ++e) { red[4 * t2 + e] = ps[e]; red[PL * CS + 4 * t2 + e] = pq[e]; }
+    __syncthreads();
+    if (t2 < 2 * CS) {
+        const int which = t2 / CS, c = t2 % CS;
         double a = 0.0;
         for (int u = 0; u < PL; ++u) a += red[(which * PL + u) * CS + c];
         part[((size_t)(b * psplit + ch) * 2 + which) * Cout + c0 + c] = a;
@@ -366,9 +376,14 @@
     if (threadIdx.x == 0) atomicMax((unsigned int*)amax + (blockIdx.x & 255), __float_as_uint(fmaxf(fmaxf(wm[0], wm[1]), fmaxf(wm[2], wm[3]))));
 }
 
-template <int LR>
+__device__ __forceinline__ float edge_dv(float g, float A, float Bc, float s1, float fk, float v, float mean) {
+    return g - fk * A - Bc * (s1 + fk * (v - mean));
+}
+
+template <int LR, bool DV>
 __global__ __launch_bounds__(256) void edge_bwd_gather_vec_kernel(const float* __restrict__ gz, const uint8_t* __restrict__ argsel,
-                                                                  const float* __restrict__ uv, const int* __restrict__ rev_off,
+                                                                  const float* __restrict__ uv, const float* __restrict__ s1, int k,
+                                                                  const int* __restrict__ rev_off,
                                                                   const int* __restrict__ rev_ent, int P, int N,
                                                                   const float* __restrict__ scale, const float* __restrict__ mean,
                                                                   const float* __restrict__ invstd,
@@ -395,6 +410,14 @@
 #pragma unroll
             for (int e = 0; e < 4; ++e) { float sc = scale[c + e]; A[e] = sc * mean_dz[c + e]; Bc[e] = sc * invstd[c + e] * mean_dzy[c + e]; }
         }
+        f32x4 u = {0.f, 0.f, 0.f, 0.f}, gj = u, sj = u, vj = u;
+        if (sub == 0) {
+            u = *(const f32x4*)(uv + (size_t)j * ld + c);
+            if (DV) {
+                gj = *(const f32x4*)(gz + (size_t)j * Cout + c);
+                if (mean_dz) { sj = *(const f32x4*)(s1 + (size_t)j * Cout + c); vj = *(const f32x4*)(uv + (size_t)j * ld + Cout + c); }
+            }
+        }
         float acc[4] = {0, 0, 0, 0};
         for (int ec = e0; ec < e1; ec += 64) {
             const int nent = min(64, e1 - ec);
@@ -419,30 +442,39 @@
 #pragma unroll
             for (int e = 0; e < 4; ++e) acc[e] += __shfl_xor(acc[e], o, 64);
         if (sub == 0) {
-            const f32x4 u = *(const f32x4*)(uv + (size_t)j * ld + c);
             f32x4 o4;
 #pragma unroll
             for (int e = 0; e < 4; ++e) { o4[e] = acc[e] - (float)(e1 - e0) * (A[e] + Bc[e] * (u[e] - mean[c + e])); pm = fmaxf(pm, fabsf(o4[e])); }
             *(f32x4*)(duv + (size_t)j * ld + c) = o4;
+            if (DV) {
+                f32x4 dv = gj;
+                if (mean_dz) {
+                    const float fk = (float)k;
+#pragma unroll
+                    for (int e = 0; e < 4; ++e) dv[e] = edge_dv(gj[e], A[e], Bc[e], sj[e], fk, vj[e], mean[c + e]);
+                }
+#pragma unroll
+                for (int e = 0; e < 4; ++e) pm = fmaxf(pm, fabsf(dv[e]));
+                *(f32x4*)(duv + (size_t)j * ld + Cout + c) = dv;
+            }
         }
     }
     if (duv_amax) edge_amax_raise(duv_amax, pm);
 }
 
-__global__ __launch_bounds__(256) void edge_select_act_kernel(const float* __restrict__ msel, const float* __restrict__ uv,
+__global__ __launch_bounds__(256) void edge_select_act_kernel(const float* __restrict__ ysel,
                                                               int P, int Cout, const float* __restrict__ scale,
                                                               const float* __restrict__ shift, int act, float slope,
                                                               float* __restrict__ out, int ldo) {
     size_t total = (size_t)P * Cout;
     for (size_t t = blockIdx.x * (size_t)blockDim.x + threadIdx.x; t < total; t += (size_t)gridDim.x * blockDim.x) {
         size_t i = t / Cout; int c = (int)(t % Cout);
-        float y = msel[t] + uv[i * 2 * Cout + Cout + c];
-        out[i * ldo + c] = lrelu_or_relu(fmaf(y, scale[c], shift[c]), act, slope);
+        out[i * ldo + c] = lrelu_or_relu(fmaf(ysel[t], scale[c], shift[c]), act, slope);
     }
 }
 
 __global__ __launch_bounds__(256) void edge_bwd_reduce_kernel(const float* __restrict__ dOut, const float* __restrict__ out,
-                                                              const float* __restrict__ msel, const float* __restrict__ uv,
+                                                              const float* __restrict__ ysel,
                                                               int P, int Cout, const float* __restrict__ mean,
                                                               const float* __restrict__ invstd, int act, float slope,
                                                               double* __restrict__ part, int lddo, int ldo) {
@@ -457,7 +489,7 @@
             size_t t = (size_t)r * Cout + c;
             float d = dOut[(size_t)r * lddo + c];
             if (act && !(out[(size_t)r * ldo + c] > 0.f)) d *= (act == 1 ? 0.f : slope);
-            float yh = (msel[t] + uv[(size_t)r * 2 * Cout + Cout + c] - mu) * is;
+            float yh = (ysel[t] - mu) * is;
             s += d; q += (double)d * yh;
         }
     }
@@ -497,29 +529,34 @@
 
 #define EVROWS 64
 __global__ __launch_bounds__(256) void edge_bwd_reduce_vec_kernel(const float* __restrict__ dOut, const float* __restrict__ out,
-                                                                  const float* __restrict__ msel, const float* __restrict__ uv,
-                                                                  int P, int Cout, const float* __restrict__ mean,
+                                                                  const float* __restrict__ ysel,
+                                                                  int P, int Cout, const float* __restrict__ scale,
+                                                                  const float* __restrict__ mean,
                                                                   const float* __restrict__ invstd, int act, float slope,
                                                                   double* __restrict__ part, int lddo, int ldo,
-                                                                  float* __restrict__ duv_amax) {
+                                                                  float* __restrict__ gz, float* __restrict__ duv_amax) {
     __shared__ double shd[256 * 8];
     const int tid = threadIdx.x, tpr = Cout >> 2, nrg = 256 / tpr;
     if (duv_amax && blockIdx.x == 0) duv_amax[tid] = 0.f;
     const int cg = tid % tpr, rg = tid / tpr, c = cg * 4;
     double s[4] = {0, 0, 0, 0}, q[4] = {0, 0, 0, 0};
     const f32x4 mu = *(const f32x4*)(mean + c), is = *(const f32x4*)(invstd + c);
+    f32x4 sc = {0.f, 0.f, 0.f, 0.f};
+    if (gz) sc = *(const f32x4*)(scale + c);
     const int r0 = blockIdx.x * EVROWS, r1 = min(P, r0 + EVROWS);
     for (int r = r0 + rg; r < r1; r += nrg) {
         const size_t t = (size_t)r * Cout + c;
         const f32x4 d4 = *(const f32x4*)(dOut + (size_t)r * lddo + c), o4 = *(const f32x4*)(out + (size_t)r * ldo + c);
-        const f32x4 m4 = *(const f32x4*)(msel + t);
-        const f32x4 v4 = *(const f32x4*)(uv + (size_t)r * 2 * Cout + Cout + c);
+        const f32x4 y4 = *(const f32x4*)(ysel + t);
+        f32x4 g4;
 #pragma unroll
         for (int e = 0; e < 4; ++e) {
             float d = d4[e];
             if (act && !(o4[e] > 0.f)) d *= (act == 1 ? 0.f : slope);
-            s[e] += d; q[e] += (double)d * ((m4[e] + v4[e] - mu[e]) * is[e]);
-        }
+            s[e] += d; q[e] += (double)d * ((y4[e] - mu[e]) * is[e]);
+            g4[e] = sc[e] * d;
+        }
+        if (gz) *(f32x4*)(gz + t) = g4;
     }
 #pragma unroll
     for (int e = 0; e < 4; ++e) { shd[tid * 8 + e] = s[e]; shd[tid * 8 + 4 + e] = q[e]; }
@@ -537,17 +574,17 @@
     }
 }
 
-__global__ __launch_bounds__(256) void edge_select_act_vec_kernel(const float* __restrict__ msel, const float* __restrict__ uv,
+__global__ __launch_bounds__(256) void edge_select_act_vec_kernel(const float* __restrict__ ysel,
                                                                   size_t total4, int C4, const float* __restrict__ scale,
                                                                   const float* __restrict__ shift, int act, float slope,
                                                                   float* __restrict__ out, int ldo) {
     for (size_t v = blockIdx.x * (size_t)blockDim.x + threadIdx.x; v < total4; v += (size_t)gridDim.x * blockDim.x) {
         const size_t i = v / C4; const int c = (int)(v % C4) * 4;
-        const f32x4 m = *(const f32x4*)(msel + v * 4), vv = *(const f32x4*)(uv + i * 8 * C4 + 4 * C4 + c);
+        const f32x4 y = *(const f32x4*)(ysel + v * 4);
         const f32x4 sc = *(const f32x4*)(scale + c), sh = *(const f32x4*)(shift + c);
         f32x4 o;
 #pragma unroll
-        for (int e = 0; e < 4; ++e) o[e] = lrelu_or_relu(fmaf(m[e] + vv[e], sc[e], sh[e]), act, slope);
+        for (int e = 0; e < 4; ++e) o[e] = lrelu_or_relu(fmaf(y[e], sc[e], sh[e]), act, slope);
         *(f32x4*)(out + i * ldo + c) = o;
     }
 }
@@ -578,7 +615,7 @@
 #pragma unroll
             for (int e = 0; e < 4; ++e) {
                 float A = sc[e] * mean_dz[c + e], Bc = sc[e] * invstd[c + e] * mean_dzy[c + e];
-                dv[e] = g[e] - fk * A - Bc * (s4[e] + fk * (vv[e] - mean[c + e]));
+                dv[e] = edge_dv(g[e], A, Bc, s4[e], fk, vv[e], mean[c + e]);
             }
         }
         *(f32x4*)(gz + v * 4) = g;
@@ -660,10 +697,9 @@
     return (int)(b < 4096 ? (b ? b : 1) : 4096);
 }
 
-int edge_bwd_reduce_parts(int P, int Cout, const void* a, const void* b, const void* c, const void* d, const void* e, const void* f,
-                          int lddo, int ldo) {
+int edge_bwd_reduce_parts(int P, int Cout, const void* a, const void* b, const void* c, const void* d, const void* e, int lddo, int ldo) {
     bool vec = Cout % 4 == 0 && Cout <= 1024 && 256 % (Cout / 4) == 0 && lddo % 4 == 0 && ldo % 4 == 0 &&
-               ((((uintptr_t)a | (uintptr_t)b | (uintptr_t)c | (uintptr_t)d | (uintptr_t)e | (uintptr_t)f) & 15) == 0);
+               ((((uintptr_t)a | (uintptr_t)b | (uintptr_t)c | (uintptr_t)d | (uintptr_t)e) & 15) == 0);
     return vec ? (P + EVROWS - 1) / EVROWS : (P + 511) / 512;
 }
 int edge_reduce_parts(int P) { return (P + 4 * EDGE_PTS_PER_WAVE - 1) / (4 * EDGE_PTS_PER_WAVE); }
@@ -687,8 +723,9 @@
     return mlsp_launch_status();
 }
 int launch_edge_reduce(hipStream_t st, const float* uv, const int* idx, const float* gamma, int P, int N, int Cout, int k,
-                       float* msel, uint8_t* argsel, float* s1, double* part, int* nparts_used) {
-    const bool al = (((uintptr_t)uv | (uintptr_t)msel | (uintptr_t)s1 | (uintptr_t)gamma) & 15) == 0 && (((uintptr_t)argsel) & 3) == 0;
+                       float* ysel, uint8_t* argsel, float* s1, double* part, int* nparts_used) {
+    if (!ysel != !argsel) return MLSP_ERR_ARG;
+    const bool al = (((uintptr_t)uv | (uintptr_t)ysel | (uintptr_t)s1 | (uintptr_t)gamma) & 15) == 0 && (((uintptr_t)argsel) & 3) == 0;
     if (nparts_used) *nparts_used = edge_reduce_parts(P);
     if (al && P % N == 0 && N % 4 == 0 && (k == 20 || k == 40 || k <= 32) && Cout % 32 == 0 && N <= 2048) {
         constexpr int CS = 16;
@@ -701,9 +738,10 @@
         const size_t red = (size_t)2 * (NT / (CS / 4)) * CS * sizeof(double);
         if ((lds > red ? lds : red) <= 150 * 1024 && B * psplit <= edge_reduce_parts(P)) {
             const size_t ldsz = lds > red ? lds : red;
-#define EW_GO(KM, EX) do { auto kern = NT == 512 ? edge_reduce_wide_kernel<KM, EX, CS, 512> : edge_reduce_wide_kernel<KM, EX, CS, 1024>; \
+#define EW_GO(KM, EX) do { auto kern = NT == 512 ? (ysel ? edge_reduce_wide_kernel<KM, EX, CS, 512, true> : edge_reduce_wide_kernel<KM, EX, CS, 512, false>) \
+                                                  : (ysel ? edge_reduce_wide_kernel<KM, EX, CS, 1024, true> : edge_reduce_wide_kernel<KM, EX, CS, 1024, false>); \
                 if (ldsz > 64 * 1024) { hipError_t e_ = mlsp_lds_limit((const void*)kern, ldsz); if (e_ != hipSuccess) return (int)e_; } \
-                hipLaunchKernelGGL(kern, dim3(B * nsl * psplit), dim3(NT), ldsz, st, uv, idx, gamma, B, N, k, Cout, psplit, msel, argsel, s1, part); } while (0)
+                hipLaunchKernelGGL(kern, dim3(B * nsl * psplit), dim3(NT), ldsz, st, uv, idx, gamma, B, N, k, Cout, psplit, ysel, argsel, s1, part); } while (0)
             if (k == 20) EW_GO(20, true); else if (k <= 20) EW_GO(20, false); else if (k <= 32) EW_GO(32, false); else EW_GO(40, true);
 #undef EW_GO
             if (nparts_used) *nparts_used = B * psplit;
@@ -716,46 +754,48 @@
         while (psplit < 8 && (B * nsl * psplit < 512 || (N / psplit) * k * 2 > 16 * 1024) && N % (psplit * 2) == 0) psplit *= 2;
         const size_t lds = (size_t)N * ELDS_CS * sizeof(float) + align_up((size_t)((N + psplit - 1) / psplit) * k * 2, 16);
         if (lds <= 150 * 1024 && B * psplit <= edge_reduce_parts(P) && lds >= (size_t)2 * (256 / (ELDS_CS / 4)) * ELDS_CS * sizeof(double)) {
-            auto kern = k == 20 ? edge_reduce_lds_kernel<20, true> : k <= 20 ? edge_reduce_lds_kernel<20, false> : k <= 32 ? edge_reduce_lds_kernel<32, false>
-                      : k == 40 ? edge_reduce_lds_kernel<40, true> : edge_reduce_lds_kernel<40, false>;
+#define EL_PICK(S) (k == 20 ? edge_reduce_lds_kernel<20, true, S> : k <= 20 ? edge_reduce_lds_kernel<20, false, S> : k <= 32 ? edge_reduce_lds_kernel<32, false, S> \
+                    : k == 40 ? edge_reduce_lds_kernel<40, true, S> : edge_reduce_lds_kernel<40, false, S>)
+            auto kern = ysel ? EL_PICK(true) : EL_PICK(false);
+#undef EL_PICK
             if (lds > 64 * 1024) {
                 hipError_t e = mlsp_lds_limit((const void*)kern, lds);
                 if (e != hipSuccess) return (int)e;
             }
-            hipLaunchKernelGGL(kern, dim3(B * nsl * psplit), dim3(256), lds, st, uv, idx, gamma, B, N, k, Cout, psplit, msel, argsel, s1, part);
+            hipLaunchKernelGGL(kern, dim3(B * nsl * psplit), dim3(256), lds, st, uv, idx, gamma, B, N, k, Cout, psplit, ysel, argsel, s1, part);
             if (nparts_used) *nparts_used = B * psplit;
             return mlsp_launch_status();
         }
     }
     if (al && (Cout == 64 || Cout == 128 || Cout == 256)) {
         dim3 g(edge_reduce_parts(P)), b(256);
-        if (Cout == 64) hipLaunchKernelGGL((edge_reduce_vec_kernel<16>), g, b, 0, st, uv, idx, gamma, P, N, k, msel, argsel, s1, part);
-        else if (Cout == 128) hipLaunchKernelGGL((edge_reduce_vec_kernel<32>), g, b, 0, st, uv, idx, gamma, P, N, k, msel, argsel, s1, part);
-        else hipLaunchKernelGGL((edge_reduce_vec_kernel<64>), g, b, 0, st, uv, idx, gamma, P, N, k, msel, argsel, s1, part);
+        if (Cout == 64) hipLaunchKernelGGL((edge_reduce_vec_kernel<16>), g, b, 0, st, uv, idx, gamma, P, N, k, ysel, argsel, s1, part);
+        else if (Cout == 128) hipLaunchKernelGGL((edge_reduce_vec_kernel<32>), g, b, 0, st, uv, idx, gamma, P, N, k, ysel, argsel, s1, part);
+        else hipLaunchKernelGGL((edge_reduce_vec_kernel<64>), g, b, 0, st, uv, idx, gamma, P, N, k, ysel, argsel, s1, part);
         return mlsp_launch_status();
     }
     size_t lds = (size_t)8 * Cout * sizeof(double);
     if (lds > 64 * 1024) return MLSP_ERR_UNSUPPORTED;
     hipLaunchKernelGGL(edge_reduce_kernel, dim3(edge_reduce_parts(P)), dim3(256), lds, st, uv, idx, gamma, P, N, Cout, k,
-                       msel, argsel, s1, part);
-    return mlsp_launch_status();
-}
-int launch_edge_select_act(hipStream_t st, const float* msel, const float* uv, int P, int Cout, const float* scale,
+                       ysel, argsel, s1, part);
+    return mlsp_launch_status();
+}
+int launch_edge_select_act(hipStream_t st, const float* ysel, int P, int Cout, const float* scale,
                            const float* shift, int act, float slope, float* out, int ldo) {
-    if (Cout % 4 == 0 && ldo % 4 == 0 && ((((uintptr_t)msel | (uintptr_t)uv | (uintptr_t)out | (uintptr_t)scale | (uintptr_t)shift) & 15) == 0)) {
+    if (Cout % 4 == 0 && ldo % 4 == 0 && ((((uintptr_t)ysel | (uintptr_t)out | (uintptr_t)scale | (uintptr_t)shift) & 15) == 0)) {
         size_t t4 = (size_t)P * Cout / 4;
-        hipLaunchKernelGGL(edge_select_act_vec_kernel, dim3(ew_blocks2(t4)), dim3(256), 0, st, msel, uv, t4, Cout / 4, scale, shift,
+        hipLaunchKernelGGL(edge_select_act_vec_kernel, dim3(ew_blocks2(t4)), dim3(256), 0, st, ysel, t4, Cout / 4, scale, shift,
                            act, slope, out, ldo);
         return mlsp_launch_status();
     }
-    hipLaunchKernelGGL(edge_select_act_kernel, dim3(ew_blocks2((size_t)P * Cout)), dim3(256), 0, st, msel, uv, P, Cout, scale,
+    hipLaunchKernelGGL(edge_select_act_kernel, dim3(ew_blocks2((size_t)P * Cout)), dim3(256), 0, st, ysel, P, Cout, scale,
                        shift, act, slope, out, ldo);
     return mlsp_launch_status();
 }
-static bool edge_bwd_reduce_vec_ok(const float* dOut, const float* out, const float* msel, const float* uv, int Cout, const float* mean,
+static bool edge_bwd_reduce_vec_ok(const float* dOut, const float* out, const float* ysel, int Cout, const float* mean,
                                    const float* invstd, int lddo, int ldo) {
     return Cout % 4 == 0 && Cout <= 1024 && 256 % (Cout / 4) == 0 && lddo % 4 == 0 && ldo % 4 == 0 &&
-           ((((uintptr_t)dOut | (uintptr_t)out | (uintptr_t)msel | (uintptr_t)uv | (uintptr_t)mean | (uintptr_t)invstd) & 15) == 0);
+           ((((uintptr_t)dOut | (uintptr_t)out | (uintptr_t)ysel | (uintptr_t)mean | (uintptr_t)invstd) & 15) == 0);
 }
 static bool edge_bwd_point_vec_ok(const float* dOut, const float* out, const float* uv, const float* s1, int Cout, const float* scale,
                                   const float* gz, const float* duv, int lddo, int ldo) {
@@ -765,21 +805,22 @@
 static bool edge_bwd_gather_vec_ok(const float* gz, const uint8_t* argsel, const float* uv, int Cout, const float* duv) {
     return (((uintptr_t)uv | (uintptr_t)gz | (uintptr_t)duv) & 15) == 0 && (((uintptr_t)argsel) & 3) == 0 && (Cout == 64 || Cout == 128 || Cout == 256);
 }
-bool edge_bwd_leaves_duv_bound(const float* dOut, const float* out, const float* msel, const float* uv, const float* s1, const uint8_t* argsel,
+bool edge_bwd_leaves_duv_bound(const float* dOut, const float* out, const float* ysel, const float* uv, const float* s1, const uint8_t* argsel,
                                int Cout, const float* scale, const float* mean, const float* invstd, const float* gz, const float* duv,
                                int lddo, int ldo) {
-    return edge_bwd_reduce_vec_ok(dOut, out, msel, uv, Cout, mean, invstd, lddo, ldo) &&
+    return edge_bwd_reduce_vec_ok(dOut, out, ysel, Cout, mean, invstd, lddo, ldo) &&
            edge_bwd_point_vec_ok(dOut, out, uv, s1, Cout, scale, gz, duv, lddo, ldo) && edge_bwd_gather_vec_ok(gz, argsel, uv, Cout, duv);
 }
-int launch_edge_bwd_reduce(hipStream_t st, const float* dOut, const float* out, const float* msel, const float* uv, int P,
-                           int Cout, const float* mean, const float* invstd, int act, float slope, double* part, int lddo, int ldo,
-                           float* duv_amax) {
-    if (edge_bwd_reduce_vec_ok(dOut, out, msel, uv, Cout, mean, invstd, lddo, ldo)) {
-        hipLaunchKernelGGL(edge_bwd_reduce_vec_kernel, dim3((P + EVROWS - 1) / EVROWS), dim3(256), 0, st, dOut, out, msel, uv, P, Cout,
-                           mean, invstd, act, slope, part, lddo, ldo, duv_amax);
+int launch_edge_bwd_reduce(hipStream_t st, const float* dOut, const float* out, const float* ysel, int P,
+                           int Cout, const float* scale, const float* mean, const float* invstd, int act, float slope, double* part, int lddo,
+                           int ldo, float* gz, float* duv_amax) {
+    if (edge_bwd_reduce_vec_ok(dOut, out, ysel, Cout, mean, invstd, lddo, ldo)) {
+        hipLaunchKernelGGL(edge_bwd_reduce_vec_kernel, dim3((P + EVROWS - 1) / EVROWS), dim3(256), 0, st, dOut, out, ysel, P, Cout,
+                           scale, mean, invstd, act, slope, part, lddo, ldo, gz, duv_amax);
         return mlsp_launch_status();
     }
-    hipLaunchKernelGGL(edge_bwd_reduce_kernel, dim3((Cout + 63) / 64, (P + 511) / 512), dim3(256), 0, st, dOut, out, msel, uv,
+    if (gz) return MLSP_ERR_ARG;
+    hipLaunchKernelGGL(edge_bwd_reduce_kernel, dim3((Cout + 63) / 64, (P + 511) / 512), dim3(256), 0, st, dOut, out, ysel,
                        P, Cout, mean, invstd, act, slope, part, lddo, ldo);
     return mlsp_launch_status();
 }
@@ -796,16 +837,18 @@
                        k, scale, mean, invstd, mean_dz, mean_dzy, act, slope, gz, duv, lddo, ldo);
     return mlsp_launch_status();
 }
-int launch_edge_bwd_gather(hipStream_t st, const float* gz, const uint8_t* argsel, const float* uv, const int* rev_off,
-                           const int* rev_ent, int P, int N, int Cout, const float* scale, const float* mean,
+int launch_edge_bwd_gather(hipStream_t st, const float* gz, const uint8_t* argsel, const float* uv, const float* s1, int k,
+                           const int* rev_off, const int* rev_ent, int P, int N, int Cout, const float* scale, const float* mean,
                            const float* invstd, const float* mean_dz, const float* mean_dzy, float* duv, float* duv_amax) {
     if (edge_bwd_gather_vec_ok(gz, argsel, uv, Cout, duv)) {
         dim3 g((P + 3) / 4), b(256);
-        if (Cout == 64) hipLaunchKernelGGL((edge_bwd_gather_vec_kernel<16>), g, b, 0, st, gz, argsel, uv, rev_off, rev_ent, P, N, scale, mean, invstd, mean_dz, mean_dzy, duv, duv_amax);
-        else if (Cout == 128) hipLaunchKernelGGL((edge_bwd_gather_vec_kernel<32>), g, b, 0, st, gz, argsel, uv, rev_off, rev_ent, P, N, scale, mean, invstd, mean_dz, mean_dzy, duv, duv_amax);
-        else hipLaunchKernelGGL((edge_bwd_gather_vec_kernel<64>), g, b, 0, st, gz, argsel, uv, rev_off, rev_ent, P, N, scale, mean, invstd, mean_dz, mean_dzy, duv, duv_amax);
+#define EG_GO(LR) do { if (s1) hipLaunchKernelGGL((edge_bwd_gather_vec_kernel<LR, true>), g, b, 0, st, gz, argsel, uv, s1, k, rev_off, rev_ent, P, N, scale, mean, invstd, mean_dz, mean_dzy, duv, duv_amax); \
+                       else hipLaunchKernelGGL((edge_bwd_gather_vec_kernel<LR, false>), g, b, 0, st, gz, argsel, uv, s1, k, rev_off, rev_ent, P, N, scale, mean, invstd, mean_dz, mean_dzy, duv, duv_amax); } while (0)
+        if (Cout == 64) EG_GO(16); else if (Cout == 128) EG_GO(32); else EG_GO(64);
+#undef EG_GO
         return mlsp_launch_status();
     }
+    if (s1) return MLSP_ERR_ARG;
     hipLaunchKernelGGL(edge_bwd_gather_kernel, dim3((P + 3) / 4), dim3(256), 0, st, gz, argsel, uv, rev_off, rev_ent, P, N,
                        Cout, scale, mean, invstd, mean_dz, mean_dzy, duv);
     return mlsp_launch_status();
diff --git a/mlsp_amd/csrc/launchers.h b/mlsp_amd/csrc/launchers.h
--- a/mlsp_amd/csrc/launchers.h
+++ b/mlsp_amd/csrc/launchers.h
@@ -80,8 +80,7 @@
                           float* dgamma, float* dbeta, float* mean_dz, float* mean_dzy, float* zero_vec);
 int launch_colsum_groups_b16(hipStream_t st, const void* X, int G, int rows_per_group, int C, float* out, float* scratch);
 
-int edge_bwd_reduce_parts(int P, int Cout, const void* a, const void* b, const void* c, const void* d, const void* e, const void* f, int lddo,
-                          int ldo);
+int edge_bwd_reduce_parts(int P, int Cout, const void* a, const void* b, const void* c, const void* d, const void* e, int lddo, int ldo);
 int edge_reduce_parts(int P);
 bool build_wd_leaves_bound(int Cout, int C);
 int launch_build_wd(hipStream_t st, const float* W, int Cout, int C, float* Wd, float* amax = nullptr);
@@ -89,21 +88,22 @@
                          const float* rva, float* sva, int Cb, const float* gb, const float* bb, const float* rmb, const float* rvb, float* svb,
                          float eps);
 int launch_unbuild_wd(hipStream_t st, const float* dWd, int Cout, int C, float* dW);
-int launch_edge_reduce(hipStream_t st, const float* uv, const int* idx, const float* gamma, int P, int N, int Cout, int k, float* msel,
+int launch_edge_reduce(hipStream_t st, const float* uv, const int* idx, const float* gamma, int P, int N, int Cout, int k, float* ysel,
                        uint8_t* argsel, float* s1, double* part, int* nparts_used);
-int launch_edge_select_act(hipStream_t st, const float* msel, const float* uv, int P, int Cout, const float* scale, const float* shift, int act,
-                           float slope, float* out, int ldo);
-bool edge_bwd_leaves_duv_bound(const float* dOut, const float* out, const float* msel, const float* uv, const float* s1, const uint8_t* argsel,
+int launch_edge_select_act(hipStream_t st, const float* ysel, int P, int Cout, const float* scale, const float* shift, int act, float slope,
+                           float* out, int ldo);
+bool edge_bwd_leaves_duv_bound(const float* dOut, const float* out, const float* ysel, const float* uv, const float* s1, const uint8_t* argsel,
                                int Cout, const float* scale, const float* mean, const float* invstd, const float* gz, const float* duv, int lddo,
                                int ldo);
-int launch_edge_bwd_reduce(hipStream_t st, const float* dOut, const float* out, const float* msel, const float* uv, int P, int Cout,
-                           const float* mean, const float* invstd, int act, float slope, double* part, int lddo, int ldo, float* duv_amax);
+int launch_edge_bwd_reduce(hipStream_t st, const float* dOut, const float* out, const float* ysel, int P, int Cout, const float* scale,
+                           const float* mean, const float* invstd, int act, float slope, double* part, int lddo, int ldo, float* gz,
+                           float* duv_amax);
 int launch_edge_bwd_point(hipStream_t st, const float* dOut, const float* out, const float* uv, const float* s1, int P, int Cout, int k,
                           const float* scale, const float* mean, const float* invstd, const float* mean_dz, const float* mean_dzy, int act,
                           float slope, float* gz, float* duv, int lddo, int ldo, float* duv_amax);
-int launch_edge_bwd_gather(hipStream_t st, const float* gz, const uint8_t* argsel, const float* uv, const int* rev_off, const int* rev_ent, int P,
-                           int N, int Cout, const float* scale, const float* mean, const float* invstd, const float* mean_dz, const float* mean_dzy,
-                           float* duv, float* duv_amax);
+int launch_edge_bwd_gather(hipStream_t st, const float* gz, const uint8_t* argsel, const float* uv, const float* s1, int k, const int* rev_off,
+                           const int* rev_ent, int P, int N, int Cout, const float* scale, const float* mean, const float* invstd,
+                           const float* mean_dz, const float* mean_dzy, float* duv, float* duv_amax);
 int launch_graph_feature_fwd(hipStream_t st, const float* x, const int* idx, int P, int N, int C, int k, float* F);
 int launch_graph_feature_bwd(hipStream_t st, const float* dF, const int* rev_off, const int* rev_ent, int P, int N, int C, int k, float* dx);
 
```

Measured after the change: 8.674 million points/s, median of 6. +1.8%, better.
